# wengroup/matten

Hardware: AMD Instinct MI355X
Metric: edge_tensor_products_per_sec (higher is better)
Workload: dtype f32; 1 GPU; configs[2]: synthetic fcc-64 crystals (64 atoms, cutoff 5 A, 1152 edges each), paper hparams lmax=4, eval forward backbone+out_layer, one batch per step per GPU; last conv layer run for its live outputs only (258/842 radial-weight columns: the irreps its only reader takes) -- `value` counts 4 edge-TP per edge all the same, `value_full_layers` is the rate with the full last layer; nodes_per_gpu=64000, edges_per_gpu=1152000, conv_layers=4

## Files before the change

### include/matten_hip.h

```cpp
#ifndef MATTEN_HIP_H
#define MATTEN_HIP_H

#include <stddef.h>
#include <stdint.h>

#ifdef __cplusplus
extern "C" {
#endif

typedef void* matten_stream_t;

#define MATTEN_OK 0
#define MATTEN_EINVAL (-1)
#define MATTEN_ELAUNCH (-2)
#define MATTEN_ENOMEM (-3)

int matten_abi_version(void);

#define MATTEN_RADIAL_MAX_MID 3

size_t matten_csr_workspace_bytes(int64_t n_edges, int64_t n_nodes);
int matten_csr_counting_max_avg_degree(void);
int matten_csr_build(const int64_t* edge_index, int64_t n_edges, int64_t n_nodes, int32_t* perm,
                     int32_t* rowptr, int32_t* src_sorted, void* workspace, size_t workspace_bytes,
                     int32_t* err_flag, matten_stream_t stream);

int64_t matten_csr_split_bound(int64_t n_nodes, int64_t n_edges, int64_t max_len);
int matten_csr_split(const int32_t* rowptr, int64_t n_nodes, int64_t n_edges, int64_t max_len, int32_t* vrowptr,
                     int64_t* vseg, const float* num_neigh, float* vnn, matten_stream_t stream);

size_t matten_group_workspace_bytes(int64_t n, int64_t n_keys);
int matten_group_by_key(const int64_t* key, int64_t n, int64_t n_keys, int32_t* order, int32_t* seg,
                        void* workspace, size_t workspace_bytes, int32_t* err_flag, matten_stream_t stream);

int matten_species_embed(const int64_t* atomic_numbers, int64_t n_nodes, const int64_t* z_to_index,
                         int64_t min_z, int64_t max_z, int64_t n_species, const float* weight ,
                         const float* bias , int64_t dim, int64_t* species_index, int32_t* species_i32,
                         float* node_feats, float* node_attrs, int32_t* err_flag, matten_stream_t stream);

int matten_edge_geom(const float* pos, const int64_t* edge_index, const float* edge_cell_shift,
                     const float* cell, int64_t n_cells, const int64_t* batch, const int32_t* perm,
                     int64_t n_edges, int64_t n_nodes, int lmax, int n_basis, float r_start, float r_end,
                     float* geom_sorted, float* sh_sorted, int sh_stride, float* edge_vectors, float* edge_lengths,
                     float* edge_attrs, float* edge_embedding, matten_stream_t stream);

int matten_radial_mlp(const float* geom_sorted, int64_t n_edges, int n_basis, float r_start, float r_end,
                      const float* w0p, int nb_pad, const float* w1p, const float* w2p, int hidden, int w_pad,
                      float act_cst, void* w_edge, int out_is_bf16, matten_stream_t stream);
int matten_radial_mlp_deep(const float* geom_sorted, int64_t n_edges, int n_basis, float r_start, float r_end,
                           const float* w0p, int nb_pad, const float* w_mid, int n_mid, const float* w2p, int hidden,
                           int w_pad, float act_cst, void* w_edge, int out_is_bf16, matten_stream_t stream);

int matten_tp_tile_nodes(void);
int matten_tp_paths(const float* x, int64_t d_in, const void* w_edge, int64_t w_pad, const float* sh_sorted,
                    int64_t sh_dim, const int32_t* rowptr, const int32_t* src_sorted, int64_t n_nodes,
                    const int32_t* path_entries, const int32_t* unit_start, int64_t n_entries,
                    int64_t units_per_tile, int64_t d_mid, float avg_num_neighbors, const float* num_neigh,
                    float* agg , int w_is_bf16, matten_stream_t stream);

int matten_agg_linear_max_mt(void);
int matten_agg_linear_block_chunks(void);
size_t matten_agg_linear_lds_bytes(int64_t w_stride, int64_t n_io, int64_t n_blocks);
size_t matten_agg_linear_max_lds_bytes(void);
int matten_agg_linear(const float* agg, int64_t ld, const int32_t* order, const int32_t* seg, int64_t n_species,
                      const float* wtab, int64_t w_stride, const int32_t* io_table, int64_t n_io,
                      const int32_t* blocks, int64_t n_blocks, const float* add, int64_t add_ld, int64_t d_out,
                      int64_t n_rows, float* out, matten_stream_t stream);
int matten_agg_linear_gate(const float* agg, int64_t ld, const int32_t* order, const int32_t* seg, int64_t n_species,
                           const float* wtab, int64_t w_stride, const int32_t* io_table, int64_t n_io,
                           const int32_t* blocks, int64_t n_blocks, const float* add, int64_t add_ld, int64_t d_out,
                           int64_t n_rows, const int32_t* cmeta, const float* act_cst, const float* bn_scale,
                           const float* bn_shift, int64_t d_act, float* out, matten_stream_t stream);
int matten_agg_linear_gate_sets(void);
int matten_radial_hidden(const float* geom_sorted, int64_t n_edges, int n_basis, float r_start, float r_end,
                         const float* w0p, int nb_pad, const float* w1p, int hidden, uint16_t* h2s,
                         const float* h_scale, matten_stream_t stream);
int matten_radial_hidden_multi(const float* geom_sorted, int64_t n_edges, int n_basis, float r_start, float r_end,
                               const float* const* w0p, int nb_pad, const float* const* w1p, int hidden,
                               uint16_t* const* h2s, const float* const* h_scale, int n_layers,
                               matten_stream_t stream);
int matten_radial_hidden_deep(const float* geom_sorted, int64_t n_edges, int n_basis, float r_start, float r_end,
                              const float* w0p, int nb_pad, const float* w_mid, int n_mid, int hidden, uint16_t* h2s,
                              const float* h_scale, matten_stream_t stream);
int matten_radial_hidden_multi_deep(const float* geom_sorted, int64_t n_edges, int n_basis, float r_start, float r_end,
                                    const float* const* w0p, int nb_pad, const float* const* w_mid, int n_mid, int hidden,
                                    uint16_t* const* h2s, const float* const* h_scale, int n_layers,
                                    matten_stream_t stream);
int matten_tp_fused(const float* x, int64_t d_in, const uint16_t* h2s, const float* w2p, int64_t w_pad,
                    const float* sh_sorted, int64_t sh_stride, const int32_t* rowptr, const int32_t* src_sorted,
                    int64_t n_nodes, const int32_t* group_entries, const int32_t* unit_map, int64_t n_entries,
                    int64_t units_per_tile, int64_t lds_floats_per_wave, int64_t d_mid, float avg_num_neighbors,
                    const float* num_neigh, const uint16_t* a_split, const float* a_scale_inv,
                    float* agg , matten_stream_t stream);

int matten_tp_max_cols(void);
int matten_tp_max_cols_l0(void);
int matten_tp_max_cols_l1(void);
int matten_tp_groups_hash(void);

int matten_species_linear(const float* x, int64_t d_in, const int32_t* order, const int32_t* seg, int64_t n_species,
                          const float* wp, int64_t w_stride, const int32_t* segs, int64_t n_segs, int64_t d_out,
                          const float* add, int64_t add_ld, int64_t n_rows, float* out, matten_stream_t stream);

int matten_species_linear_rows(const float* x, int64_t d_in, const int32_t* order, const int32_t* seg, int64_t n_species,
                               const float* wp, int64_t w_stride, const int32_t* segs, int64_t n_segs, int64_t d_out,
                               const float* add, int64_t add_ld, int64_t n_rows, float* out, matten_stream_t stream);

int matten_gate_bn(const float* x, int64_t d_in, const int32_t* meta, int64_t d_out, const float* act_cst,
                   const float* running_mean, const float* running_var, const float* bn_weight,
                   const float* bn_bias, float eps, int64_t n_rows, float* out, matten_stream_t stream);

int matten_segment_reduce(const float* x, int64_t dim, const int64_t* ptr, int64_t n_segments, int mean,
                          float* out, matten_stream_t stream);
int matten_segment_minmax(const float* x, int64_t dim, const int64_t* ptr, int64_t n_segments, int take_max, float* out,
                          int64_t* arg, matten_stream_t stream);
int matten_segment_minmax_bwd(const float* dy, int64_t dim, const int64_t* arg, int64_t n_segments, float* dx,
                              matten_stream_t stream);

int64_t matten_radial_mlp_bwd_small_slices(int64_t n_edges);
int64_t matten_radial_mlp_bwd_w2_ranges(int64_t n_edges, int64_t w_pad);
int matten_radial_mlp_bwd(const float* geom_sorted, int64_t n_edges, int n_basis, float r_start, float r_end,
                          const float* w0p, int nb_pad, const float* w1p, const float* w2p, int hidden, int w_pad,
                          int w_cols, const void* dw, int64_t dw_ld, int dw_is_bf16, float* h2_scratch,
                          float* part_small, float* part_w2, float scale0, float scale1, float scale2,
                          float* grad_small, float* grad_w2, matten_stream_t stream);
int64_t matten_radial_mlp_bwd_w2_ranges_deep(int64_t n_edges, int64_t w_pad, int n_mid);
int matten_radial_mlp_bwd_deep(const float* geom_sorted, int64_t n_edges, int n_basis, float r_start, float r_end,
                               const float* w0p, int nb_pad, const float* w_mid, int n_mid, const float* w2p, int hidden,
                               int w_pad, int w_cols, const void* dw, int64_t dw_ld, int dw_is_bf16, float* h2_scratch,
                               float* part_small, float* part_w2, float scale0, float scale1, float scale2,
                               float* grad_small, float* grad_w2, matten_stream_t stream);
int matten_radial_pack(const float* w0, const float* w1, const float* w2, int n_basis, int nb_pad, int w_cols, int w_pad,
                       float scale0, float scale1, float scale2, float* w0p, float* w1p, float* w2p,
                       matten_stream_t stream);
int matten_radial_pack_deep(const float* w0, const float* w_mid, int n_mid, const float* w2, int n_basis, int nb_pad,
                            int w_cols, int w_pad, float scale0, float scale1, float scale2, float* w0p, float* w_mid_p,
                            float* w2p, matten_stream_t stream);
int matten_radial_pack_cols(const float* w0, const float* w1, const float* w2, int n_basis, int nb_pad, int w_cols,
                            const int64_t* cols, int n_cols, int w_pad, float scale0, float scale1, float scale2, float* w0p,
                            float* w1p, float* w2p, matten_stream_t stream);
int matten_radial_h_scale(const float* w0, const float* w1, int n_basis, float r_start, float r_end, float act_cst,
                          float* out2, matten_stream_t stream);
int matten_radial_pack_cols_deep(const float* w0, const float* w_mid, int n_mid, const float* w2, int n_basis, int nb_pad,
                                 int w_cols, const int64_t* cols, int n_cols, int w_pad, float scale0, float scale1,
                                 float scale2, float* w0p, float* w_mid_p, float* w2p, matten_stream_t stream);
int matten_radial_h_scale_deep(const float* w0, const float* w_mid, int n_mid, int n_basis, float r_start, float r_end,
// ... 34 lines not shown
                                 int64_t dw_ld, int edge_is_bf16, int64_t n_nodes, const int32_t* out_ptr,
                                 const int32_t* out_perm, float* dx_edges, int64_t lds_floats, int max_l, int max_mul,
                                 matten_stream_t stream);

int matten_species_linear_wgrad(const float* x, int64_t d_in, const float* dy, int64_t d_out, const int32_t* order,
                                const int32_t* seg, int64_t n_species, int64_t n_rows, const int32_t* segs,
                                int64_t n_segs, int64_t w_stride, float* dwp, float* scratch, matten_stream_t stream);

int matten_gate_bwd(const float* x, int64_t d_in, const int32_t* meta, int64_t d_out, const float* act_cst,
                    const float* dy, int64_t n_rows, float* dx, matten_stream_t stream);

int64_t matten_bn_scratch_floats(int64_t n_rows, int64_t dim);
int matten_bn_train_fwd(const float* x, int64_t dim, int64_t n_rows, const int32_t* col2chan, const int32_t* chan,
                        int64_t n_chan, const float* weight, const float* bias, float eps, float* mean, float* nu,
                        float* y, float* running_mean, float* running_var, float momentum, float* scratch,
                        matten_stream_t stream);
int matten_bn_train_bwd(const float* x, const float* dy, int64_t dim, int64_t n_rows, const int32_t* col2chan,
                        const int32_t* chan, int64_t n_chan, const float* mean, const float* nu, const float* weight,
                        float eps, float* A, float* B, float* dx, float* dweight, float* dbias, float* scratch,
                        matten_stream_t stream);

int matten_norm_act(const float* x, int64_t dim, int64_t n_rows, const int32_t* chan, int64_t n_chan, int act,
                    float epsilon, const float* running_mean, const float* running_var, const float* bn_weight,
                    const float* bn_bias, float bn_eps, float* y, matten_stream_t stream);
int matten_norm_act_bwd(const float* x, const float* dy, int64_t dim, int64_t n_rows, const int32_t* chan, int64_t n_chan,
                        int act, float epsilon, float* dx, matten_stream_t stream);

int matten_instance_norm_fwd(const float* x, int64_t dim, int64_t n_rows, const int64_t* seg_ptr, const int64_t* seg_of_row,
                             int64_t n_seg, const int32_t* col2chan, const int32_t* chan, int64_t n_chan,
                             const float* weight, const float* bias, float eps, float* mean, float* nu, float* y,
                             matten_stream_t stream);
int matten_instance_norm_bwd(const float* x, const float* dy, int64_t dim, int64_t n_rows, const int64_t* seg_ptr,
                             const int64_t* seg_of_row, int64_t n_seg, const int32_t* col2chan, const int32_t* chan,
                             int64_t n_chan, const float* mean, const float* nu, const float* weight, float eps, float* A,
                             float* B, float* dx, matten_stream_t stream);

int matten_segment_reduce_bwd(const float* dy, int64_t dim, const int64_t* ptr, int64_t n_segments, int mean, float* dx,
                              matten_stream_t stream);


int matten_graph_prep(const double* pos, const double* cell, const int64_t* ptr, int64_t n_crystals, double r_cut,
                      double* frac, double* bound, int64_t* batch, float* pos_f32, float* cell_f32,
                      matten_stream_t stream);
int matten_neighbor_count(const double* pos, const double* cell, const int64_t* ptr, const double* frac,
                          const double* bound, const int64_t* pair_ptr, double r_cut, int64_t n_crystals,
                          int64_t max_atoms, int32_t* counts, int32_t* counts_t, matten_stream_t stream);
int matten_neighbor_summary(const int64_t* offsets, const int64_t* pair_ptr, int64_t n_crystals, int64_t* out2,
                            matten_stream_t stream);
int matten_neighbor_fill(const double* pos, const double* cell, const int64_t* ptr, const double* frac,
                         const double* bound, const int64_t* pair_ptr, double r_cut, int64_t n_crystals,
                         int64_t max_atoms, const int64_t* offsets, int64_t n_edges, int64_t* edge_index,
                         float* edge_cell_shift, float* num_neigh, const int64_t* offsets_t, int64_t n_atoms,
                         int32_t* rowptr, int32_t* src_sorted, int32_t* perm, matten_stream_t stream);

#ifdef __cplusplus
}
#endif
#endif
```

### matten_amd/_lib.py

```python
from __future__ import annotations

import ctypes
import os
from ctypes import c_float, c_int, c_int32, c_int64, c_size_t, c_void_p

_HERE = os.path.dirname(os.path.abspath(__file__))
LIB_PATH = os.path.join(_HERE, "libmatten_hip.so")

ABI_VERSION = 45

P = c_void_p
SIGNATURES = {
    "matten_abi_version": (c_int, []),
    "matten_csr_workspace_bytes": (c_size_t, [c_int64, c_int64]),
    "matten_group_workspace_bytes": (c_size_t, [c_int64, c_int64]),
    "matten_csr_counting_max_avg_degree": (c_int, []),
    "matten_csr_build": (c_int, [P, c_int64, c_int64, P, P, P, P, c_size_t, P, P]),
    "matten_csr_split_bound": (c_int64, [c_int64, c_int64, c_int64]),
    "matten_csr_split": (c_int, [P, c_int64, c_int64, c_int64, P, P, P, P, P]),
    "matten_group_by_key": (c_int, [P, c_int64, c_int64, P, P, P, c_size_t, P, P]),
    "matten_species_embed": (c_int, [P, c_int64, P, c_int64, c_int64, c_int64, P, P, c_int64, P, P, P, P, P, P]),
    "matten_edge_geom": (c_int, [P, P, P, P, c_int64, P, P, c_int64, c_int64, c_int, c_int, c_float, c_float, P, P, c_int, P, P, P, P, P]),
    "matten_radial_mlp": (c_int, [P, c_int64, c_int, c_float, c_float, P, c_int, P, P, c_int, c_int, c_float, P, c_int, P]),
    "matten_radial_mlp_deep": (c_int, [P, c_int64, c_int, c_float, c_float, P, c_int, P, c_int, P, c_int, c_int, c_float, P, c_int,
                                       P]),
    "matten_tp_tile_nodes": (c_int, []),
    "matten_tp_paths": (c_int, [P, c_int64, P, c_int64, P, c_int64, P, P, c_int64, P, P, c_int64, c_int64, c_int64, c_float, P, P, c_int,
                                P]),
    "matten_radial_hidden_multi": (c_int, [P, c_int64, c_int, c_float, c_float, P, c_int, P, c_int, P, P, c_int, P]),
    "matten_radial_hidden_multi_deep": (c_int, [P, c_int64, c_int, c_float, c_float, P, c_int, P, c_int, c_int, P, P, c_int, P]),
    "matten_agg_linear_max_mt": (c_int, []),
    "matten_agg_linear_block_chunks": (c_int, []),
    "matten_agg_linear_lds_bytes": (c_size_t, [c_int64, c_int64, c_int64]),
    "matten_agg_linear_max_lds_bytes": (c_size_t, []),
    "matten_agg_linear": (c_int, [P, c_int64, P, P, c_int64, P, c_int64, P, c_int64, P, c_int64, P, c_int64, c_int64,
                                  c_int64, P, P]),
    "matten_agg_linear_gate": (c_int, [P, c_int64, P, P, c_int64, P, c_int64, P, c_int64, P, c_int64, P, c_int64, c_int64,
                                       c_int64, P, P, P, P, c_int64, P, P]),
    "matten_agg_linear_gate_sets": (c_int, []),
    "matten_radial_hidden": (c_int, [P, c_int64, c_int, c_float, c_float, P, c_int, P, c_int, P, P, P]),
    "matten_radial_hidden_deep": (c_int, [P, c_int64, c_int, c_float, c_float, P, c_int, P, c_int, c_int, P, P, P]),
    "matten_tp_max_cols": (c_int, []),
    "matten_tp_max_cols_l0": (c_int, []),
    "matten_tp_max_cols_l1": (c_int, []),
    "matten_tp_groups_hash": (c_int, []),
    "matten_tp_fused": (c_int, [P, c_int64, P, P, c_int64, P, c_int64, P, P, c_int64, P, P, c_int64, c_int64, c_int64, c_int64, c_float, P, P, P, P, P]),
    "matten_species_linear": (c_int, [P, c_int64, P, P, c_int64, P, c_int64, P, c_int64, c_int64, P, c_int64, c_int64, P, P]),
    "matten_species_linear_rows": (c_int, [P, c_int64, P, P, c_int64, P, c_int64, P, c_int64, c_int64, P, c_int64, c_int64, P, P]),
    "matten_radial_mlp_bwd_small_slices": (c_int64, [c_int64]),
    "matten_radial_mlp_bwd_w2_ranges": (c_int64, [c_int64, c_int64]),
    "matten_radial_mlp_bwd_w2_ranges_deep": (c_int64, [c_int64, c_int64, c_int]),
    "matten_radial_mlp_bwd": (c_int, [P, c_int64, c_int, c_float, c_float, P, c_int, P, P, c_int, c_int, c_int, P, c_int64,
                                      c_int, P, P, P, c_float, c_float, c_float, P, P, P]),
    "matten_radial_mlp_bwd_deep": (c_int, [P, c_int64, c_int, c_float, c_float, P, c_int, P, c_int, P, c_int, c_int, c_int, P,
                                           c_int64, c_int, P, P, P, c_float, c_float, c_float, P, P, P]),
    "matten_radial_pack": (c_int, [P, P, P, c_int, c_int, c_int, c_int, c_float, c_float, c_float, P, P, P, P]),
    "matten_radial_pack_deep": (c_int, [P, P, c_int, P, c_int, c_int, c_int, c_int, c_float, c_float, c_float, P, P, P, P]),
    "matten_radial_pack_cols": (c_int, [P, P, P, c_int, c_int, c_int, P, c_int, c_int, c_float, c_float, c_float, P, P, P, P]),
    "matten_radial_pack_cols_deep": (c_int, [P, P, c_int, P, c_int, c_int, c_int, P, c_int, c_int, c_float, c_float, c_float, P, P,
                                             P, P]),
    "matten_radial_h_scale": (c_int, [P, P, c_int, c_float, c_float, c_float, P, P]),
    "matten_radial_h_scale_deep": (c_int, [P, P, c_int, c_int, c_float, c_float, c_float, P, P]),
    "matten_split_a_tiles": (c_int, [P, c_int64, P, c_int64, P, P, P, P]),
    "matten_gather_scale": (c_int, [P, P, P, c_int64, c_int64, c_int, P, P, P, P]),
    "matten_species_linear_wgrad_scratch_floats": (c_int64, [c_int64, c_int64, c_int64]),
    "matten_tp_backward": (c_int, [P, c_int64, P, c_int64, P, c_int64, P, P, P, c_int64, P, P, P, c_int64, c_float, P, c_int64, P, P, c_int64,
                                   P, P, c_int64, c_int, P]),
    "matten_tp_backward_lit": (c_int, [P, c_int64, P, c_int64, P, c_int64, P, P, P, c_int64, c_int64, P, c_int64, P, c_int64, c_float,
                                       P, c_int64, P, P, c_int64, c_int, c_int64, P, P, P, c_int, P]),
    "matten_tp_backward_lit_wfree": (c_int, [P, c_int64, P, P, P, P, c_int64, P, P, P, c_int64, c_int64, P, c_int64, P, c_int64, c_float,
                                             P, c_int64, P, P, c_int64, c_int, c_int64, P, P, P, c_int64, c_int, c_int, P]),
    "matten_adam_step": (c_int, [P, P, P, P, c_int64, P, c_float, c_float, c_float, c_float, c_float, P]),
    "matten_species_linear_wgrad": (c_int, [P, c_int64, P, c_int64, P, P, c_int64, c_int64, P, c_int64, c_int64, P, P, P]),
    "matten_gate_bwd": (c_int, [P, c_int64, P, c_int64, P, P, c_int64, P, P]),
    "matten_bn_scratch_floats": (c_int64, [c_int64, c_int64]),
    "matten_bn_train_fwd": (c_int, [P, c_int64, c_int64, P, P, c_int64, P, P, c_float, P, P, P, P, P, c_float, P, P]),
    "matten_bn_train_bwd": (c_int, [P, P, c_int64, c_int64, P, P, c_int64, P, P, P, c_float, P, P, P, P, P, P, P]),
    "matten_norm_act": (c_int, [P, c_int64, c_int64, P, c_int64, c_int, c_float, P, P, P, P, c_float, P, P]),
    "matten_norm_act_bwd": (c_int, [P, P, c_int64, c_int64, P, c_int64, c_int, c_float, P, P]),
    "matten_instance_norm_fwd": (c_int, [P, c_int64, c_int64, P, P, c_int64, P, P, c_int64, P, P, c_float, P, P, P, P]),
    "matten_instance_norm_bwd": (c_int, [P, P, c_int64, c_int64, P, P, c_int64, P, P, c_int64, P, P, P, c_float, P, P, P, P]),
    "matten_segment_reduce_bwd": (c_int, [P, c_int64, P, c_int64, c_int, P, P]),
    "matten_graph_prep": (c_int, [P, P, P, c_int64, ctypes.c_double, P, P, P, P, P, P]),
    "matten_neighbor_count": (c_int, [P, P, P, P, P, P, ctypes.c_double, c_int64, c_int64, P, P, P]),
    "matten_neighbor_summary": (c_int, [P, P, c_int64, P, P]),
    "matten_neighbor_fill": (c_int, [P, P, P, P, P, P, ctypes.c_double, c_int64, c_int64, P, c_int64, P, P, P, P, c_int64,
                                     P, P, P, P]),
    "matten_gate_bn": (c_int, [P, c_int64, P, c_int64, P, P, P, P, P, c_float, c_int64, P, P]),
    "matten_segment_reduce": (c_int, [P, c_int64, P, c_int64, c_int, P, P]),
    "matten_segment_minmax": (c_int, [P, c_int64, P, c_int64, c_int, P, P, P]),
    "matten_segment_minmax_bwd": (c_int, [P, c_int64, P, c_int64, P, P]),
    "matten_dense_rows": (c_int, [P, c_int64, P, c_int64, c_int64, P, P]),
}

_lib = None


class MattenHipError(RuntimeError):
    pass


def load() -> ctypes.CDLL:
    global _lib
    if _lib is not None:
        return _lib
    if not os.path.exists(LIB_PATH):
        raise MattenHipError(
            f"{LIB_PATH} not found: the HIP extension is not built. matten_amd has no CPU fallback; "
            "run `make -C matten_amd/csrc` (needs hipcc, --offload-arch=gfx950)."
        )
    lib = ctypes.CDLL(LIB_PATH)
    for name, (res, args) in SIGNATURES.items():
        try:
            fn = getattr(lib, name)
        except AttributeError as e:
            raise MattenHipError(f"symbol {name} missing from {LIB_PATH}") from e
        fn.restype = res
        fn.argtypes = args
    v = lib.matten_abi_version()
    if v != ABI_VERSION:
        raise MattenHipError(f"ABI version mismatch: library {v}, python binding {ABI_VERSION}")
    _lib = lib
    return lib


_ERRORS = {-1: "MATTEN_EINVAL (bad argument)", -2: "MATTEN_ELAUNCH (HIP launch failed)", -3: "MATTEN_ENOMEM (workspace too small)"}


def check(rc: int, what: str) -> None:
    if rc != 0:
        raise MattenHipError(f"{what} failed: {_ERRORS.get(rc, rc)}")
```

### matten_amd/autograd.py

```python
from typing import Optional

import os

import torch

from . import ops


class SpeciesEmbedFn(torch.autograd.Function):

    @staticmethod
    def forward(ctx, weight, bias, feats, species_order, segs):
        ctx.species_order, ctx.segs = species_order, segs
        ctx.n_species = weight.shape[1]
        return feats.view_as(feats)

    @staticmethod
    def backward(ctx, g):
        g = g.contiguous()
        n, dim = g.shape
        ones = torch.ones(n, 1, dtype=torch.float32, device=g.device)
        per_species = ops.species_linear_wgrad(ones, g, ctx.species_order, ctx.n_species, [ctx.segs], dim)
        return per_species.t(), per_species.sum(0), None, None, None

# ... 115 lines not shown
    @staticmethod
    def backward(ctx, g):
        x, w_edge = ctx.saved_tensors
        mod, dev = ctx.mod, g.device
        sh, src, dst = ctx.graph
        impl = os.environ.get("MATTEN_TP_BWD", "lit")
        if impl == "lit":
            out_csr = ctx.out_csr if os.environ.get("MATTEN_TP_BWD_DX", "ordered") != "atomic" else None
            dx, dw = ops.tp_backward_lit(x, w_edge, sh, src, dst, mod._tables.get("bw_blocks", dev),
                                         mod._tables.get("bw_paths", dev), mod.plan.bw_sum_lanes, g.contiguous(), ctx.avg,
                                         ctx.num_neigh, out_csr=out_csr, max_l=mod.plan.bw_max_l,
                                         blocks_cover_input=int(mod.plan.bw_blocks[:, 1].dot(2 * mod.plan.bw_blocks[:, 2] + 1))
                                         == mod.plan.d_in)
            return dx, dw, None, None, None, None
        dx, dw = ops.tp_backward(x, w_edge, sh, src, dst, mod._tables.get("bw_col_meta", dev),
                                 mod._tables.get("bw_nnz_ijk", dev), mod._tables.get("bw_nnz_c", dev), g.contiguous(),
                                 ctx.avg, ctx.num_neigh,
                                 in_groups=None if os.environ.get("MATTEN_TP_BWD_GROUPED", "1") == "0" else
                                 (mod._tables.get("bw_in_ptr", dev), mod._tables.get("bw_in_cols", dev)))
        return dx, dw, None, None, None, None


W_FREE_ADJOINT = os.environ.get("MATTEN_TP_BWD_WFREE", "1") != "0"


class FusedTensorProductFn(torch.autograd.Function):

    @staticmethod
    def forward(ctx, x, mod, data, avg, num_neigh, *ws):
        from .data.irreps import DataKey

        dev = x.device
        p, mlp = mod.plan, mod.weight_nn
        nb, r0, r1 = data[DataKey.AMD_RBF].tolist()
        ctx.mod, ctx.avg, ctx.num_neigh = mod, avg, num_neigh
        ctx.rbf = (int(nb), float(r0), float(r1))
        ctx.graph = (data[DataKey.AMD_GEOM], data[DataKey.AMD_SH], data[DataKey.AMD_SRC], data["_amd_dst_sorted"])
        ctx.out_csr = data.get("_amd_out_csr")
        ctx.save_for_backward(x, *ws)
        gent = mod._tables.get("gentries", dev)
        if mlp.deep:
            w0p, w1p, w2p, hs, frag, inv = ops.fused_operands_deep(ws[0], _stack_mid(ws), ws[-1], mlp.pack_scales(),
                                                                   mod._tables.get("fused_cols", dev), gent, p.fused_a_tiles,
                                                                   r0, r1, mlp.act_cst)
            h2p = ops.radial_hidden_deep(data[DataKey.AMD_GEOM], int(nb), r0, r1, w0p, w1p, hs)
        else:
            w0p, w1p, w2p, hs, frag, inv = ops.fused_operands(*ws, mlp.pack_scales(), mod._tables.get("fused_cols", dev),
                                                              gent, p.fused_a_tiles, r0, r1, mlp.act_cst)
            h2p = ops.radial_hidden(data[DataKey.AMD_GEOM], int(nb), r0, r1, w0p, w1p, hs)
        if W_FREE_ADJOINT and p.bw_max_mul <= ops.WFREE_MAX_MUL:
            ctx.h2p, ctx.hs = h2p, hs
        return ops.tp_fused(x, h2p, w2p, data[DataKey.AMD_SH], data[DataKey.AMD_ROWPTR], data[DataKey.AMD_SRC], gent,
                            mod._tables.get("gumap", dev), len(p.fused_unit_map), p.fused_lds_floats_per_wave, p.d_mid, avg,
                            num_neigh, a_split=(frag, inv))

    @staticmethod
    def backward(ctx, g):
        x, *ws = ctx.saved_tensors
        mod, dev = ctx.mod, g.device
        mlp = mod.weight_nn
        geom, sh, src, dst = ctx.graph
        scales = mlp.pack_scales()
        w0p, w1p, w2p = _radial_pack(mlp, ws)
        out_csr = ctx.out_csr if os.environ.get("MATTEN_TP_BWD_DX", "ordered") != "atomic" else None
        covered = int(mod.plan.bw_blocks[:, 1].dot(2 * mod.plan.bw_blocks[:, 2] + 1)) == mod.plan.d_in
        h2p = getattr(ctx, "h2p", None)
        if h2p is not None:
            frag, inv = ops.split_a_tiles_dev(w2p, mod._tables.get("bw_w_entries", dev), mod.plan.bw_a_tiles, ctx.hs)
            dx, dw = ops.tp_backward_lit(x, None, sh, src, dst, mod._tables.get("bw_blocks", dev),
                                         mod._tables.get("bw_paths", dev), mod.plan.bw_sum_lanes, g.contiguous(), ctx.avg,
                                         ctx.num_neigh, out_csr=out_csr, blocks_cover_input=covered, wfree=(h2p, frag, inv),
                                         dw_shape=((geom.shape[0], w2p.shape[1]), EDGE_STORAGE_DTYPE),
                                         lds_floats=mod.plan.bw_wfree_lds_floats, max_l=mod.plan.bw_max_l,
                                         max_mul=mod.plan.bw_max_mul)
        else:
            w_edge = _radial_mlp(mlp, geom, ctx.rbf, w0p, w1p, w2p)
            dx, dw = ops.tp_backward_lit(x, w_edge, sh, src, dst, mod._tables.get("bw_blocks", dev),
                                         mod._tables.get("bw_paths", dev), mod.plan.bw_sum_lanes, g.contiguous(), ctx.avg,
                                         ctx.num_neigh, out_csr=out_csr, blocks_cover_input=covered, max_l=mod.plan.bw_max_l)
            del w_edge
        return (dx, None, None, None, None) + _radial_mlp_bwd(mlp, geom, ctx.rbf, w0p, w1p, w2p, dw, scales)


class GateFn(torch.autograd.Function):
    @staticmethod
    def forward(ctx, x, mod):
        dev = x.device
        ctx.mod = mod
        ctx.save_for_backward(x)
        return ops.gate_bn(x, mod._tables.get("meta", dev), mod._tables.get("act_cst", dev))

    @staticmethod
    def backward(ctx, g):
        (x,) = ctx.saved_tensors
        mod, dev = ctx.mod, g.device
        return ops.gate_bwd(x, mod._tables.get("meta", dev), mod._tables.get("act_cst", dev), g.contiguous()), None


class NormActFn(torch.autograd.Function):
    @staticmethod
    def forward(ctx, x, mod):
        ctx.mod = mod
        ctx.save_for_backward(x)
        return ops.norm_act(x, mod._tables.get("chan", x.device), mod.plan.act_code, mod.plan.epsilon)

    @staticmethod
    def backward(ctx, g):
# ... 88 lines not shown
```

### matten_amd/csrc/csr.hip

```cpp
#include <cstring>

#include <rocprim/device/device_radix_sort.hpp>
#include <rocprim/device/device_scan.hpp>

#include "common.h"

namespace {

__global__ void csr_keys_kernel(const int64_t* __restrict__ edge_index, int64_t E, int64_t N,
                                int32_t* __restrict__ keys, int32_t* __restrict__ vals, int32_t* err_flag) {
    int64_t e = (int64_t)blockIdx.x * blockDim.x + threadIdx.x;
    if (e >= E) return;
    int64_t s = edge_index[e];
    int64_t d = edge_index[E + e];
    if (s < 0 || s >= N || d < 0 || d >= N) {
        atomicOr(err_flag, 1);
        d = d < 0 ? 0 : (d >= N ? N - 1 : d);
    }
    keys[e] = (int32_t)d;
    vals[e] = (int32_t)e;
}

__global__ void csr_rowptr_kernel(const int32_t* __restrict__ keys_sorted, int64_t E, int64_t N,
                                  int32_t* __restrict__ rowptr) {
    int64_t n = (int64_t)blockIdx.x * blockDim.x + threadIdx.x;
    if (n > N) return;
    int64_t lo = 0, hi = E;
    while (lo < hi) {
        int64_t mid = (lo + hi) >> 1;
        if (keys_sorted[mid] < (int32_t)n) lo = mid + 1; else hi = mid;
    }
    rowptr[n] = (int32_t)lo;
}

__global__ void csr_src_kernel(const int64_t* __restrict__ edge_index, const int32_t* __restrict__ perm, int64_t E,
                               int64_t N, int32_t* __restrict__ src_sorted) {
    int64_t e = (int64_t)blockIdx.x * blockDim.x + threadIdx.x;
    if (e >= E) return;
    int64_t s = edge_index[perm[e]];
    s = s < 0 ? 0 : (s >= N ? N - 1 : s);
    src_sorted[e] = (int32_t)s;
}

__global__ void zero_i32_kernel(int32_t* __restrict__ p, int64_t n) {
    int64_t i = (int64_t)blockIdx.x * blockDim.x + threadIdx.x;
    if (i < n) p[i] = 0;
}

__global__ void csr_count_kernel(const int64_t* __restrict__ edge_index, int64_t E, int64_t N,
                                 int32_t* __restrict__ deg, int32_t* __restrict__ slot, int32_t* err_flag) {
    int64_t e = (int64_t)blockIdx.x * blockDim.x + threadIdx.x;
    if (e >= E) return;
    int64_t s = edge_index[e];
    int64_t d = edge_index[E + e];
    if (s < 0 || s >= N || d < 0 || d >= N) {
        atomicOr(err_flag, 1);
        d = d < 0 ? 0 : (d >= N ? N - 1 : d);
    }
    slot[e] = atomicAdd(&deg[d], 1);
}

__global__ void csr_place_kernel(const int64_t* __restrict__ edge_index, int64_t E, int64_t N,
                                 const int32_t* __restrict__ rowptr, const int32_t* __restrict__ slot,
                                 int32_t* __restrict__ ids) {
    int64_t e = (int64_t)blockIdx.x * blockDim.x + threadIdx.x;
    if (e >= E) return;
    int64_t d = edge_index[E + e];
    d = d < 0 ? 0 : (d >= N ? N - 1 : d);
    ids[rowptr[d] + slot[e]] = (int32_t)e;
}

constexpr int CSR_HUB_DEGREE = 2048;
constexpr int CSR_HUB_THREADS = 1024;
constexpr int CSR_HUB_BLOCKS = 64;

__global__ void csr_rank_kernel(const int64_t* __restrict__ edge_index, const int32_t* __restrict__ rowptr,
                                const int32_t* __restrict__ ids, int64_t E, int64_t N, int32_t* __restrict__ perm,
                                int32_t* __restrict__ src_sorted, int32_t* __restrict__ hubs) {
    const int64_t node = ((int64_t)blockIdx.x * blockDim.x + threadIdx.x) >> 4;
    if (node >= N) return;
    const int sub = threadIdx.x & 15;
    const int beg = rowptr[node], d = rowptr[node + 1] - beg;
    if (d > CSR_HUB_DEGREE) {
        if (sub == 0) hubs[atomicAdd(&hubs[N], 1)] = (int32_t)node;
        return;
    }
    for (int i = sub; i < d; i += 16) {
        const int id = ids[beg + i];
        int rank = 0;
        int j = 0;
        for (; j + 8 <= d; j += 8) {
            int v[8];
#pragma unroll
            for (int q = 0; q < 8; ++q) v[q] = ids[beg + j + q];
#pragma unroll
            for (int q = 0; q < 8; ++q) rank += v[q] < id;
        }
        for (; j < d; ++j) rank += ids[beg + j] < id;
        perm[beg + rank] = id;
        int64_t s = edge_index[id];
        s = s < 0 ? 0 : (s >= N ? N - 1 : s);
        src_sorted[beg + rank] = (int32_t)s;
    }
}

__global__ __launch_bounds__(CSR_HUB_THREADS) void csr_hub_kernel(const int64_t* __restrict__ edge_index,
                                                                  const int32_t* __restrict__ rowptr, int32_t* ids,
                                                                  int64_t N, int32_t* __restrict__ perm,
                                                                  int32_t* __restrict__ src_sorted,
                                                                  const int32_t* __restrict__ hubs) {
    const int n_hubs = hubs[N];
    for (int h = blockIdx.x; h < n_hubs; h += gridDim.x) {
        const int node = hubs[h];
        const int beg = rowptr[node], d = rowptr[node + 1] - beg;
        int32_t* a = ids + beg;
        for (int64_t k = 2; (k >> 1) < d; k <<= 1) {
            for (int64_t j = k >> 1; j > 0; j >>= 1) {
                const int64_t m = (j == (k >> 1)) ? k - 1 : j;
                for (int64_t i = threadIdx.x; i < d; i += CSR_HUB_THREADS) {
                    const int64_t l = i ^ m;
                    if (l > i && l < d) {
                        const int32_t x = a[i], y = a[l];
                        if (y < x) a[i] = y, a[l] = x;
                    }
                }
                __syncthreads();
            }
        }
        for (int64_t i = threadIdx.x; i < d; i += CSR_HUB_THREADS) {
            const int32_t id = a[i];
            perm[beg + i] = id;
            int64_t s = edge_index[id];
            s = s < 0 ? 0 : (s >= N ? N - 1 : s);
            src_sorted[beg + i] = (int32_t)s;
        }
        __syncthreads();
    }
}

__global__ void group_keys_kernel(const int64_t* __restrict__ key, int64_t n, int64_t n_keys,
                                  int32_t* __restrict__ keys, int32_t* __restrict__ vals, int32_t* err_flag) {
    int64_t i = (int64_t)blockIdx.x * blockDim.x + threadIdx.x;
    if (i >= n) return;
    int64_t k = key[i];
    if (k < 0 || k >= n_keys) {
        atomicOr(err_flag, 1);
        k = k < 0 ? 0 : n_keys - 1;
    }
    keys[i] = (int32_t)k;
    vals[i] = (int32_t)i;
}

constexpr int GROUP_COUNTING_MAX_KEYS = 256;
constexpr int GROUP_WAVES = 4;

__device__ __forceinline__ int group_key_of(const int64_t* __restrict__ key, int64_t i, int64_t n, int64_t n_keys,
                                            int32_t* err_flag) {
    if (i >= n) return -1;
    int64_t k = key[i];
    if (k < 0 || k >= n_keys) {
        atomicOr(err_flag, 1);
        k = k < 0 ? 0 : n_keys - 1;
    }
    return (int)k;
}

__global__ __launch_bounds__(GROUP_WAVES * 64) void group_hist_kernel(const int64_t* __restrict__ key, int64_t n,
                                                                      int64_t n_keys, int64_t n_runs,
                                                                      int32_t* __restrict__ cnt, int32_t* err_flag) {
    __shared__ int h[GROUP_WAVES][GROUP_COUNTING_MAX_KEYS];
    const int wv = threadIdx.x >> 6, lane = threadIdx.x & 63;
    const int64_t run = (int64_t)blockIdx.x * GROUP_WAVES + wv;
    for (int kk = lane; kk < n_keys; kk += 64) h[wv][kk] = 0;
    __builtin_amdgcn_wave_barrier();
    const int k = group_key_of(key, run * 64 + lane, n, n_keys, err_flag);
    if (k >= 0) atomicAdd(&h[wv][k], 1);
    __builtin_amdgcn_s_waitcnt(0xc07f);
    __builtin_amdgcn_wave_barrier();
    if (run < n_runs)
        for (int kk = lane; kk < n_keys; kk += 64) cnt[(int64_t)kk * n_runs + run] = h[wv][kk];
}

__global__ __launch_bounds__(GROUP_WAVES * 64) void group_place_kernel(const int64_t* __restrict__ key, int64_t n,
                                                                       int64_t n_keys, int64_t n_runs,
                                                                       const int32_t* __restrict__ offs,
                                                                       int32_t* __restrict__ order,
                                                                       int32_t* __restrict__ seg, int32_t* err_flag) {
    const int lane = threadIdx.x & 63;
    const int64_t i = (int64_t)blockIdx.x * blockDim.x + threadIdx.x;
    const int64_t run = i >> 6;
    if (i <= n_keys) seg[i] = i < n_keys ? offs[i * n_runs] : (int32_t)n;
    const int k = group_key_of(key, i, n, n_keys, err_flag);
    unsigned long long todo = __ballot(k >= 0);
    int rank = 0;
    while (todo) {
        const int kf = __shfl(k, __ffsll((long long)todo) - 1);
        const unsigned long long m = __ballot(k == kf);
        if (k == kf) rank = __popcll(m & ((1ull << lane) - 1ull));
        todo &= ~m;
    }
    if (k >= 0) order[offs[(int64_t)k * n_runs + run] + rank] = (int32_t)i;
}

inline size_t align256(size_t x) { return (x + 255) & ~(size_t)255; }

inline int key_bits(int64_t N) {
    int b = 1;
    while (((int64_t)1 << b) < N && b < 31) ++b;
    return b;
}

}

__global__ __launch_bounds__(1024) void csr_split_kernel(const int* __restrict__ rowptr, int N, int max_len, int nv_bound,
                                                         int* __restrict__ vrowptr, int64_t* __restrict__ vseg,
                                                         const float* __restrict__ num_neigh, float* __restrict__ vnn) {
    __shared__ int sh[1024];
    __shared__ int carry_s;
    const int t = threadIdx.x;
    if (t == 0) carry_s = 0;
    __syncthreads();
    const int E = rowptr[N];
    for (int base = 0; base < N; base += 1024) {
        const int n = base + t;
        int beg = 0, k = 0, d = 0;
        if (n < N) {
            beg = rowptr[n];
            d = rowptr[n + 1] - beg;
            k = max(1, (d + max_len - 1) / max_len);
        }
        sh[t] = k;
        __syncthreads();
        for (int off = 1; off < 1024; off <<= 1) {
            const int v = t >= off ? sh[t - off] : 0;
            __syncthreads();
            sh[t] += v;
            __syncthreads();
        }
        const int carry = carry_s;
        const int first = carry + sh[t] - k;
        if (n < N) {
            vseg[n] = first;
            for (int i = 0; i < k; ++i) {
                const int v = first + i;
                if (v < nv_bound) {
                    vrowptr[v] = beg + (int)((int64_t)i * d / k);
                    if (vnn) vnn[v] = num_neigh[n];
                }
            }
        }
        __syncthreads();
        if (t == 1023) carry_s = carry + sh[1023];
        __syncthreads();
    }
    const int nv = min(carry_s, nv_bound);
    if (t == 0) vseg[N] = nv;
    for (int v = nv + t; v <= nv_bound; v += 1024) {
        vrowptr[v] = E;
        if (vnn && v < nv_bound) vnn[v] = 1.0f;
    }
}

extern "C" size_t matten_csr_workspace_bytes(int64_t E, int64_t N) {
    if (E < 0 || N < 0) return 0;
    size_t tmp = 0;
    int32_t* p = nullptr;
    (void)rocprim::radix_sort_pairs(nullptr, tmp, p, p, p, p, (size_t)(E > 0 ? E : 1), 0, key_bits(N), 0, false);
    size_t scan_tmp = 0;
    (void)rocprim::exclusive_scan(nullptr, scan_tmp, p, p, 0, (size_t)(N + 1), rocprim::plus<int32_t>());
    return 3 * align256((size_t)(E > 0 ? E : 1) * sizeof(int32_t)) + align256(tmp) + align256((size_t)(N + 1) * sizeof(int32_t)) +
           align256(scan_tmp) + 256;
}

extern "C" size_t matten_group_workspace_bytes(int64_t n, int64_t n_keys) {
    if (n < 0 || n_keys <= 0) return 0;
    size_t need = matten_csr_workspace_bytes(n, n_keys);
    if (n_keys <= GROUP_COUNTING_MAX_KEYS) {
        const size_t table = (size_t)n_keys * (size_t)((n + 63) / 64 + 1);
        size_t scan_tmp = 0;
        int32_t* p = nullptr;
        (void)rocprim::exclusive_scan(nullptr, scan_tmp, p, p, 0, table, rocprim::plus<int32_t>());
        const size_t counting = 2 * align256(table * sizeof(int32_t)) + align256(scan_tmp) + 256;
        if (counting > need) need = counting;
    }
    return need;
}

constexpr int64_t CSR_COUNTING_MAX_AVG_DEGREE = 64;

extern "C" int matten_csr_counting_max_avg_degree(void) { return (int)CSR_COUNTING_MAX_AVG_DEGREE; }

extern "C" int matten_csr_build(const int64_t* edge_index, int64_t E, int64_t N, int32_t* perm, int32_t* rowptr,
                                int32_t* src_sorted, void* workspace, size_t workspace_bytes, int32_t* err_flag,
                                matten_stream_t stream_) {
    hipStream_t stream = (hipStream_t)stream_;
    if (E < 0 || N < 0 || N >= ((int64_t)1 << 31) || E >= ((int64_t)1 << 31)) return MATTEN_EINVAL;
    if (!rowptr || !err_flag) return MATTEN_EINVAL;
    if (E == 0) {
        zero_i32_kernel<<<(unsigned)matten_cdiv(N + 1, 256), 256, 0, stream>>>(rowptr, N + 1);
        MATTEN_LAUNCH_CHECK();
        return MATTEN_OK;
    }
    if (!edge_index || !perm || !src_sorted || !workspace) return MATTEN_EINVAL;
    size_t need = matten_csr_workspace_bytes(E, N);
    if (workspace_bytes < need) return MATTEN_ENOMEM;

    char* ws = (char*)workspace;
    size_t seg = align256((size_t)E * sizeof(int32_t));
    int32_t* keys_in = (int32_t*)ws;
    int32_t* keys_out = (int32_t*)(ws + seg);
    int32_t* vals_in = (int32_t*)(ws + 2 * seg);
    void* tmp = ws + 3 * seg;
    size_t tmp_bytes = workspace_bytes - 3 * seg;

    const int T = 256;
    if (N > 0 && E <= CSR_COUNTING_MAX_AVG_DEGREE * N) {
        int32_t* ids = (int32_t*)ws;
        int32_t* slot = (int32_t*)(ws + seg);
        int32_t* deg = (int32_t*)(ws + 2 * seg);
        const size_t deg_bytes = align256((size_t)(N + 1) * sizeof(int32_t));
        void* scan_tmp = ws + 2 * seg + deg_bytes;
        size_t scan_bytes = workspace_bytes - 2 * seg - deg_bytes;
        zero_i32_kernel<<<(unsigned)matten_cdiv(N + 1, T), T, 0, stream>>>(deg, N + 1);
        MATTEN_LAUNCH_CHECK();
        csr_count_kernel<<<(unsigned)matten_cdiv(E, T), T, 0, stream>>>(edge_index, E, N, deg, slot, err_flag);
        MATTEN_LAUNCH_CHECK();
        if (rocprim::exclusive_scan(scan_tmp, scan_bytes, deg, rowptr, 0, (size_t)(N + 1), rocprim::plus<int32_t>(),
                                    stream) != hipSuccess)
            return MATTEN_ELAUNCH;
        csr_place_kernel<<<(unsigned)matten_cdiv(E, T), T, 0, stream>>>(edge_index, E, N, rowptr, slot, ids);
        MATTEN_LAUNCH_CHECK();
        csr_rank_kernel<<<(unsigned)matten_cdiv(N * 16, T), T, 0, stream>>>(edge_index, rowptr, ids, E, N, perm,
                                                                           src_sorted, deg);
        MATTEN_LAUNCH_CHECK();
        if (E > CSR_HUB_DEGREE) {
            const int64_t max_hubs = E / CSR_HUB_DEGREE;
            csr_hub_kernel<<<(unsigned)(max_hubs < CSR_HUB_BLOCKS ? max_hubs : CSR_HUB_BLOCKS), CSR_HUB_THREADS, 0,
                             stream>>>(edge_index, rowptr, ids, N, perm, src_sorted, deg);
            MATTEN_LAUNCH_CHECK();
        }
        return MATTEN_OK;
    }
    csr_keys_kernel<<<(unsigned)matten_cdiv(E, T), T, 0, stream>>>(edge_index, E, N, keys_in, vals_in, err_flag);
    MATTEN_LAUNCH_CHECK();
    if (rocprim::radix_sort_pairs(tmp, tmp_bytes, keys_in, keys_out, vals_in, perm, (size_t)E, 0, key_bits(N), stream,
                                  false) != hipSuccess)
        return MATTEN_ELAUNCH;
    csr_rowptr_kernel<<<(unsigned)matten_cdiv(N + 1, T), T, 0, stream>>>(keys_out, E, N, rowptr);
    MATTEN_LAUNCH_CHECK();
    csr_src_kernel<<<(unsigned)matten_cdiv(E, T), T, 0, stream>>>(edge_index, perm, E, N, src_sorted);
    MATTEN_LAUNCH_CHECK();
    return MATTEN_OK;
}

extern "C" int matten_group_by_key(const int64_t* key, int64_t n, int64_t n_keys, int32_t* order, int32_t* seg,
                                   void* workspace, size_t workspace_bytes, int32_t* err_flag, matten_stream_t stream_) {
    hipStream_t stream = (hipStream_t)stream_;
    if (n < 0 || n_keys <= 0 || n_keys >= ((int64_t)1 << 31) || n >= ((int64_t)1 << 31)) return MATTEN_EINVAL;
    if (!seg || !err_flag) return MATTEN_EINVAL;
    if (n == 0) {
        zero_i32_kernel<<<(unsigned)matten_cdiv(n_keys + 1, 256), 256, 0, stream>>>(seg, n_keys + 1);
        MATTEN_LAUNCH_CHECK();
        return MATTEN_OK;
    }
    if (!key || !order || !workspace) return MATTEN_EINVAL;
    if (workspace_bytes < matten_group_workspace_bytes(n, n_keys)) return MATTEN_ENOMEM;
    char* ws = (char*)workspace;
    if (n_keys <= GROUP_COUNTING_MAX_KEYS) {
        const int64_t n_runs = (n + 63) / 64;
        const size_t table = (size_t)n_keys * (size_t)n_runs;
        const size_t tb = align256((size_t)n_keys * (size_t)(n_runs + 1) * sizeof(int32_t));
        int32_t* cnt = (int32_t*)ws;
        int32_t* offs = (int32_t*)(ws + tb);
        void* scan_tmp = ws + 2 * tb;
        size_t scan_bytes = workspace_bytes - 2 * tb;
        const int TB = GROUP_WAVES * 64;
        group_hist_kernel<<<(unsigned)matten_cdiv(n_runs, GROUP_WAVES), TB, 0, stream>>>(key, n, n_keys, n_runs, cnt,
                                                                                        err_flag);
        MATTEN_LAUNCH_CHECK();
        if (rocprim::exclusive_scan(scan_tmp, scan_bytes, cnt, offs, 0, table, rocprim::plus<int32_t>(), stream) !=
            hipSuccess)
            return MATTEN_ELAUNCH;
        const int64_t threads = n > n_keys + 1 ? n : n_keys + 1;
        group_place_kernel<<<(unsigned)matten_cdiv(threads, TB), TB, 0, stream>>>(key, n, n_keys, n_runs, offs, order,
                                                                                 seg, err_flag);
        MATTEN_LAUNCH_CHECK();
        return MATTEN_OK;
    }
    size_t sg = align256((size_t)n * sizeof(int32_t));
    int32_t* keys_in = (int32_t*)ws;
    int32_t* keys_out = (int32_t*)(ws + sg);
    int32_t* vals_in = (int32_t*)(ws + 2 * sg);
    void* tmp = ws + 3 * sg;
    size_t tmp_bytes = workspace_bytes - 3 * sg;
    const int T = 256;
    group_keys_kernel<<<(unsigned)matten_cdiv(n, T), T, 0, stream>>>(key, n, n_keys, keys_in, vals_in, err_flag);
    MATTEN_LAUNCH_CHECK();
    if (rocprim::radix_sort_pairs(tmp, tmp_bytes, keys_in, keys_out, vals_in, order, (size_t)n, 0, key_bits(n_keys),
                                  stream, false) != hipSuccess)
        return MATTEN_ELAUNCH;
    csr_rowptr_kernel<<<(unsigned)matten_cdiv(n_keys + 1, T), T, 0, stream>>>(keys_out, n, n_keys, seg);
    MATTEN_LAUNCH_CHECK();
    return MATTEN_OK;
}

extern "C" int64_t matten_csr_split_bound(int64_t n_nodes, int64_t n_edges, int64_t max_len) {
    return max_len > 0 ? n_nodes + n_edges / max_len : n_nodes;
}

extern "C" int matten_csr_split(const int32_t* rowptr, int64_t n_nodes, int64_t n_edges, int64_t max_len, int32_t* vrowptr,
                                int64_t* vseg, const float* num_neigh, float* vnn, matten_stream_t stream_) {
    if (n_nodes < 0 || n_edges < 0 || max_len <= 0 || n_nodes >= ((int64_t)1 << 30) || n_edges >= ((int64_t)1 << 31))
        return MATTEN_EINVAL;
    if (!rowptr || !vrowptr || !vseg || ((num_neigh == nullptr) != (vnn == nullptr))) return MATTEN_EINVAL;
    const int64_t bound = matten_csr_split_bound(n_nodes, n_edges, max_len);
    if (bound >= ((int64_t)1 << 31)) return MATTEN_EINVAL;
    csr_split_kernel<<<1, 1024, 0, (hipStream_t)stream_>>>(rowptr, (int)n_nodes, (int)max_len, (int)bound, vrowptr, vseg,
                                                          num_neigh, vnn);
    MATTEN_LAUNCH_CHECK();
    return MATTEN_OK;
}
```

### matten_amd/csrc/neighbor.hip

```cpp
#include "common.h"

#pragma clang fp contract(off)

namespace {

struct Cry {
    const double* pos;
    const double* cell;
    const int64_t* ptr;
    const double* frac;
    const double* bound;
    const int64_t* pair_ptr;
};

__global__ __launch_bounds__(64) void graph_prep_kernel(const double* __restrict__ pos, const double* __restrict__ cell,
                                                        const int64_t* __restrict__ ptr, double r_cut,
                                                        double* __restrict__ frac, double* __restrict__ bound,
                                                        int64_t* __restrict__ batch, float* __restrict__ pos_f32,
                                                        float* __restrict__ cell_f32) {
    const int64_t b = blockIdx.x;
    const double* cl = cell + 9 * b;
    const double ax = cl[0], ay = cl[1], az = cl[2], bx = cl[3], by = cl[4], bz = cl[5], cx = cl[6], cy = cl[7], cz = cl[8];
    const double c0x = by * cz - bz * cy, c0y = bz * cx - bx * cz, c0z = bx * cy - by * cx;
    const double c1x = cy * az - cz * ay, c1y = cz * ax - cx * az, c1z = cx * ay - cy * ax;
    const double c2x = ay * bz - az * by, c2y = az * bx - ax * bz, c2z = ax * by - ay * bx;
    const double det = (ax * c0x + ay * c0y) + az * c0z;
    const double i00 = c0x / det, i10 = c0y / det, i20 = c0z / det;
    const double i01 = c1x / det, i11 = c1y / det, i21 = c1z / det;
    const double i02 = c2x / det, i12 = c2y / det, i22 = c2z / det;
    if (threadIdx.x < 9) cell_f32[9 * b + threadIdx.x] = (float)cl[threadIdx.x];
    if (threadIdx.x == 0) {
        bound[3 * b] = r_cut * sqrt((i00 * i00 + i10 * i10) + i20 * i20);
        bound[3 * b + 1] = r_cut * sqrt((i01 * i01 + i11 * i11) + i21 * i21);
        bound[3 * b + 2] = r_cut * sqrt((i02 * i02 + i12 * i12) + i22 * i22);
    }
    const int64_t lo = ptr[b], hi = ptr[b + 1];
    for (int64_t n = lo + threadIdx.x; n < hi; n += blockDim.x) {
        const double x = pos[3 * n], y = pos[3 * n + 1], z = pos[3 * n + 2];
        frac[3 * n] = (x * i00 + y * i10) + z * i20;
        frac[3 * n + 1] = (x * i01 + y * i11) + z * i21;
        frac[3 * n + 2] = (x * i02 + y * i12) + z * i22;
        pos_f32[3 * n] = (float)x, pos_f32[3 * n + 1] = (float)y, pos_f32[3 * n + 2] = (float)z;
        batch[n] = b;
    }
}

__device__ __forceinline__ void shift_range(double bound, double df, int& lo, int& hi) {
    const double slack = 1e-6 * (1.0 + fabs(df) + bound);
    lo = (int)ceil(-bound - df - slack);
    hi = (int)floor(bound - df + slack);
}

struct CsrOut {
    const int64_t* offsets_t;
    int32_t* rowptr;
    int32_t* src_sorted;
    int32_t* perm;
    int64_t n_atoms;
};

template <bool FILL>
__global__ __launch_bounds__(256) void neighbor_kernel(Cry c, double r_cut, int32_t* __restrict__ counts,
                                                       int32_t* __restrict__ counts_t,
                                                       const int64_t* __restrict__ offsets,
                                                       int64_t* __restrict__ edge_index, int64_t n_edges,
                                                       float* __restrict__ shifts, float* __restrict__ num_neigh,
                                                       CsrOut csr) {
    const int64_t b = blockIdx.y;
    const int64_t lo = c.ptr[b];
    const int64_t n = c.ptr[b + 1] - lo;
    const int64_t t = (int64_t)blockIdx.x * blockDim.x + threadIdx.x;
    if (t >= n * n) return;
    const int64_t i = lo + t / n, j = lo + t % n;
    const int64_t pair = c.pair_ptr[b] + t;
    const double* cl = c.cell + 9 * b;
    int x0, x1, y0, y1, z0, z1;
    shift_range(c.bound[3 * b], c.frac[3 * j] - c.frac[3 * i], x0, x1);
    shift_range(c.bound[3 * b + 1], c.frac[3 * j + 1] - c.frac[3 * i + 1], y0, y1);
    shift_range(c.bound[3 * b + 2], c.frac[3 * j + 2] - c.frac[3 * i + 2], z0, z1);
    const double pix = c.pos[3 * i], piy = c.pos[3 * i + 1], piz = c.pos[3 * i + 2];
    const double pjx = c.pos[3 * j], pjy = c.pos[3 * j + 1], pjz = c.pos[3 * j + 2];
    const double r2 = r_cut * r_cut;
    const double r2_in = r2 * (1.0 - 1e-15), r2_out = r2 * (1.0 + 1e-15);
    int64_t out = FILL ? offsets[pair] : 0;
    if (FILL && num_neigh && j == lo) num_neigh[i] = (float)(offsets[pair + n] - offsets[pair]);
    const int64_t pair_t = c.pair_ptr[b] + (j - lo) * n + (i - lo);
    int64_t out_t = 0;
    if (FILL && csr.rowptr) {
        out_t = csr.offsets_t[pair_t] - csr.offsets_t[0];
        if (i == lo) csr.rowptr[j] = (int32_t)out_t;
        if (pair == 0) csr.rowptr[csr.n_atoms] = (int32_t)n_edges;
    }
    int cnt = 0;
    for (int sx = x0; sx <= x1; ++sx)
        for (int sy = y0; sy <= y1; ++sy) {
            const double ax = (double)sx * cl[0] + (double)sy * cl[3];
            const double ay = (double)sx * cl[1] + (double)sy * cl[4];
            const double az = (double)sx * cl[2] + (double)sy * cl[5];
            for (int sz = z0; sz <= z1; ++sz) {
                const double tx = ax + (double)sz * cl[6];
                const double ty = ay + (double)sz * cl[7];
                const double tz = az + (double)sz * cl[8];
                const double dx = (pjx + tx) - pix, dy = (pjy + ty) - piy, dz = (pjz + tz) - piz;
                const double d2 = (dx * dx + dy * dy) + dz * dz;
                bool hit = d2 < r2_in;
                if (!hit && d2 <= r2_out) hit = sqrt(d2) < r_cut;
                if (hit && !(i == j && sx == 0 && sy == 0 && sz == 0)) {
                    if (FILL) {
                        edge_index[out] = i;
                        edge_index[n_edges + out] = j;
                        shifts[3 * out] = (float)sx;
                        shifts[3 * out + 1] = (float)sy;
                        shifts[3 * out + 2] = (float)sz;
                        if (csr.rowptr) {
                            csr.perm[out_t] = (int32_t)out;
                            csr.src_sorted[out_t] = (int32_t)i;
                            ++out_t;
                        }
                        ++out;
                    }
                    ++cnt;
                }
            }
        }
    if (!FILL) {
        counts[pair] = cnt;
        if (counts_t) counts_t[pair_t] = cnt;
    }
}

__global__ __launch_bounds__(256) void neighbor_summary_kernel(const int64_t* __restrict__ offsets,
                                                               const int64_t* __restrict__ pair_ptr, int64_t n_crystals,
                                                               int64_t* __restrict__ out) {
    __shared__ long long red[256];
    long long m = LLONG_MAX;
    for (int64_t b = threadIdx.x; b < n_crystals; b += blockDim.x)
        m = min(m, (long long)(offsets[pair_ptr[b + 1]] - offsets[pair_ptr[b]]));
    red[threadIdx.x] = m;
    __syncthreads();
    for (int o = 128; o > 0; o >>= 1) {
        if (threadIdx.x < o) red[threadIdx.x] = min(red[threadIdx.x], red[threadIdx.x + o]);
        __syncthreads();
    }
    if (threadIdx.x == 0) {
        out[0] = offsets[pair_ptr[n_crystals]];
        out[1] = n_crystals > 0 ? (int64_t)red[0] : 0;
    }
}

}

extern "C" int matten_graph_prep(const double* pos, const double* cell, const int64_t* ptr, int64_t n_crystals,
                                 double r_cut, double* frac, double* bound, int64_t* batch, float* pos_f32,
                                 float* cell_f32, matten_stream_t stream_) {
    hipStream_t stream = (hipStream_t)stream_;
    if (n_crystals < 0 || !(r_cut > 0.0) || n_crystals >= ((int64_t)1 << 31)) return MATTEN_EINVAL;
    if (n_crystals == 0) return MATTEN_OK;
    if (!pos || !cell || !ptr || !frac || !bound || !batch || !pos_f32 || !cell_f32) return MATTEN_EINVAL;
    graph_prep_kernel<<<(unsigned)n_crystals, 64, 0, stream>>>(pos, cell, ptr, r_cut, frac, bound, batch, pos_f32, cell_f32);
    MATTEN_LAUNCH_CHECK();
    return MATTEN_OK;
}

extern "C" int matten_neighbor_count(const double* pos, const double* cell, const int64_t* ptr, const double* frac,
                                     const double* bound, const int64_t* pair_ptr, double r_cut, int64_t n_crystals,
                                     int64_t max_atoms, int32_t* counts, int32_t* counts_t, matten_stream_t stream_) {
    hipStream_t stream = (hipStream_t)stream_;
    if (n_crystals < 0 || max_atoms < 0 || !(r_cut > 0.0) || n_crystals > 65535) return MATTEN_EINVAL;
    if (n_crystals == 0 || max_atoms == 0) return MATTEN_OK;
    if (!pos || !cell || !ptr || !frac || !bound || !pair_ptr || !counts) return MATTEN_EINVAL;
    Cry c{pos, cell, ptr, frac, bound, pair_ptr};
    dim3 grid((unsigned)matten_cdiv(max_atoms * max_atoms, 256), (unsigned)n_crystals);
    neighbor_kernel<false><<<grid, 256, 0, stream>>>(c, r_cut, counts, counts_t, nullptr, nullptr, 0, nullptr, nullptr, CsrOut{});
    MATTEN_LAUNCH_CHECK();
    return MATTEN_OK;
}

extern "C" int matten_neighbor_summary(const int64_t* offsets, const int64_t* pair_ptr, int64_t n_crystals,
                                       int64_t* out2, matten_stream_t stream_) {
    hipStream_t stream = (hipStream_t)stream_;
    if (n_crystals < 0 || !offsets || !pair_ptr || !out2) return MATTEN_EINVAL;
    neighbor_summary_kernel<<<1, 256, 0, stream>>>(offsets, pair_ptr, n_crystals, out2);
    MATTEN_LAUNCH_CHECK();
    return MATTEN_OK;
}

extern "C" int matten_neighbor_fill(const double* pos, const double* cell, const int64_t* ptr, const double* frac,
                                    const double* bound, const int64_t* pair_ptr, double r_cut, int64_t n_crystals,
                                    int64_t max_atoms, const int64_t* offsets, int64_t n_edges, int64_t* edge_index,
                                    float* edge_cell_shift, float* num_neigh, const int64_t* offsets_t, int64_t n_atoms,
                                    int32_t* rowptr, int32_t* src_sorted, int32_t* perm, matten_stream_t stream_) {
    hipStream_t stream = (hipStream_t)stream_;
    if (n_crystals < 0 || max_atoms < 0 || n_edges < 0 || !(r_cut > 0.0) || n_crystals > 65535) return MATTEN_EINVAL;
    if (n_crystals == 0 || max_atoms == 0) return MATTEN_OK;
    if (!pos || !cell || !ptr || !frac || !bound || !pair_ptr || !offsets) return MATTEN_EINVAL;
    if (n_edges > 0 && (!edge_index || !edge_cell_shift)) return MATTEN_EINVAL;
    const bool want_csr = offsets_t || rowptr || src_sorted || perm;
    if (want_csr && (!offsets_t || !rowptr || n_atoms < 0 || n_edges >= ((int64_t)1 << 31) ||
                     (n_edges > 0 && (!src_sorted || !perm))))
        return MATTEN_EINVAL;
    Cry c{pos, cell, ptr, frac, bound, pair_ptr};
    CsrOut csr{offsets_t, want_csr ? rowptr : nullptr, src_sorted, perm, n_atoms};
    dim3 grid((unsigned)matten_cdiv(max_atoms * max_atoms, 256), (unsigned)n_crystals);
    neighbor_kernel<true><<<grid, 256, 0, stream>>>(c, r_cut, nullptr, nullptr, offsets, edge_index, n_edges, edge_cell_shift,
                                                    num_neigh, csr);
    MATTEN_LAUNCH_CHECK();
    return MATTEN_OK;
}
```

### matten_amd/csrc/node.hip

```cpp
#include "common.h"

namespace {

__device__ __forceinline__ float apply_act(int code, float v) {
    switch (code) {
        case 1: return v / (1.0f + expf(-v));
        case 2: return tanhf(v);
        case 3: return 1.0f / (1.0f + expf(-v));
        case 4: return (v > 20.0f ? v : log1pf(expf(v))) - 0.6931471805599453f;
        case 5: return fabsf(v);
        default: return v;
    }
}

#ifndef GB_R
#define GB_R 16
#endif
#ifndef GB_U
#define GB_U 8
#endif
constexpr int GB_ROWS = GB_R, GB_UNROLL = GB_U;
__global__ __launch_bounds__(256) void gate_bn_kernel(const float* __restrict__ x, int d_in,
                                                           const int4* __restrict__ meta, int d_out,
                                                           const float* __restrict__ act_cst,
// ... 121 lines not shown
}

extern "C" int matten_segment_reduce(const float* x, int64_t dim, const int64_t* ptr, int64_t n_segments, int mean,
                                     float* out, matten_stream_t stream_) {
    hipStream_t stream = (hipStream_t)stream_;
    if (n_segments < 0 || dim <= 0) return MATTEN_EINVAL;
    if (n_segments == 0) return MATTEN_OK;
    if (!x || !ptr || !out) return MATTEN_EINVAL;
    const int T = 256;
    segment_reduce_kernel<<<(unsigned)matten_cdiv(n_segments * dim, T), T, 0, stream>>>(x, (int)dim, ptr, n_segments,
                                                                                        mean, out);
    MATTEN_LAUNCH_CHECK();
    return MATTEN_OK;
}

extern "C" int matten_segment_minmax(const float* x, int64_t dim, const int64_t* ptr, int64_t n_segments, int take_max,
                                     float* out, int64_t* arg, matten_stream_t stream_) {
    hipStream_t stream = (hipStream_t)stream_;
    if (n_segments < 0 || dim <= 0) return MATTEN_EINVAL;
    if (n_segments == 0) return MATTEN_OK;
    if (!x || !ptr || !out) return MATTEN_EINVAL;
    const int T = 256;
    segment_minmax_kernel<<<(unsigned)matten_cdiv(n_segments * dim, T), T, 0, stream>>>(x, (int)dim, ptr, n_segments,
                                                                                        take_max, out, arg);
    MATTEN_LAUNCH_CHECK();
    return MATTEN_OK;
}

extern "C" int matten_segment_minmax_bwd(const float* dy, int64_t dim, const int64_t* arg, int64_t n_segments, float* dx,
                                         matten_stream_t stream_) {
    hipStream_t stream = (hipStream_t)stream_;
    if (n_segments < 0 || dim <= 0) return MATTEN_EINVAL;
    if (n_segments == 0) return MATTEN_OK;
    if (!dy || !arg || !dx) return MATTEN_EINVAL;
    const int T = 256;
    segment_minmax_bwd_kernel<<<(unsigned)matten_cdiv(n_segments * dim, T), T, 0, stream>>>(dy, (int)dim, arg, n_segments, dx);
    MATTEN_LAUNCH_CHECK();
    return MATTEN_OK;
}

extern "C" int matten_dense_rows(const float* x, int64_t n_in, const float* q, int64_t n_out, int64_t n_rows,
                                 float* out, matten_stream_t stream_) {
    hipStream_t stream = (hipStream_t)stream_;
    if (n_rows < 0 || n_in <= 0 || n_out <= 0) return MATTEN_EINVAL;
    if (n_rows == 0) return MATTEN_OK;
    if (!x || !q || !out) return MATTEN_EINVAL;
    const int T = 256;
    dense_rows_kernel<<<(unsigned)matten_cdiv(n_rows * n_out, T), T, 0, stream>>>(x, (int)n_in, q, (int)n_out, n_rows,
                                                                                  out);
    MATTEN_LAUNCH_CHECK();
    return MATTEN_OK;
}

extern "C" int matten_abi_version(void) { return 45; }
```

### matten_amd/csrc/tp_fused.hip

```cpp
#include "tp_walk.h"

namespace {

using namespace matten_walk;

constexpr int KIND_MERGED = 256;
struct StoreAgg {
    template <class G>
    __device__ __forceinline__ void store(const Args& a, const GroupEntry& ge, const float* __restrict__ acc,
                                          float a_scale_inv, int node, int j, int u, bool valid) const {
        if (TPF_LAB_NO_STORE ? (valid && acc[0] == 12345.678f) : valid) {
            const float nn = a.avg_nn > 0.0f ? a.avg_nn : a.num_neigh[node];
            const float norm = a_scale_inv / sqrtf(nn);
            float* orow = a.agg + (int64_t)node * a.d_mid;
            const bool merged = (ge.kind & KIND_MERGED) != 0;
            const GroupEntry& g2 = (&ge)[merged ? 1 : 0];
            const bool second = merged && u >= 2;
            const unsigned mask = merged ? (second ? g2.mask : (unsigned)g2.w_base) : ge.mask;
            const int uc = second ? u - 2 : u;
#pragma unroll
            for (int cc = 0; cc < G::NC; ++cc) {
                if ((mask >> cc) & 1u) {
                    const int d3 = 2 * G::L3[cc] + 1;
                    const int ks = second ? g2.t_off[cc] : ge.t_off[cc];
                    float* op = orow + (second ? g2.out_off[cc] : ge.out_off[cc]) + (ks ? uc : uc * d3);
                    const int kstep = ks ? ks : 1;
#pragma unroll
                    for (int k = 0; k < 2 * matten::CG_LMAX + 1; ++k)
                        if (k < d3) op[k * kstep] = acc[G::OFF[cc] + k] * norm;
                }
            }
        }
    }
};

template <int L1, int GI>
__device__ __forceinline__ void run_group(const Args& a, const GroupEntry& ge, float* __restrict__ tile, int node,
                                          int lane, bool valid, int beg, int deg_node, int maxdeg) {
    const int deg = valid ? deg_node : 0;
    using G = matten::Group<L1, GI>;
    constexpr int NC = G::NC;
    float acc[G::NACC];
#pragma unroll
    for (int k = 0; k < G::NACC; ++k) acc[k] = 0.0f;

    const unsigned mask = ge.mask;
    const int cu_log2 = ge.cu_log2;
    const int cu = 1 << cu_log2;
    const int npw = 64 >> cu_log2;
    const int ch_log2 = npw >= 16 ? 0 : (4 - (6 - cu_log2));
    const int CH = 1 << ch_log2;
    const int T = npw >= 16 ? (npw >> 4) : 1;
    const int ncols = ge.mul * NC;
    const int MT = (ncols + 15) >> 4;
    const int ycol = MT * 16;
    const int stride = MT * 16 + 32 + 4;

    const int j = lane >> cu_log2;
    const int u = lane & (cu - 1);
    const int g = lane >> 4, c = lane & 15;
    const int xcol = ge.x_off + u * G::D1;
    constexpr int CAPC = cap_channels(L1, NC);
    constexpr int MTMAX = (CAPC * NC + 15) / 16;
    f16x8 ah[MTMAX], al[MTMAX];
    float a_scale_inv;
    {
        float av[MTMAX][8];
        float amax = 0.0f;
#pragma unroll
        for (int mt = 0; mt < MTMAX; ++mt) {
#pragma unroll
            for (int kk = 0; kk < 8; ++kk) {
                const int k = 16 * (kk >> 2) + 4 * g + (kk & 3);
                av[mt][kk] = (mt < MT) ? a.w2p[(int64_t)k * a.w_pad + ge.w_base + mt * 16 + c] : 0.0f;
                amax = fmaxf(amax, fabsf(av[mt][kk]));
            }
        }
#pragma unroll
        for (int off = 32; off > 0; off >>= 1) amax = fmaxf(amax, __shfl_xor(amax, off));
        int e = (int)((__float_as_uint(amax) >> 23) & 0xffu) - 127;
        e = amax > 0.0f ? max(-100, min(100, e)) : 13;
        const float a_scale = __uint_as_float((unsigned)(127 + 13 - e) << 23);
        a_scale_inv = __uint_as_float((unsigned)(127 - 13 + e) << 23);
#pragma unroll
        for (int mt = 0; mt < MTMAX; ++mt) {
#pragma unroll
            for (int kk = 0; kk < 8; ++kk) {
                _Float16 hi, lo;
                split_f16(av[mt][kk] * a_scale, hi, lo);
                ah[mt][kk] = hi;
                al[mt][kk] = lo;
            }
        }
    }

    const int e_last = deg > 0 ? beg + deg - 1 : 0;
    float xn[G::D1];
    int src_nn;
    {
        const int src0 = a.src_sorted[min(beg, e_last)];
        src_nn = a.src_sorted[min(beg + 1, e_last)];
        const float* xp0 = a.x + (int64_t)src0 * a.d_in + xcol;
#pragma unroll
        for (int i = 0; i < G::D1; ++i) xn[i] = xp0[i];
    }
    for (int s0 = 0; s0 < maxdeg; s0 += CH) {
#pragma unroll
        for (int t = 0; t < 4; ++t) {
            if (t < T) {
                const int n = 16 * t + c;
                const int jn = n >> ch_log2, so = n & (CH - 1);
                const int begn = __shfl(beg, jn << cu_log2);
                const int degn = __shfl(deg_node, jn << cu_log2);
                f16x8 bh = {0, 0, 0, 0, 0, 0, 0, 0}, bl = {0, 0, 0, 0, 0, 0, 0, 0};
                if (s0 + so < degn) {
                    const int64_t en = begn + s0 + so;
                    const f16x8* hp = reinterpret_cast<const f16x8*>(a.h2s + en * (2 * HID) + g * 8);
                    bh = hp[0];
                    bl = hp[HID / 8];
                    const f32x4* yp4 = reinterpret_cast<const f32x4*>(a.sh + en * a.sh_stride + g * 8);
                    f32x4* yd = reinterpret_cast<f32x4*>(tile + (16 * t + c) * stride + ycol + g * 8);
                    yd[0] = yp4[0];
                    yd[1] = yp4[1];
                }
#pragma unroll
                for (int mt = 0; mt < MTMAX; ++mt) {
                    if (mt < MT) {
                        const f32x4 zero = {0.f, 0.f, 0.f, 0.f};
                        f32x4 dx = __builtin_amdgcn_mfma_f32_16x16x32_f16(al[mt], bh, zero, 0, 0, 0);
                        f32x4 dh = __builtin_amdgcn_mfma_f32_16x16x32_f16(ah[mt], bh, zero, 0, 0, 0);
                        dx = __builtin_amdgcn_mfma_f32_16x16x32_f16(ah[mt], bl, dx, 0, 0, 0);
                        *reinterpret_cast<f32x4*>(tile + (16 * t + c) * stride + mt * 16 + 4 * g) =
                            dh + SPLIT_LO_INV * dx;
                    }
                }
            }
        }
        __builtin_amdgcn_s_waitcnt(0xc07f);
        __builtin_amdgcn_wave_barrier();
        for (int so = 0; so < CH; ++so) {
            const int s = s0 + so;
            if (s >= maxdeg) break;
            float x[G::D1];
#pragma unroll
            for (int i = 0; i < G::D1; ++i) x[i] = xn[i];
            {
                const float* xp = a.x + (int64_t)src_nn * a.d_in + xcol;
#pragma unroll
                for (int i = 0; i < G::D1; ++i) xn[i] = xp[i];
                src_nn = a.src_sorted[min(beg + s + 2, e_last)];
            }
            if (s < deg) {
                const float* wp = tile + ((j << ch_log2) + so) * stride + u * NC;
                const float* yp = tile + ((j << ch_log2) + so) * stride + ycol + G::Y0;
                float y[G::NY], w[NC];
#pragma unroll
                for (int jj = 0; jj < G::NY; ++jj) y[jj] = yp[jj];
#pragma unroll
                for (int cc = 0; cc < NC; ++cc) w[cc] = wp[cc];
                G::apply(mask, x, y, w, acc);
            }
        }
        __builtin_amdgcn_wave_barrier();
    }
    StoreAgg{}.store<G>(a, ge, acc, a_scale_inv, node, j, u, valid);
}

#define MATTEN_RGS_ARGS a, ge, tile, stage, (um >> 8) & 0xffff, tile_id, r, reps, lane, StoreAgg{}
#define MATTEN_RGS(L1, GI, TT, TD, P) \
    do { \
        using HM = HotMask<L1, GI>; \
        if (HM::M0 && ge.mask == HM::M0) run_group_shared<L1, GI, TT, TD, P, HM::M0>(MATTEN_RGS_ARGS); \
        else if (HM::M1 && ge.mask == HM::M1) run_group_shared<L1, GI, TT, TD, P, HM::M1>(MATTEN_RGS_ARGS); \
        else run_group_shared<L1, GI, TT, TD, P, 0u>(MATTEN_RGS_ARGS); \
    } while (0)
#if defined(MATTEN_LAB) && defined(TPF_ONLY_VARIANT)
#ifndef TPF_ONLY_MASK
#define TPF_ONLY_MASK 0
#endif
#define MATTEN_RGS_ONLY(L1, GI, TT, TD, P) run_group_shared<L1, GI, TT, TD, P, (unsigned)(TPF_ONLY_MASK)>(MATTEN_RGS_ARGS)
#define MATTEN_GROUP_CASE_SHARED(L1, GI) \
    case (L1 * matten::GROUP_KIND_STRIDE + GI): \
        if (TPF_ONLY_VARIANT == 0) MATTEN_RGS_ONLY(L1, GI, 1, (TPF_CHUNK_DEEP && L1 == 0 ? 2 : 0), true); \
        else if (TPF_ONLY_VARIANT == 1) MATTEN_RGS_ONLY(L1, GI, 2, 0, false); \
        else if (TPF_ONLY_VARIANT == 2) MATTEN_RGS_ONLY(L1, GI, 1, (TPF_CHUNK_DEEP && L1 == 0 ? 2 : TwoDeepOk<L1, GI>::value ? 1 : 0), false); \
        else MATTEN_RGS_ONLY(L1, GI, 1, 0, false); \
        break;
#else
#define MATTEN_GROUP_CASE_SHARED(L1, GI) \
    case (L1 * matten::GROUP_KIND_STRIDE + GI): \
        if (paired && TPF_CHUNK_DEEP && L1 == 0 && nodes_per_wave <= 8 && nodes_per_wave >= 4) MATTEN_RGS(L1, GI, 1, (L1 == 0 ? 2 : 0), true); \
        else if (paired) MATTEN_RGS(L1, GI, 1, 0, true); \
        else if (nodes_per_wave > 16) MATTEN_RGS(L1, GI, 2, 0, false); \
        else if (TPF_CHUNK_DEEP && L1 == 0 && nodes_per_wave <= 8 && nodes_per_wave >= 4) MATTEN_RGS(L1, GI, 1, (L1 == 0 ? 2 : 0), false); \
        else if (TwoDeepOk<L1, GI>::value && nodes_per_wave <= 8 && nodes_per_wave >= TPF_TWO_DEEP_MIN_NPW) MATTEN_RGS(L1, GI, 1, (TwoDeepOk<L1, GI>::value ? 1 : 0), false); \
        else MATTEN_RGS(L1, GI, 1, 0, false); \
        break;
#endif

#define MATTEN_GROUP_CASE(L1, GI) \
    case (L1 * matten::GROUP_KIND_STRIDE + GI): run_group<L1, GI>(a, ge, tile, un.node, lane, un.valid, un.beg, un.deg, un.maxdeg); break;

#ifndef TPF_MIN_BLOCKS
#define TPF_MIN_BLOCKS 3
#endif
#ifndef TPF_CHUNK_DEEP
#define TPF_CHUNK_DEEP 1
#endif
#ifndef TPF_TWO_DEEP_MIN_NPW
#define TPF_TWO_DEEP_MIN_NPW 2
#endif
#if defined(MATTEN_LAB) && defined(TPF_ONLY_L1) && defined(TPF_ONLY_GI)
#define TPF_FOR_EACH_GROUP(X) X(TPF_ONLY_L1, TPF_ONLY_GI)
#elif defined(MATTEN_LAB) && defined(TPF_ONLY_LIGHT)
#define TPF_FOR_EACH_GROUP(X) X(0, 0) X(1, 0) X(1, 1)
#elif defined(MATTEN_LAB) && defined(TPF_ONLY_HEAVY)
#define TPF_FOR_EACH_GROUP(X) X(2, 0) X(2, 1) X(3, 0) X(3, 1) X(4, 0) X(4, 1)
#else
#define TPF_FOR_EACH_GROUP(X) MATTEN_FOR_EACH_GROUP(X)
#endif
__global__ __launch_bounds__(WAVES_PER_BLOCK * 64, TPF_MIN_BLOCKS) void tp_fused_kernel(Args a, const GroupEntry* __restrict__ entries,
                                                                        const int* __restrict__ umap,
                                                                        int n_entries, int units_per_tile,
                                                                        int blocks_per_tile, int n_tiles) {
    extern __shared__ __attribute__((aligned(16))) float lds[];
    const int xcd = blockIdx.x % N_XCD;
    const int q = blockIdx.x / N_XCD;
    const int tile_id = (q / blocks_per_tile) * N_XCD + xcd;
    if (tile_id >= n_tiles) return;
    const int wave = __builtin_amdgcn_readfirstlane(threadIdx.x >> 6);
    const int unit = (q % blocks_per_tile) * WAVES_PER_BLOCK + wave;
    if (unit >= units_per_tile) return;
    const int lane = threadIdx.x & 63;
    float* tile = lds + wave * a.lds_per_wave;

    const int um = __builtin_amdgcn_readfirstlane(umap[unit]);
    if (((um >> 8) & 0xffff) >= n_entries) return;
    const GroupEntry& ge = entries[(um >> 8) & 0xffff];
    const int r = um & 255;
    const bool shared_stage = (um >> 24) & 1;
    const int reps = 1 << ((um >> 27) & 3);

    const int cu_log2 = ge.cu_log2;
    const int nodes_per_wave = 64 >> cu_log2;
    if (shared_stage) {
        float* stage = lds + WAVES_PER_BLOCK * a.lds_per_wave;
        const bool paired = (um >> 26) & 1;
        if ((um >> 25) & 1) {
            if (paired) run_loader_only_paired(a, ge, stage, tile_id, r, reps, lane);
            else run_loader_only(a, ge, stage, tile_id, r, reps, lane);
            return;
        }
        switch (ge.kind & (KIND_MERGED - 1)) {
            TPF_FOR_EACH_GROUP(MATTEN_GROUP_CASE_SHARED)
            default: break;
        }
        return;
    }
#if !(defined(MATTEN_LAB) && defined(TPF_ONLY_VARIANT))
    const UnitNodes un = unit_nodes(a, ge, tile_id, r, lane);
    switch (ge.kind & (KIND_MERGED - 1)) {
        TPF_FOR_EACH_GROUP(MATTEN_GROUP_CASE)
        default: break;
    }
#endif
}

constexpr int NT = 4;
__device__ __forceinline__ float silu(float z) {
#if defined(MATTEN_LAB) && defined(RH_ABLATE_NO_SILU)
    return z * 0.5f;
#endif
    return z * __builtin_amdgcn_rcpf(1.0f + __builtin_amdgcn_exp2f(-1.4426950408889634f * z));
}

template <int KS0, int N_MID>
__global__ __launch_bounds__(256) void radial_hidden_kernel(const float4* __restrict__ geom, int64_t E, int n_basis,
                                                            float r_start, float r_end,
                                                            const float* __restrict__ w0p,
                                                            const float* __restrict__ w_mid, _Float16* __restrict__ h2s,
                                                            const float* __restrict__ h_scale) {
    const int lane = threadIdx.x & 63;
    const int wave = threadIdx.x >> 6;
    const int g = lane >> 4, c = lane & 15;
    const int64_t e0 = ((int64_t)blockIdx.x * 4 + wave) * (NT * 16);
    if (e0 >= E) return;
    const float hs = h_scale ? *h_scale : 1.0f;
    const float inv_c = 1.0f / (r_end - r_start);
    const float bes_pref = sqrtf(2.0f * inv_c) * sqrtf((float)n_basis);
    float a1[N_MID > 0 ? N_MID : 1][2][8];
#pragma unroll
    for (int m = 0; m < N_MID; ++m)
#pragma unroll
        for (int kk = 0; kk < 8; ++kk) {
            int k = 16 * (kk >> 2) + 4 * g + (kk & 3);
            a1[m][0][kk] = w_mid[m * HID * HID + k * HID + c];
            a1[m][1][kk] = w_mid[m * HID * HID + k * HID + 16 + c];
        }
    float lens[NT];
#pragma unroll
    for (int nt = 0; nt < NT; ++nt) {
        const int64_t e = e0 + nt * 16 + c;
        lens[nt] = geom[e < E ? e : E - 1].w;
    }
#pragma unroll
    for (int nt = 0; nt < NT; ++nt) {
        const int64_t e = e0 + nt * 16 + c;
        const float len = lens[nt];
        const float xr = len - r_start;
        const float t01 = xr * inv_c, inv_xr = __builtin_amdgcn_rcpf(xr);
        f32x4 h0 = {0.f, 0.f, 0.f, 0.f}, h1 = {0.f, 0.f, 0.f, 0.f};
#pragma unroll
        for (int kk = 0; kk < KS0; ++kk) {
// ... 207 lines not shown
                                const float* h_scale, matten_stream_t stream_) {
    hipStream_t stream = (hipStream_t)stream_;
    if (n_edges < 0 || hidden != HID || (nb_pad & 3) || nb_pad < n_basis || nb_pad > 16 || n_mid < 0 ||
        n_mid > MATTEN_RADIAL_MAX_MID)
        return MATTEN_EINVAL;
    if (n_edges == 0) return MATTEN_OK;
    if (!geom_sorted || !w0p || (n_mid > 0 && !w_mid) || !h2s) return MATTEN_EINVAL;
    unsigned grid = (unsigned)matten_cdiv(n_edges, 4 * NT * 16);
#define LAUNCH(K, M) \
    radial_hidden_kernel<K, M><<<grid, 256, 0, stream>>>((const float4*)geom_sorted, n_edges, n_basis, r_start, r_end, w0p, w_mid, (_Float16*)h2s, h_scale)
#define LAUNCH_M(K)                  \
    switch (n_mid) {                 \
        case 0: LAUNCH(K, 0); break; \
        case 1: LAUNCH(K, 1); break; \
        case 2: LAUNCH(K, 2); break; \
        default: LAUNCH(K, 3); break; \
    }
    switch (nb_pad >> 2) {
        case 1: LAUNCH_M(1); break;
        case 2: LAUNCH_M(2); break;
        case 3: LAUNCH_M(3); break;
        default: LAUNCH_M(4); break;
    }
#undef LAUNCH_M
#undef LAUNCH
    MATTEN_LAUNCH_CHECK();
    return MATTEN_OK;
}

extern "C" int matten_radial_hidden(const float* geom_sorted, int64_t n_edges, int n_basis, float r_start, float r_end,
                                    const float* w0p, int nb_pad, const float* w1p, int hidden, uint16_t* h2s,
                                    const float* h_scale, matten_stream_t stream_) {
    if (!w1p && n_edges > 0) return MATTEN_EINVAL;
    return radial_hidden_launch(geom_sorted, n_edges, n_basis, r_start, r_end, w0p, nb_pad, w1p, 1, hidden, h2s, h_scale,
                                stream_);
}

extern "C" int matten_radial_hidden_deep(const float* geom_sorted, int64_t n_edges, int n_basis, float r_start, float r_end,
                                         const float* w0p, int nb_pad, const float* w_mid, int n_mid, int hidden,
                                         uint16_t* h2s, const float* h_scale, matten_stream_t stream_) {
    return radial_hidden_launch(geom_sorted, n_edges, n_basis, r_start, r_end, w0p, nb_pad, w_mid, n_mid, hidden, h2s,
                                h_scale, stream_);
}

#if TPF_TRACING
static unsigned* g_tp_trace = nullptr;
static int64_t g_tp_trace_waves = 0, g_tp_trace_skip = 0;
extern "C" int matten_lab_tp_trace(unsigned* buf, int64_t n_waves, int64_t skip) {
    g_tp_trace = buf, g_tp_trace_waves = n_waves, g_tp_trace_skip = skip;
    return 0;
}
#endif

extern "C" int matten_tp_fused(const float* x, int64_t d_in, const uint16_t* h2s, const float* w2p, int64_t w_pad,
                               const float* sh_sorted, int64_t sh_stride, const int32_t* rowptr,
                               const int32_t* src_sorted, int64_t n_nodes, const int32_t* group_entries,
                               const int32_t* unit_map, int64_t n_entries, int64_t units_per_tile,
                               int64_t lds_floats_per_wave, int64_t d_mid, float avg_num_neighbors,
                               const float* num_neigh, const uint16_t* a_split, const float* a_scale_inv, float* agg,
                               matten_stream_t stream_) {
    hipStream_t stream = (hipStream_t)stream_;
    if (n_nodes < 0 || d_in <= 0 || w_pad <= 0 || sh_stride < 32 || (sh_stride & 3) || n_entries <= 0 ||
        units_per_tile <= 0 || d_mid <= 0 || lds_floats_per_wave <= 0 || (lds_floats_per_wave & 3))
        return MATTEN_EINVAL;
    if (n_nodes == 0) return MATTEN_OK;
    if (!x || !h2s || !w2p || !sh_sorted || !rowptr || !src_sorted || !group_entries || !unit_map || !agg)
        return MATTEN_EINVAL;
    if (!(avg_num_neighbors > 0.0f) && !num_neigh) return MATTEN_EINVAL;
    const size_t lds = sizeof(float) * ((size_t)lds_floats_per_wave * WAVES_PER_BLOCK + STAGE_TOTAL_FLOATS + PAIR_INFO_INTS);
    if (lds > 64 * 1024) return MATTEN_EINVAL;
    if ((a_split == nullptr) != (a_scale_inv == nullptr)) return MATTEN_EINVAL;
    Args a{x, (const _Float16*)h2s, w2p, (const _Float16*)a_split, a_scale_inv, sh_sorted, rowptr, src_sorted, num_neigh, agg, (int)d_in, (int)w_pad, (int)sh_stride,
           (int)d_mid, (int)n_nodes, (int)lds_floats_per_wave, avg_num_neighbors};
    const int n_tiles = (int)matten_cdiv(n_nodes, TILE_NODES);
    const int blocks_per_tile = (int)matten_cdiv(units_per_tile, WAVES_PER_BLOCK);
    const int64_t grid = matten_cdiv(n_tiles, N_XCD) * N_XCD * (int64_t)blocks_per_tile;
    if (grid >= ((int64_t)1 << 31)) return MATTEN_EINVAL;
#if TPF_TRACING
    a.trace = nullptr;
    if (g_tp_trace && grid * WAVES_PER_BLOCK <= g_tp_trace_waves) {
        if (g_tp_trace_skip <= 0) a.trace = g_tp_trace;
        if (g_tp_trace_skip == 0) g_tp_trace = nullptr;
        if (g_tp_trace_skip > 0) --g_tp_trace_skip;
    }
#endif
    tp_fused_kernel<<<(unsigned)grid, WAVES_PER_BLOCK * 64, lds, stream>>>(
        a, (const GroupEntry*)group_entries, unit_map, (int)n_entries, (int)units_per_tile, blocks_per_tile, n_tiles);
    MATTEN_LAUNCH_CHECK();
    return MATTEN_OK;
}

extern "C" int matten_tp_max_cols(void) { return TPF_MAX_COLS; }
extern "C" int matten_tp_max_cols_l0(void) { return TPF_MAX_COLS_L0; }
extern "C" int matten_tp_max_cols_l1(void) { return TPF_MAX_COLS_L1; }
extern "C" int matten_tp_groups_hash(void) { return matten::GROUPS_HASH; }
```

### matten_amd/csrc/tp_walk.h

```cpp
#pragma once
#include <type_traits>

#include "cg_gen.h"
#include "common.h"
#include "sh.h"

#ifndef MATTEN_LAB
#if defined(MATTEN_ABLATE_NO_GATHER) || defined(MATTEN_ABLATE_NO_XLOAD) || defined(MATTEN_ABLATE_NO_H2LOAD) || \
    defined(MATTEN_ABLATE_NO_MFMA) || defined(MATTEN_ABLATE_NO_VALU) || defined(MATTEN_ABLATE_NO_STORE) ||      \
    defined(MATTEN_ABLATE_NO_BARRIER) || defined(MATTEN_ABLATE_NO_LOOP) || defined(MATTEN_ABLATE_NO_EPI) || defined(MATTEN_ABLATE_ONE_YQUAD)
#error "MATTEN_ABLATE_* switches are honoured by -DMATTEN_LAB builds only (tools/*.sh)"
#endif
#endif
#if defined(MATTEN_LAB) && defined(MATTEN_ABLATE_NO_GATHER)
#define TPF_SRC(v) ((v) >= 0 ? (node < a.n_nodes ? node : 0) : 0)
#else
#define TPF_SRC(v) (v)
#endif
#if defined(MATTEN_LAB) && defined(MATTEN_ABLATE_NO_XLOAD)
#define TPF_XLD(xp, i, v) (1e-9f * (float)((v) + (i)))
#else
#define TPF_XLD(xp, i, v) ((xp)[i])
#endif
#if defined(MATTEN_LAB) && defined(MATTEN_ABLATE_NO_H2LOAD)
// ... 72 lines not shown
#ifndef TPF_SETPRIO
#define TPF_SETPRIO 3
#endif
#ifndef TPF_W_FIRST
#define TPF_W_FIRST 1
#endif
#ifndef TPF_W_FIRST2
#define TPF_W_FIRST2 1
#endif
#ifndef TPF_PAIR_SUM
#define TPF_PAIR_SUM 1
#endif
#ifndef TPF_EXACT_Y0
#define TPF_EXACT_Y0 0
#endif

#ifndef TPF_REP_PREFETCH
#define TPF_REP_PREFETCH 1
#endif
#ifndef TPF_MAX_COLS
#define TPF_MAX_COLS 64
#endif
#ifndef TPF_MAX_COLS_L0
#define TPF_MAX_COLS_L0 96
#endif
#ifndef TPF_MAX_COLS_L1
#define TPF_MAX_COLS_L1 TPF_MAX_COLS
#endif
__host__ __device__ constexpr int cap_channels(int l1, int nc) {
    int cap = 64;
    while (cap > 1 && cap * nc > (l1 == 0 ? TPF_MAX_COLS_L0 : l1 == 1 ? TPF_MAX_COLS_L1 : TPF_MAX_COLS)) cap /= 2;
    return cap;
}
constexpr int TILE_NODES = 64;
constexpr int WAVES_PER_BLOCK = 4;
constexpr int N_XCD = 8;
constexpr int MAXC = matten::GROUP_MAX_COMBOS;
constexpr int HID = 32;

struct GroupEntry {
    int kind;
    int x_off;
    int mul;
    int cu_log2;
    unsigned mask;
    int w_base;
    int a_tile;
    int n_mt;
    int t_off[MAXC];
    int out_off[MAXC];
};
static_assert(sizeof(GroupEntry) == 32 * 4, "GroupEntry layout");

struct Args {
    const float* x;
    const _Float16* h2s;
    const float* w2p;
    const _Float16* a_split;
    const float* a_scale_inv;
    const float* sh;
    const int* rowptr;
    const int* src_sorted;
    const float* num_neigh;
    float* agg;
    int d_in, w_pad, sh_stride, d_mid, n_nodes, lds_per_wave;
    float avg_nn;
#if TPF_TRACING
    unsigned* trace;
#endif
};


struct UnitNodes {
    int node, beg, deg, maxdeg;
    bool valid;
};
struct RawNodes {
    int node, b0, b1;
    bool valid;
};
__device__ __forceinline__ RawNodes unit_nodes_issue(const Args& a, const GroupEntry& ge, int tile_id, int r, int lane) {
    const int cu_log2 = ge.cu_log2;
    const int nodes_per_wave = 64 >> cu_log2;
    const int g_in_tile = r * nodes_per_wave + (lane >> cu_log2);
    const int u = lane & ((1 << cu_log2) - 1);
    RawNodes n;
    n.node = tile_id * TILE_NODES + g_in_tile;
    const bool in_range = (g_in_tile < TILE_NODES) && (n.node < a.n_nodes);
    n.valid = in_range && (u < ge.mul);
    n.b0 = 0, n.b1 = 0;
    if (in_range) {
        n.b0 = a.rowptr[n.node];
        n.b1 = a.rowptr[n.node + 1];
    }
    return n;
}
__device__ __forceinline__ UnitNodes unit_nodes_finish(const RawNodes& raw) {
    UnitNodes n;
    n.node = raw.node, n.valid = raw.valid, n.beg = raw.b0, n.deg = raw.b1 - raw.b0;
    int maxdeg = n.deg;
#pragma unroll
    for (int off = 32; off > 0; off >>= 1) maxdeg = max(maxdeg, __shfl_xor(maxdeg, off));
    if constexpr (TPF_LAB_NO_LOOP) maxdeg = 0;
    n.maxdeg = maxdeg;
    return n;
}
__device__ __forceinline__ UnitNodes unit_nodes(const Args& a, const GroupEntry& ge, int tile_id, int r, int lane) {
    return unit_nodes_finish(unit_nodes_issue(a, ge, tile_id, r, lane));
}

constexpr int STAGE_ROW = 68;
constexpr int STAGE_TMAX = 2;
constexpr int STAGE_FLOATS = 16 * STAGE_TMAX * STAGE_ROW;
constexpr int STAGE_TOTAL_FLOATS = 2 * STAGE_FLOATS;

template <int MTC>
__device__ __forceinline__ void mfma_tiles(const f16x8* __restrict__ ah, const f16x8* __restrict__ al, f16x8 bh, f16x8 bl,
                                           float* __restrict__ trow) {
    const f32x4 zero = {0.f, 0.f, 0.f, 0.f};
    f32x4 dx[MTC], dh[MTC];
#pragma unroll
    for (int mt = 0; mt < MTC; ++mt) {
        dx[mt] = __builtin_amdgcn_mfma_f32_16x16x32_f16(al[mt], bh, zero, 0, 0, 0);
        dh[mt] = __builtin_amdgcn_mfma_f32_16x16x32_f16(ah[mt], bh, zero, 0, 0, 0);
    }
#pragma unroll
    for (int mt = 0; mt < MTC; ++mt) dx[mt] = __builtin_amdgcn_mfma_f32_16x16x32_f16(ah[mt], bl, dx[mt], 0, 0, 0);
#pragma unroll
    for (int mt = 0; mt < MTC; ++mt) *reinterpret_cast<f32x4*>(trow + mt * 16) = dh[mt] + SPLIT_LO_INV * dx[mt];
}



template <int TT>
struct StageLoader {
    const char* base;
    const char* safe;
    int64_t row_bytes;
    float* st_w;
    int beg_ld[TT], deg_ld[TT], so_ld[TT];
    int CH;
    f32x4 pf[TT];

    __device__ __forceinline__ void init(const Args& a, float* stage, int cu_log2, int beg, int deg_node) {
        const int npw = 64 >> cu_log2;
        const int ch_log2 = npw >= 16 ? 0 : 4 - (6 - cu_log2);
        CH = 1 << ch_log2;
        const int piece = threadIdx.x & 15;
        base = piece < 8 ? reinterpret_cast<const char*>(a.h2s) + piece * 16
                         : reinterpret_cast<const char*>(a.sh) + (piece - 8) * 16;
        row_bytes = piece < 8 ? (int64_t)(2 * HID * sizeof(_Float16)) : (int64_t)a.sh_stride * 4;
        safe = reinterpret_cast<const char*>(a.w2p);
        st_w = stage + (threadIdx.x >> 4) * STAGE_ROW + piece * 4;
#pragma unroll
        for (int t = 0; t < TT; ++t) {
            const int n = (int)(threadIdx.x >> 4) + 16 * t;
            const int jn = (n >> ch_log2) & (npw - 1);
            so_ld[t] = n & (CH - 1);
            beg_ld[t] = __shfl(beg, jn << cu_log2);
            deg_ld[t] = __shfl(deg_node, jn << cu_log2);
            pf[t] = f32x4{0.f, 0.f, 0.f, 0.f};
// ... 16 lines not shown
constexpr int PAIR_INFO_INTS = 2 * 16 * 2 + 2;
struct PairLoader {
    const char* base;
    const char* safe;
    int64_t row_bytes;
    float* st_w;
    int beg_ld[2], deg_ld[2], so_ld;
    int CH, maxdeg;
    f32x4 pf[2];

    __device__ __forceinline__ void init(const Args& a, float* stage, int* info, int cu_log2, int beg, int deg_node,
                                         int my_maxdeg) {
        const int npw = 64 >> cu_log2;
        const int ch_log2 = 4 - (6 - cu_log2);
        CH = 1 << ch_log2;
        const int wave = threadIdx.x >> 6, lane = threadIdx.x & 63;
        if ((wave & 1) == 0 && (lane & ((1 << cu_log2) - 1)) == 0) {
            info[((wave >> 1) * 16 + (lane >> cu_log2)) * 2] = beg;
            info[((wave >> 1) * 16 + (lane >> cu_log2)) * 2 + 1] = deg_node;
            if (lane == 0) info[2 * 16 * 2 + (wave >> 1)] = my_maxdeg;
        }
        __syncthreads();
        maxdeg = max(info[2 * 16 * 2], info[2 * 16 * 2 + 1]);
        const int piece = threadIdx.x & 15;
        base = piece < 8 ? reinterpret_cast<const char*>(a.h2s) + piece * 16
                         : reinterpret_cast<const char*>(a.sh) + (piece - 8) * 16;
        row_bytes = piece < 8 ? (int64_t)(2 * HID * sizeof(_Float16)) : (int64_t)a.sh_stride * 4;
        safe = reinterpret_cast<const char*>(a.w2p);
        const int n = (int)(threadIdx.x >> 4);
        st_w = stage + n * STAGE_ROW + piece * 4;
        const int jn = (n >> ch_log2) & (npw - 1);
        so_ld = n & (CH - 1);
#pragma unroll
        for (int t = 0; t < 2; ++t) {
            beg_ld[t] = info[(t * 16 + jn) * 2];
            deg_ld[t] = info[(t * 16 + jn) * 2 + 1];
            pf[t] = f32x4{0.f, 0.f, 0.f, 0.f};
        }
    }
    __device__ __forceinline__ void issue(int s0) {
#pragma unroll
        for (int t = 0; t < 2; ++t)
            pf[t] = *reinterpret_cast<const f32x4*>(
                deg_ld[t] > 0 ? base + (int64_t)(beg_ld[t] + min(s0 + so_ld, deg_ld[t] - 1)) * row_bytes : safe);
    }
    __device__ __forceinline__ void publish(int buf) {
#pragma unroll
        for (int t = 0; t < 2; ++t)
            *reinterpret_cast<f32x4*>(st_w + buf * (32 * STAGE_ROW) + 16 * t * STAGE_ROW) = pf[t];
    }
};

__device__ __forceinline__ void run_loader_only_paired(const Args& a, const GroupEntry& ge, float* __restrict__ stage,
                                                       int tile_id, int r0, int reps, int lane) {
    for (int rep = 0; rep < reps; ++rep) {
        const UnitNodes un = unit_nodes(a, ge, tile_id, r0 + 2 * rep, lane);
        PairLoader ld;
        ld.init(a, stage, reinterpret_cast<int*>(stage + STAGE_TOTAL_FLOATS), ge.cu_log2, un.beg, un.deg, un.maxdeg);
        ld.issue(0);
        ld.publish(0);
        __syncthreads();
        int buf = 0;
        for (int s0 = 0; s0 < ld.maxdeg; s0 += ld.CH, buf ^= 1) {
            ld.issue(s0 + ld.CH);
            ld.publish(buf ^ 1);
            __syncthreads();
        }
    }
}

template <int TT>
__device__ __forceinline__ void run_loader_only_t(const Args& a, const GroupEntry& ge, float* __restrict__ stage, int tile_id,
                                                  int r0, int reps, int lane) {
    for (int rep = 0; rep < reps; ++rep) {
        const UnitNodes un = unit_nodes(a, ge, tile_id, r0 + rep, lane);
        StageLoader<TT> ld;
        ld.init(a, stage, ge.cu_log2, un.beg, un.deg);
        ld.issue(0);
        ld.publish(0);
        __syncthreads();
        int buf = 0;
        for (int s0 = 0; s0 < un.maxdeg; s0 += ld.CH, buf ^= 1) {
            ld.issue(s0 + ld.CH);
            ld.publish(buf ^ 1);
            __syncthreads();
        }
    }
}
__device__ __forceinline__ void run_loader_only(const Args& a, const GroupEntry& ge, float* __restrict__ stage, int tile_id,
                                                int r0, int reps, int lane) {
    if ((64 >> ge.cu_log2) > 16) run_loader_only_t<2>(a, ge, stage, tile_id, r0, reps, lane);
    else run_loader_only_t<1>(a, ge, stage, tile_id, r0, reps, lane);
}

template <int L1, int GI>
struct TwoDeepOk { static constexpr bool value = L1 == 0 || (L1 == 1 && (GI == 0 || TPF_PAIR_SUM)); };

template <int L1, int GI, int TT, int TWO_DEEP, bool PAIRED, unsigned CMASK, class Epilogue>
__device__ __forceinline__ void run_group_shared(const Args& a, const GroupEntry& ge, float* __restrict__ tile,
                                                 float* __restrict__ stage, int entry, int tile_id, int r0, int reps, int lane,
                                                 const Epilogue& epi) {
    static_assert(!PAIRED || TT == 1, "paired workgroups stage 2 x 16 rows");
#if TPF_TRACING
    const unsigned tr_in_hi = tpf_stamp_hi();
    const unsigned tr_in = tpf_stamp();
    unsigned tr_mfma = 0, tr_con = 0, tr_pub = 0, tr_bar = 0, tr_chunks = 0, tr_pro = 0, tr_epi = 0;
    unsigned tr_pro_pre = 0, tr_epi_sg = 0;
#endif
    const int row0 = PAIRED ? 16 * (int)(threadIdx.x >> 7) : 0;
    constexpr int STAGE_BUF = (PAIRED ? 32 : 16 * TT) * STAGE_ROW;
    using G = matten::Group<L1, GI>;
    constexpr int NC = G::NC;

    const unsigned mask = ge.mask;
    const int cu_log2 = ge.cu_log2;
    const int cu = 1 << cu_log2;
    const int npw = 64 >> cu_log2;
    const int ch_log2 = npw >= 16 ? 0 : 4 - (6 - cu_log2);
    const int CH = 1 << ch_log2;
    const int ncols = ge.mul * NC;
#if defined(MATTEN_LAB) && defined(TPF_ONLY_MT)
    const int MT = TPF_ONLY_MT;
#else
    const int MT = (ncols + 15) >> 4;
#endif

    const int j = lane >> cu_log2;
    const int u = lane & (cu - 1);
    const int g = lane >> 4, c = lane & 15;
    const int xcol = ge.x_off + u * G::D1;
    constexpr int CAPC = cap_channels(L1, NC);
    constexpr int MTMAX = (CAPC * NC + 15) / 16;
    const int stride = MT * 16 + 4;
    f16x8 ah[MTMAX], al[MTMAX];
    float a_scale_inv;
    if (a.a_split) {
        const f16x8* ap = reinterpret_cast<const f16x8*>(a.a_split) + ((int64_t)ge.a_tile * 64 + lane) * 2;
#pragma unroll
        for (int mt = 0; mt < MTMAX; ++mt) {
            const f16x8 z = {0, 0, 0, 0, 0, 0, 0, 0};
            ah[mt] = mt < MT ? ap[mt * 128] : z;
            al[mt] = mt < MT ? ap[mt * 128 + 1] : z;
        }
        a_scale_inv = a.a_scale_inv[entry];
    } else
    {
        float av[MTMAX][8];
        float amax = 0.0f;
#pragma unroll
        for (int mt = 0; mt < MTMAX; ++mt) {
#pragma unroll
            for (int kk = 0; kk < 8; ++kk) {
                const int k = 16 * (kk >> 2) + 4 * g + (kk & 3);
                av[mt][kk] = (mt < MT) ? a.w2p[(int64_t)k * a.w_pad + ge.w_base + mt * 16 + c] : 0.0f;
                amax = fmaxf(amax, fabsf(av[mt][kk]));
            }
        }
#pragma unroll
        for (int off = 32; off > 0; off >>= 1) amax = fmaxf(amax, __shfl_xor(amax, off));
        int e = (int)((__float_as_uint(amax) >> 23) & 0xffu) - 127;
        e = amax > 0.0f ? max(-100, min(100, e)) : 13;
        const float a_scale = __uint_as_float((unsigned)(127 + 13 - e) << 23);
        a_scale_inv = __uint_as_float((unsigned)(127 - 13 + e) << 23);
#pragma unroll
        for (int mt = 0; mt < MTMAX; ++mt) {
#pragma unroll
            for (int kk = 0; kk < 8; ++kk) {
                _Float16 hi, lo;
                split_f16(av[mt][kk] * a_scale, hi, lo);
                ah[mt][kk] = hi;
                al[mt][kk] = lo;
            }
        }
    }

    typename std::conditional<PAIRED, PairLoader, StageLoader<TT>>::type ld;
    static_assert(!TWO_DEEP || TwoDeepOk<L1, GI>::value, "two rows in flight only for the light kinds");
    static_assert(TWO_DEEP != 2 || G::D1 == 1, "a chunk of rows in flight: scalar input blocks");
    constexpr bool two_deep = TWO_DEEP == 1;
    constexpr bool chunk_deep = TWO_DEEP == 2;
    constexpr int XQ = 4;
    float xqa[XQ], xqb[XQ];
    int sq[XQ];
    int node, beg, deg, maxdeg, e_last;
    bool valid;
    float xn[G::D1], xb[G::D1];
    int src_nn, src_b = 0;
    auto start_group = [&](const UnitNodes& un) {
        node = un.node, beg = un.beg, valid = un.valid, maxdeg = un.maxdeg;
        deg = valid ? un.deg : 0;
        if constexpr (PAIRED) {
            ld.init(a, stage, reinterpret_cast<int*>(stage + STAGE_TOTAL_FLOATS), cu_log2, un.beg, un.deg, un.maxdeg);
            maxdeg = ld.maxdeg;
        } else {
            ld.init(a, stage, cu_log2, un.beg, un.deg);
        }
        ld.issue(0);
        e_last = deg > 0 ? beg + deg - 1 : 0;
        if constexpr (chunk_deep) {
            int s0q[XQ];
#pragma unroll
            for (int i = 0; i < XQ; ++i) s0q[i] = a.src_sorted[min(beg + i, e_last)];
#pragma unroll
            for (int i = 0; i < XQ; ++i) sq[i] = a.src_sorted[min(beg + CH + i, e_last)];
#pragma unroll
            for (int i = 0; i < XQ; ++i) {
                const float* xp = a.x + (int64_t)TPF_SRC(s0q[i]) * a.d_in + xcol;
                xqa[i] = TPF_XLD(xp, 0, s0q[i]);
            }
            return;
        }
        const int src0 = a.src_sorted[min(beg, e_last)];
        const int src1 = a.src_sorted[min(beg + 1, e_last)];
        const float* xp0 = a.x + (int64_t)src0 * a.d_in + xcol;
#pragma unroll
        for (int i = 0; i < G::D1; ++i) xn[i] = xp0[i];
        src_nn = src1;
        if (two_deep) {
            const float* xp1 = a.x + (int64_t)src1 * a.d_in + xcol;
#pragma unroll
            for (int i = 0; i < G::D1; ++i) xb[i] = xp1[i];
            src_nn = a.src_sorted[min(beg + 2, e_last)];
            src_b = a.src_sorted[min(beg + 3, e_last)];
        }
    };
    constexpr int RSTEP = PAIRED ? 2 : 1;
    start_group(unit_nodes(a, ge, tile_id, r0, lane));
    for (int rep = 0; rep < reps; ++rep) {
#if TPF_TRACING
    const unsigned tr_rep = rep == 0 ? tr_in : tpf_stamp();
#endif
    const bool more = rep + 1 < reps;
    const RawNodes raw_next = unit_nodes_issue(a, ge, tile_id, r0 + RSTEP * (rep + (more ? 1 : 0)), lane);
    float acc[G::NACC];
#pragma unroll
    for (int k = 0; k < G::NACC; ++k) acc[k] = 0.0f;
    ld.publish(0);
#if TPF_TRACING
    tr_pro_pre += (unsigned)(tpf_stamp() - tr_rep);
#endif
    __syncthreads();
#if TPF_TRACING
    const unsigned tr_loop = tpf_stamp();
    unsigned tr_a = tr_loop;
    tr_pro += (unsigned)(tr_loop - tr_rep);
#endif
    auto chunk_body = [&](const int s0, const int buf, float (&xcur)[XQ], float (&xnext)[XQ]) {
        __builtin_amdgcn_s_setprio(TPF_SETPRIO);
        ld.issue(s0 + CH);
        const float* sb = stage + buf * STAGE_BUF + row0 * STAGE_ROW;
#pragma unroll
        for (int t = 0; t < TT; ++t) {
            {
                const f16x8 bh = *reinterpret_cast<const f16x8*>(sb + (16 * t + c) * STAGE_ROW + g * 4);
                const f16x8 bl = *reinterpret_cast<const f16x8*>(sb + (16 * t + c) * STAGE_ROW + 16 + g * 4);
                if constexpr (TPF_LAB_NO_MFMA) {
                    if ((float)bh[0] == 12345.f) tile[c] = (float)bl[0];
                    continue;
                }
                float* trow = tile + (16 * t + c) * stride + 4 * g;
                if (MTMAX == 1 || MT == 1) mfma_tiles<1>(ah, al, bh, bl, trow);
                else if (MTMAX == 2 || MT == 2) mfma_tiles<(MTMAX < 2 ? MTMAX : 2)>(ah, al, bh, bl, trow);
                else if (MTMAX == 3 || MT == 3) mfma_tiles<(MTMAX < 3 ? MTMAX : 3)>(ah, al, bh, bl, trow);
                else if (MTMAX == 4 || MT == 4) mfma_tiles<(MTMAX < 4 ? MTMAX : 4)>(ah, al, bh, bl, trow);
                else if (MTMAX == 5 || MT == 5) mfma_tiles<(MTMAX < 5 ? MTMAX : 5)>(ah, al, bh, bl, trow);
                else if (MTMAX == 6 || MT == 6) mfma_tiles<(MTMAX < 6 ? MTMAX : 6)>(ah, al, bh, bl, trow);
                else mfma_tiles<MTMAX>(ah, al, bh, bl, trow);
            }
        }
        __builtin_amdgcn_s_waitcnt(0xc07f);
        __builtin_amdgcn_wave_barrier();
        __builtin_amdgcn_s_setprio(0);
#if TPF_TRACING
        const unsigned tr_b = tpf_stamp();
#endif
        auto contract = [&](int so, const float* __restrict__ x) {
            const float* wp = tile + ((j << ch_log2) + so) * stride + u * NC;
            const float* yp = sb + ((j << ch_log2) + so) * STAGE_ROW + 32 + G::Y0;
            float y[G::NY], w[NC];
            if constexpr (TPF_W_FIRST) {
#pragma unroll
                for (int cc = 0; cc < NC; ++cc) w[cc] = wp[cc];
                asm volatile("" ::: "memory");
            }
            if constexpr (TPF_EXACT_Y0 && L1 == 0 && G::Y0 == 0 && G::NY % 4 == 1) {
                y[G::NY - 1] = yp[G::NY - 1];
// ... 102 lines not shown
                    src_b = a.src_sorted[min(beg + s + 5, e_last)];
                }
            }
        } else {
            for (int so = 0; so < CH; ++so) {
                const int s = s0 + so;
                if (s >= maxdeg) break;
                float x[G::D1];
#pragma unroll
                for (int i = 0; i < G::D1; ++i) x[i] = xn[i];
                {
                    const float* xp = a.x + (int64_t)TPF_SRC(src_nn) * a.d_in + xcol;
#pragma unroll
                    for (int i = 0; i < G::D1; ++i) xn[i] = TPF_XLD(xp, i, src_nn);
                    src_nn = a.src_sorted[min(beg + s + 2, e_last)];
                }
                if (s < deg) contract(so, x);
            }
        }
#if TPF_TRACING
        const unsigned tr_c = tpf_stamp_after(acc);
#endif
        ld.publish(buf ^ 1);
#if TPF_TRACING
        const unsigned tr_d = tpf_stamp();
#endif
        if constexpr (TPF_LAB_NO_BARRIER) {
            __builtin_amdgcn_s_waitcnt(0xc07f);
            __builtin_amdgcn_wave_barrier();
        } else {
            __syncthreads();
        }
#if TPF_TRACING
        const unsigned tr_e = tpf_stamp();
        tr_mfma += (unsigned)(tr_b - tr_a), tr_con += (unsigned)(tr_c - tr_b), tr_pub += (unsigned)(tr_d - tr_c);
        tr_bar += (unsigned)(tr_e - tr_d), tr_chunks += 1;
        tr_a = tr_e;
#endif
    };
    if constexpr (chunk_deep) {
        for (int s0 = 0; s0 < maxdeg; s0 += 2 * CH) {
            chunk_body(s0, 0, xqa, xqb);
            if (s0 + CH < maxdeg) chunk_body(s0 + CH, 1, xqb, xqa);
        }
    } else {
        int buf = 0;
        for (int s0 = 0; s0 < maxdeg; s0 += CH, buf ^= 1) chunk_body(s0, buf, xqa, xqb);
    }
#if TPF_TRACING
    const unsigned tr_end = tpf_stamp();
#endif
    const int node_done = node;
    const bool valid_done = valid;
    if (TPF_REP_PREFETCH && more) start_group(unit_nodes_finish(raw_next));
#if TPF_TRACING
    tr_epi_sg += (unsigned)(tpf_stamp() - tr_end);
#endif
    epi.template store<G>(a, ge, acc, a_scale_inv, node_done, j, u, valid_done);
    if (!TPF_REP_PREFETCH && more) start_group(unit_nodes_finish(raw_next));
#if TPF_TRACING
    if (a.trace && lane == 0) {
        if (rep + 1 == reps) asm volatile("s_waitcnt vmcnt(0)" ::: "memory");
        const unsigned tr_out = tpf_stamp();
        tr_epi += (unsigned)(tr_out - tr_end);
        if (rep + 1 == reps) {
            unsigned* tr = a.trace + ((size_t)blockIdx.x * WAVES_PER_BLOCK + (threadIdx.x >> 6)) * 16;
            tr[0] = 1u, tr[1] = (unsigned)ge.kind, tr[2] = (unsigned)cu_log2 | (PAIRED ? 256u : 0u) | ((unsigned)reps << 9) | ((unsigned)TT << 12) | ((unsigned)MT << 16);
            tr[3] = tr_chunks, tr[4] = tr_pro, tr[5] = tr_mfma, tr[6] = tr_con, tr[7] = tr_pub, tr[8] = tr_bar;
            tr[9] = tr_epi, tr[10] = (unsigned)(tr_out - tr_in), tr[11] = (unsigned)ge.mask;
            tr[12] = tr_in, tr[13] = tr_in_hi, tr[14] = tr_pro_pre, tr[15] = tr_epi_sg;
        }
    }
#endif
    }
}

template <int L1, int GI> struct HotMask { static constexpr unsigned M0 = 0, M1 = 0; };
#ifndef TPF_NO_HOT_MASKS
template <> struct HotMask<0, 0> { static constexpr unsigned M0 = 0x1f, M1 = 0xf; };
#endif
#ifndef TPF_HOT_ALL
#define TPF_HOT_ALL 1
#endif
#if TPF_HOT_ALL
template <> struct HotMask<1, 0> { static constexpr unsigned M0 = 0x7f, M1 = 0; };
template <> struct HotMask<1, 1> { static constexpr unsigned M0 = 0x1b, M1 = 0xf; };
template <> struct HotMask<2, 0> { static constexpr unsigned M0 = 0x7ff, M1 = 0x6ff; };
template <> struct HotMask<2, 1> { static constexpr unsigned M0 = 0x1d, M1 = 0xf; };
template <> struct HotMask<3, 0> { static constexpr unsigned M0 = 0x3ff, M1 = 0x37f; };
template <> struct HotMask<3, 1> { static constexpr unsigned M0 = 0x7f, M1 = 0x3f; };
template <> struct HotMask<4, 0> { static constexpr unsigned M0 = 0xfb, M1 = 0; };
template <> struct HotMask<4, 1> { static constexpr unsigned M0 = 0x7d, M1 = 0; };
#endif
#ifndef TPF_HOT_ALT
#define TPF_HOT_ALT 1
#endif
#if TPF_HOT_ALT
template <> struct HotMask<0, 1> { static constexpr unsigned M0 = 0x7, M1 = 0; };
template <> struct HotMask<1, 4> { static constexpr unsigned M0 = 0x3f, M1 = 0; };
template <> struct HotMask<2, 4> { static constexpr unsigned M0 = 0x3f, M1 = 0; };
template <> struct HotMask<1, 2> { static constexpr unsigned M0 = 0xf, M1 = 0; };
template <> struct HotMask<1, 3> { static constexpr unsigned M0 = 0x3, M1 = 0; };
template <> struct HotMask<2, 2> { static constexpr unsigned M0 = 0x7, M1 = 0; };
template <> struct HotMask<2, 3> { static constexpr unsigned M0 = 0x3f, M1 = 0; };
template <> struct HotMask<3, 2> { static constexpr unsigned M0 = 0x1f, M1 = 0; };
template <> struct HotMask<3, 3> { static constexpr unsigned M0 = 0xf, M1 = 0; };
template <> struct HotMask<4, 2> { static constexpr unsigned M0 = 0x7, M1 = 0; };
template <> struct HotMask<4, 3> { static constexpr unsigned M0 = 0x3f, M1 = 0; };
#endif

}
```

### matten_amd/nn/_nequip.py

```python
from typing import Union

import torch

from .. import ops
from ..data.irreps import DataKey, ModuleIrreps
from ..o3 import Irreps


def with_batch(data: DataKey.Type) -> DataKey.Type:
    if DataKey.BATCH not in data:
        pos = data[DataKey.POSITIONS]
        data[DataKey.BATCH] = torch.zeros(len(pos), dtype=torch.long, device=pos.device)
    return data


def ensure_graph(data: DataKey.Type, err=None) -> DataKey.Type:
    if DataKey.AMD_ROWPTR not in data:
        n_nodes = data[DataKey.POSITIONS].shape[0]
        perm, rowptr, src, err = ops.csr_build(data[DataKey.EDGE_INDEX], n_nodes, err=err)
        data[DataKey.AMD_PERM], data[DataKey.AMD_ROWPTR], data[DataKey.AMD_SRC] = perm, rowptr, src
        data["_amd_csr_err"] = err
    return data


def ensure_edge_geometry(data: DataKey.Type, lmax: int = None, want_vectors=False, want_lengths=False,
                         want_attrs=False, want_embedding=False) -> DataKey.Type:
    have = DataKey.AMD_GEOM in data
    missing = (
        (want_vectors and DataKey.EDGE_VECTORS not in data)
        or (want_lengths and DataKey.EDGE_LENGTH not in data)
        or (want_attrs and DataKey.EDGE_ATTRS not in data)
        or (want_embedding and DataKey.EDGE_EMBEDDING not in data)
    )
    if have and not missing:
        return data
    ensure_graph(data)
    if lmax is None:
        lmax = int(data["_amd_lmax"]) if "_amd_lmax" in data else 0
    data["_amd_lmax"] = lmax
    nb, r0, r1 = 0, 0.0, 1.0
    if DataKey.AMD_RBF in data:
        nb, r0, r1 = data[DataKey.AMD_RBF].tolist()
        nb = int(nb)
    out = ops.edge_geom(
        data[DataKey.POSITIONS], data[DataKey.EDGE_INDEX], data.get(DataKey.EDGE_CELL_SHIFT),
        data.get(DataKey.CELL), data.get(DataKey.BATCH), data[DataKey.AMD_PERM], lmax, nb, r0, r1,
        want_vectors=want_vectors, want_lengths=want_lengths, want_attrs=want_attrs,
        want_embedding=want_embedding and nb > 0,
    )
    data[DataKey.AMD_GEOM], data[DataKey.AMD_SH] = out["geom_sorted"], out["sh_sorted"]
    for key, name in ((DataKey.EDGE_VECTORS, "edge_vectors"), (DataKey.EDGE_LENGTH, "edge_lengths"),
                      (DataKey.EDGE_ATTRS, "edge_attrs"), (DataKey.EDGE_EMBEDDING, "edge_embedding")):
        if out[name] is not None:
            data[key] = out[name]
    return data


def ensure_training_edge_tensors(data: DataKey.Type) -> DataKey.Type:
    if "_amd_dst_sorted" not in data:
        ensure_edge_geometry(data)
        perm = data[DataKey.AMD_PERM].long()
        data["_amd_dst_sorted"] = data[DataKey.EDGE_INDEX][1][perm].to(torch.int32).contiguous()
        src = data[DataKey.AMD_SRC].long()
        pairs = torch.stack([src, src])
        out_perm, out_ptr, _, _ = ops.csr_build(pairs, int(data[DataKey.POSITIONS].shape[0]))
        data["_amd_out_csr"] = (out_ptr, out_perm)
    return data


def with_edge_vectors(data: DataKey.Type, with_lengths: bool = True) -> DataKey.Type:
    return ensure_edge_geometry(data, want_vectors=True, want_lengths=with_lengths)

# ... 34 lines not shown
```

### matten_amd/nn/utils.py

```python
import os
from typing import Callable, Dict, List, Optional

import numpy as np
import torch
from torch import Tensor

from .. import autograd as _ag
from .. import ops, plan as _plan
from ..data.irreps import DataKey, ModuleIrreps
from ..o3 import Irrep, Irreps
from ._activation import act_const_table, normalize2mom_const
from ._tables import DerivedWeight, DeviceTables

ACTIVATION = {"e": {"ssp": "ssp", "silu": "silu", "sigmoid": "sigmoid"}, "o": {"abs": "abs", "tanh": "tanh"}}

tp_path_exists = _plan.tp_path_exists


def _inverse_permutation(gather):
    import numpy as np

    g = np.asarray(gather).reshape(-1)
    assert g.size == 0 or (np.sort(g) == np.arange(g.size)).all(), "packed weight table is not a permutation"
    inv = np.empty_like(g)
# ... 241 lines not shown
            bw_blocks=self.plan.bw_blocks, bw_paths=self.plan.bw_paths, bw_w_entries=self.plan.bw_w_entries,
            fused_cols=self.plan.fused_cols,
        )

        self._a_split = DerivedWeight(self._split_last_layer)
        self._a_split_c = None

    def _split_last_layer(self, *ws: Tensor):
        w2p = self.weight_nn._packed.get(*ws)[2]
        frag, scale_inv = ops.split_a_tiles(w2p, self.plan.group_entries)
        return frag, (scale_inv * self.weight_nn._h_scale.get(*ws[:-1])[1]).contiguous()

    def a_split(self, r_start: float, r_end: float):
        mlp = self.weight_nn
        mlp.h_scale(r_start, r_end)
        c = float(r_end - r_start)
        if c != self._a_split_c:
            self._a_split_c = c
            self._a_split._key = None
        return self._a_split.get(*mlp.weights())

    @property
    def irreps_out(self) -> Irreps:
        return self.irreps_mid.simplify()

    def forward(self, node_feats: Tensor, data: DataKey.Type, avg_num_neighbors=None, out_layout=None) -> Tensor:
        nb, r0, r1 = data[DataKey.AMD_RBF].tolist()
        dev = node_feats.device
        avg = avg_num_neighbors if avg_num_neighbors is not None else 0.0
        num_neigh = None if avg_num_neighbors is not None else data[DataKey.NUM_NEIGH]
        if _ag.needs_grad_lazy(lambda: (node_feats, *_ag.params_of(self.weight_nn))):
            from ._nequip import ensure_training_edge_tensors

            ensure_training_edge_tensors(data)
            mode = os.environ.get("MATTEN_TRAIN_TP", "auto")
            n_edges = data[DataKey.AMD_SRC].shape[0]
            if mode == "auto":
                if self._train_tp_auto is None:
                    self._train_tp_auto = "fused" if n_edges >= TRAIN_FUSED_MIN_EDGES else "paths"
                mode = self._train_tp_auto
            if self.impl == "fused" and mode == "fused":
                return _ag.FusedTensorProductFn.apply(node_feats, self, data, avg, num_neigh, *self.weight_nn.weights())
            w_edge = self.weight_nn.forward_train(data[DataKey.AMD_GEOM], int(nb), r0, r1)
            return _ag.TensorProductScatterFn.apply(node_feats, w_edge, self, data, avg, num_neigh)
        if self.impl == "fused":
            h2p, w2p = self.weight_nn.hidden(data[DataKey.AMD_GEOM], int(nb), r0, r1, data)
            rowptr = data[DataKey.AMD_ROWPTR]
            split = None
            piece = hub_split_len(node_feats.shape[0])
            if out_layout is None and piece > 0 and node_feats.shape[0] < HUB_SPLIT_MAX_ROWS:
                key = ("_amd_csr_split", piece, num_neigh is None)
                split = data.get(key)
                if split is None or split[3] is not rowptr:
                    split = ops.csr_split(rowptr, data[DataKey.AMD_SRC].shape[0], piece, num_neigh) + (rowptr,)
                    data[key] = split
            agg = ops.tp_fused(
                node_feats, h2p, w2p, data[DataKey.AMD_SH], rowptr if split is None else split[0], data[DataKey.AMD_SRC],
                out_layout[0] if out_layout is not None else self._tables.get("gentries", dev),
                self._tables.get("gumap", dev), len(self.plan.fused_unit_map),
                self.plan.fused_lds_floats_per_wave, out_layout[1] if out_layout is not None else self.plan.d_mid, avg,
                num_neigh if split is None else split[2], a_split=self.a_split(r0, r1),
            )
            return agg if split is None else ops.segment_reduce(agg, split[1], mean=False)
        w_edge = self.weight_nn(data[DataKey.AMD_GEOM], int(nb), r0, r1)
        return ops.tp_paths(
            node_feats, w_edge, data[DataKey.AMD_SH], data[DataKey.AMD_ROWPTR], data[DataKey.AMD_SRC],
            self._tables.get("entries", dev), self._tables.get("unit_start", dev), self.plan.units_per_tile,
            self.plan.d_mid, avg, num_neigh,
        )


class ActivationLayer(torch.nn.Module):
    def __init__(
        self,
        tp_irreps_in1: Irreps,
        tp_irreps_in2: Irreps,
        tp_irreps_out: Irreps,
        *,
        activation_type: str = "gate",
        activation_scalars: Dict[str, str] = None,
        activation_gates: Dict[str, str] = None,
    ):
        super().__init__()
        key = {"e": 1, "o": -1}
        scal = {1: "ssp", -1: "tanh"} if activation_scalars is None else {
            key[k]: ACTIVATION[k][v] for k, v in activation_scalars.items()
        }
        gat = {1: "ssp", -1: "abs"} if activation_gates is None else {
            key[k]: ACTIVATION[k][v] for k, v in activation_gates.items()
        }
        self.activation_type = activation_type
        if activation_type == "norm":
            self.plan = _plan.plan_norm_act(tp_irreps_in1, tp_irreps_in2, tp_irreps_out, scal)
            self._tables = DeviceTables(chan=self.plan.chan)
            return
        if activation_type != "gate":
            supported = ("gate", "norm")
            raise ValueError(f"Support `activation_type` includes {supported}, got {activation_type}")
        self.plan = _plan.plan_gate(tp_irreps_in1, tp_irreps_in2, tp_irreps_out, scal, gat)
        self._tables = DeviceTables(meta=self.plan.meta, act_cst=act_const_table().numpy())

    @property
    def irreps_in(self) -> Irreps:
        return self.plan.irreps_in

    @property
    def irreps_out(self) -> Irreps:
        return self.plan.irreps_out

    def _forward_norm_act(self, x: Tensor, norm, data) -> Tensor:
        dev = x.device
        bn = norm.n if (norm is not None and norm.method == "batch") else None
        if _ag.needs_grad(x) or (bn is not None and bn.training) or (norm is not None and norm.method == "instance"):
            y = _ag.NormActFn.apply(x, self) if _ag.needs_grad(x) else ops.norm_act(
# ... 112 lines not shown
```

### matten_amd/ops.py

```python
from __future__ import annotations

from typing import Optional, Tuple

import os

import numpy as np

import torch

from . import _lib
from .nn._tables import bump_weights_epoch


_EVENTS = None
_EVENTS_ONLY = None


def enable_event_timing(flag: bool = True, only=None) -> None:
    global _EVENTS, _EVENTS_ONLY
    _EVENTS = {} if flag else None
    _EVENTS_ONLY = tuple(only) if (flag and only) else None


def event_timings_ms():
# ... 14 lines not shown
        return self

    def __exit__(self, *exc):
        if self.on and _EVENTS is not None:
            b = torch.cuda.Event(enable_timing=True)
            b.record(torch.cuda.current_stream())
            _EVENTS.setdefault(self.name, []).append((self.a, b))
        return False


SH_STRIDE = 32


def _ptr(t: Optional[torch.Tensor]):
    return None if t is None else t.data_ptr()


_raw_stream = getattr(torch._C, "_cuda_getCurrentRawStream", None)


def _stream() -> int:
    if _raw_stream is not None:
        return _raw_stream(torch.cuda.current_device())
    return torch.cuda.current_stream().cuda_stream


def _need(t: torch.Tensor, dtype, name: str) -> torch.Tensor:
    if not isinstance(t, torch.Tensor):
        raise TypeError(f"{name}: expected a tensor, got {type(t)}")
    if not t.is_cuda:
        raise _lib.MattenHipError(
            f"{name} is on {t.device}: matten_amd runs on MI355X only (no CPU fallback). Move the batch to cuda."
        )
    if t.dtype != dtype:
        raise TypeError(f"{name}: expected dtype {dtype}, got {t.dtype}")
    return t if t.is_contiguous() else t.contiguous()


def _need_rows(t: torch.Tensor, dtype, name: str) -> torch.Tensor:
    if isinstance(t, torch.Tensor) and t.dim() == 2 and t.stride(1) == 1 and t.stride(0) >= t.shape[1] and t.is_cuda \
            and t.dtype == dtype:
        return t
    return _need(t, dtype, name)


def _err_flag(err, dev) -> torch.Tensor:
    if err is None:
        return torch.zeros(1, dtype=torch.int32, device=dev)
    if err.dtype != torch.int32 or err.numel() != 1 or err.device != dev:
        raise ValueError("err must be an int32 tensor of one element on the inputs' device")
    return err


def csr_build(edge_index: torch.Tensor, n_nodes: int, err: torch.Tensor = None) -> Tuple[torch.Tensor, torch.Tensor, torch.Tensor, torch.Tensor]:
    lib = _lib.load()
    edge_index = _need(edge_index, torch.int64, "edge_index")
    E = edge_index.shape[1]
    dev = edge_index.device
    perm = torch.empty(E, dtype=torch.int32, device=dev)
    rowptr = torch.empty(n_nodes + 1, dtype=torch.int32, device=dev)
    src = torch.empty(E, dtype=torch.int32, device=dev)
    err = _err_flag(err, dev)
    nbytes = lib.matten_csr_workspace_bytes(E, n_nodes)
    ws = torch.empty(max(nbytes, 1), dtype=torch.uint8, device=dev)
    _lib.check(
        lib.matten_csr_build(_ptr(edge_index), E, n_nodes, _ptr(perm), _ptr(rowptr), _ptr(src), _ptr(ws), nbytes,
                             _ptr(err), _stream()),
        "matten_csr_build",
    )
    return perm, rowptr, src, err


def csr_split(rowptr: torch.Tensor, n_edges: int, max_len: int, num_neigh: torch.Tensor = None):
    lib = _lib.load()
    rowptr = _need(rowptr, torch.int32, "rowptr")
    N = rowptr.shape[0] - 1
    bound = int(lib.matten_csr_split_bound(N, n_edges, max_len))
    dev = rowptr.device
    vrowptr = torch.empty(bound + 1, dtype=torch.int32, device=dev)
    vseg = torch.empty(N + 1, dtype=torch.int64, device=dev)
    vnn = None
    if num_neigh is not None:
        num_neigh = _need(num_neigh, torch.float32, "num_neigh")
        vnn = torch.empty(bound, dtype=torch.float32, device=dev)
    _lib.check(lib.matten_csr_split(_ptr(rowptr), N, n_edges, max_len, _ptr(vrowptr), _ptr(vseg), _ptr(num_neigh), _ptr(vnn),
                                    _stream()), "matten_csr_split")
    return vrowptr, vseg, vnn


def group_by_key(key: torch.Tensor, n_keys: int, err: torch.Tensor = None) -> Tuple[torch.Tensor, torch.Tensor, torch.Tensor]:
    lib = _lib.load()
    key = _need(key, torch.int64, "key")
    n = key.shape[0]
    dev = key.device
    order = torch.empty(n, dtype=torch.int32, device=dev)
    seg = torch.empty(n_keys + 1, dtype=torch.int32, device=dev)
    err = _err_flag(err, dev)
    nbytes = lib.matten_group_workspace_bytes(n, n_keys)
    ws = torch.empty(max(nbytes, 1), dtype=torch.uint8, device=dev)
    _lib.check(lib.matten_group_by_key(_ptr(key), n, n_keys, _ptr(order), _ptr(seg), _ptr(ws), nbytes, _ptr(err),
                                       _stream()), "matten_group_by_key")
    return order, seg, err


def species_embed(atomic_numbers, z_to_index, min_z: int, max_z: int, n_species: int, weight, bias,
                  want_attrs: bool = False, err: torch.Tensor = None):
    lib = _lib.load()
    Z = _need(atomic_numbers, torch.int64, "atomic_numbers")
    lut = _need(z_to_index, torch.int64, "_Z_to_index")
    W = _need(weight, torch.float32, "linear.weight")
    b = _need(bias, torch.float32, "linear.bias")
    N, dim = Z.shape[0], W.shape[0]
    dev = Z.device
    sidx = torch.empty(N, dtype=torch.int64, device=dev)
    s32 = torch.empty(N, dtype=torch.int32, device=dev)
    feats = torch.empty(N, dim, dtype=torch.float32, device=dev)
    attrs = torch.empty(N, n_species, dtype=torch.float32, device=dev) if want_attrs else None
    err = _err_flag(err, dev)
    _lib.check(
        lib.matten_species_embed(_ptr(Z), N, _ptr(lut), min_z, max_z, n_species, _ptr(W), _ptr(b), dim, _ptr(sidx),
                                 _ptr(s32), _ptr(feats), _ptr(attrs), _ptr(err), _stream()),
        "matten_species_embed",
    )
    return sidx, s32, feats, attrs, err


def edge_geom(pos, edge_index, edge_cell_shift, cell, batch, perm, lmax: int, n_basis: int = 0, r_start: float = 0.0,
              r_end: float = 1.0, want_vectors=False, want_lengths=False, want_attrs=False, want_embedding=False):
    lib = _lib.load()
    pos = _need(pos, torch.float32, "pos")
    edge_index = _need(edge_index, torch.int64, "edge_index")
    E = edge_index.shape[1]
    dev = pos.device
    n_cells = 0
    if cell is not None:
        cell = _need(cell, torch.float32, "cell").reshape(-1, 3, 3)
        n_cells = cell.shape[0]
        edge_cell_shift = _need(edge_cell_shift, torch.float32, "edge_cell_shift")
        if n_cells > 1:
# ... 339 lines not shown
    geom_sorted = _need(geom_sorted, torch.float32, "geom_sorted")
    w0ps = [_need(w, torch.float32, "w0p") for w in w0ps]
    mids = [_mid(w, "w_mid") for w in w_mids]
    L, E = len(w0ps), geom_sorted.shape[0]
    if not 1 <= L <= 8 or len(mids) != L or any(w.shape != w0ps[0].shape for w in w0ps) or \
            any(m[1] != mids[0][1] for m in mids):
        raise ValueError("radial_hidden_multi_deep: 1..8 layers with equal basis / hidden sizes and depth")
    n_mid = mids[0][1]
    out = [torch.empty(E, 2, 32, dtype=torch.float16, device=geom_sorted.device) for _ in range(L)]
    arr = lambda ts: (ctypes.c_void_p * L)(*[t.data_ptr() for t in ts])
    if h_scales is not None:
        h_scales = [_need(h, torch.float32, "h_scale") for h in h_scales]
        if len(h_scales) != L:
            raise ValueError("one h_scale per layer")
    with _timed("radial_hidden_multi"):
        rc = lib.matten_radial_hidden_multi_deep(_ptr(geom_sorted), E, n_basis, r_start, r_end, arr(w0ps), w0ps[0].shape[0],
                                                 arr([m[0] for m in mids]) if n_mid else None, n_mid, w0ps[0].shape[1],
                                                 arr(out), arr(h_scales) if h_scales is not None else None, L, _stream())
    _lib.check(rc, "matten_radial_hidden_multi_deep")
    return out


def split_a_tiles(w2p: torch.Tensor, group_entries) -> Tuple[torch.Tensor, torch.Tensor]:
    dev = w2p.device
    g = torch.arange(4, device=dev)[:, None]
    kk = torch.arange(8, device=dev)[None, :]
    k_idx = 16 * (kk >> 2) + 4 * g + (kk & 3)
    tiny = 2.0 ** -14
    tiles, inv = [], []
    for row in np.asarray(group_entries).reshape(-1, 32):
        w_base, n_mt = int(row[5]), int(row[7])
        if int(row[0]) < 0 or n_mt == 0:
            inv.append(torch.ones((), device=dev))
            continue
        A = w2p[k_idx][:, :, w_base:w_base + 16 * n_mt]
        A = A.reshape(4, 8, n_mt, 16).permute(2, 0, 3, 1)
        amax = A.abs().max()
        e = torch.where(amax > 0, (torch.frexp(amax)[1] - 1).clamp(-100, 100), torch.full_like(amax, 13, dtype=torch.int32))
        scale = torch.ldexp(torch.ones_like(amax), 13 - e)
        inv.append(torch.ldexp(torch.ones_like(amax), e - 13))
        v = A * scale
        hi = torch.where(v.abs() < tiny, torch.zeros_like(v), v.half().float())
        lo = (v - hi) * 2048.0
        lo = torch.where(lo.abs() < tiny, torch.zeros_like(lo), lo)
        tiles.append(torch.cat([hi.half(), lo.half()], dim=-1).reshape(n_mt, 64, 16))
    return torch.cat(tiles).contiguous(), torch.stack(inv).float().contiguous()


_GROUPS_CHECKED = False


def tp_fused(x, h2p, w2p, sh_sorted, rowptr, src_sorted, entries, unit_map, units_per_tile: int,
             lds_floats_per_wave: int, d_mid: int, avg_num_neighbors: float, num_neigh=None,
             a_split=None) -> torch.Tensor:
    lib = _lib.load()
    from .plan import TP_TILE_NODES

    if lib.matten_tp_tile_nodes() != TP_TILE_NODES:
        raise _lib.MattenHipError("plan.TP_TILE_NODES does not match the library's node tile")
    from .plan import TP_MAX_COLS, TP_MAX_COLS_L0, TP_MAX_COLS_L1
    if (lib.matten_tp_max_cols() != TP_MAX_COLS or lib.matten_tp_max_cols_l0() != TP_MAX_COLS_L0
            or lib.matten_tp_max_cols_l1() != TP_MAX_COLS_L1):
        raise _lib.MattenHipError("plan.TP_MAX_COLS does not match the library's entry width (-DTPF_MAX_COLS)")
    global _GROUPS_CHECKED
    from .plan import tp_groups_hash
    if not _GROUPS_CHECKED and lib.matten_tp_groups_hash() != tp_groups_hash():
        raise _lib.MattenHipError("the library's coupling code (cg_gen.h) was generated for other coupling groups than plan.TP_GROUPS "
                                  "(MATTEN_TP_GROUPS / an interrupted tools/*.sh A/B build?): make -C matten_amd/csrc clean all")
    _GROUPS_CHECKED = True
    x = _need_rows(x, torch.float32, "node_features")
    h2p = _need(h2p, torch.float16, "h2s")
    if h2p.dim() != 3 or h2p.shape[1:] != (2, 32):
        raise ValueError(f"h2s must be [E,2,32] fp16 (ops.split_hidden / ops.radial_hidden), got {tuple(h2p.shape)}")
    w2p = _need(w2p, torch.float32, "w2p")
    sh_sorted = _need(sh_sorted, torch.float32, "sh_sorted")
    N, d_in = rowptr.shape[0] - 1, x.stride(0)
    if num_neigh is not None:
        num_neigh = _need(num_neigh, torch.float32, "num_neigh")
    if a_split is not None:
        a_split = (_need(a_split[0], torch.float16, "a_split"), _need(a_split[1], torch.float32, "a_scale_inv"))
        if a_split[1].numel() != entries.shape[0]:
            raise ValueError("a_scale_inv needs one value per group entry")
    if unit_map.numel() != units_per_tile:
        raise ValueError(f"unit_map has {unit_map.numel()} units, expected {units_per_tile} (plan.fused_unit_map)")
    agg = torch.empty(N, d_mid, dtype=torch.float32, device=x.device)
    with _timed(f"tp_scatter/d_mid={d_mid}/d_in={x.shape[1]}"):
        rc = lib.matten_tp_fused(_ptr(x), d_in, _ptr(h2p), _ptr(w2p), w2p.shape[1], _ptr(sh_sorted),
                                 sh_sorted.shape[1], _ptr(rowptr), _ptr(src_sorted), N, _ptr(entries),
                                 _ptr(unit_map), entries.shape[0], units_per_tile, lds_floats_per_wave, d_mid,
                                 float(avg_num_neighbors or 0.0), _ptr(num_neigh),
                                 _ptr(a_split[0]) if a_split is not None else None,
                                 _ptr(a_split[1]) if a_split is not None else None, _ptr(agg), _stream())
    _lib.check(rc, "matten_tp_fused")
    return agg


def agg_linear(agg, species_order, wtab, io_table, blocks, d_out: int, add=None) -> torch.Tensor:
    lib = _lib.load()
    from .plan import AGG_BLOCK, AGG_MAX_MT
    if lib.matten_agg_linear_block_chunks() != AGG_BLOCK or lib.matten_agg_linear_max_mt() != AGG_MAX_MT:
        raise _lib.MattenHipError("plan.AGG_BLOCK / AGG_MAX_MT do not match the library (-DAL_BLK_CHUNKS)")
    agg = _need(agg, torch.float32, "agg")
    wtab = _need(wtab, torch.float32, "A fragments")
    n_rows, ld = agg.shape
    order, seg = species_order if species_order is not None else (None, None)
    n_species = wtab.shape[0] if wtab.dim() == 2 else 1
    if add is not None:
        add = _need_rows(add, torch.float32, "add")
    out = torch.empty(n_rows, d_out, dtype=torch.float32, device=agg.device)
    with _timed(f"agg_linear/ld={ld}"):
        rc = lib.matten_agg_linear(_ptr(agg), ld, _ptr(order), _ptr(seg), n_species, _ptr(wtab), wtab.shape[-1],
                                   _ptr(io_table), io_table.shape[0], _ptr(blocks), blocks.shape[0], _ptr(add),
                                   add.stride(0) if add is not None else d_out, d_out, n_rows, _ptr(out), _stream())
    _lib.check(rc, "matten_agg_linear")
    return out


def agg_linear_gate(agg, species_order, wtab, io_table, blocks, d_out: int, cmeta, act_cst, d_act: int, add=None,
                    bn_scale=None, bn_shift=None) -> torch.Tensor:
    lib = _lib.load()
    from .plan import AGG_BLOCK, AGG_GATE_SETS, AGG_MAX_MT
    if (lib.matten_agg_linear_block_chunks() != AGG_BLOCK or lib.matten_agg_linear_max_mt() != AGG_MAX_MT
            or lib.matten_agg_linear_gate_sets() != AGG_GATE_SETS):
        raise _lib.MattenHipError("plan.AGG_BLOCK / AGG_MAX_MT / AGG_GATE_SETS do not match the library")
    agg = _need(agg, torch.float32, "agg")
    wtab = _need(wtab, torch.float32, "A fragments")
    n_rows, ld = agg.shape
    order, seg = species_order if species_order is not None else (None, None)
    n_species = wtab.shape[0] if wtab.dim() == 2 else 1
    if add is not None:
        add = _need_rows(add, torch.float32, "add")
    if cmeta.shape != (d_out, 4):
        raise ValueError("cmeta must be [d_out, 4]")
    if bn_scale is not None:
        bn_scale, bn_shift = _need(bn_scale, torch.float32, "bn_scale"), _need(bn_shift, torch.float32, "bn_shift")
        if bn_scale.numel() != d_act or bn_shift.numel() != d_act:
            raise ValueError("bn_scale / bn_shift must have one value per activated column")
    out = torch.empty(n_rows, d_act, dtype=torch.float32, device=agg.device)
    with _timed(f"agg_linear/ld={ld}"):
        rc = lib.matten_agg_linear_gate(_ptr(agg), ld, _ptr(order), _ptr(seg), n_species, _ptr(wtab), wtab.shape[-1],
                                        _ptr(io_table), io_table.shape[0], _ptr(blocks), blocks.shape[0], _ptr(add),
                                        add.stride(0) if add is not None else d_out, d_out, n_rows, _ptr(cmeta),
                                        _ptr(act_cst), _ptr(bn_scale), _ptr(bn_shift), d_act, _ptr(out), _stream())
    _lib.check(rc, "matten_agg_linear_gate")
    return out
# ... 306 lines not shown
    _lib.check(lib.matten_segment_reduce_bwd(_ptr(dy), dy.shape[1], _ptr(ptr), dy.shape[0], int(mean), _ptr(dx),
                                             _stream()), "matten_segment_reduce_bwd")
    return dx


def graph_prep(pos64, cell64, ptr, r_cut: float):
    lib = _lib.load()
    pos64 = _need(pos64, torch.float64, "pos")
    cell64 = _need(cell64, torch.float64, "cell")
    ptr = _need(ptr, torch.int64, "ptr")
    N, B, dev = pos64.shape[0], ptr.shape[0] - 1, pos64.device
    frac = torch.empty(N, 3, dtype=torch.float64, device=dev)
    bound = torch.empty(B, 3, dtype=torch.float64, device=dev)
    batch = torch.empty(N, dtype=torch.int64, device=dev)
    pos32 = torch.empty(N, 3, dtype=torch.float32, device=dev)
    cell32 = torch.empty(3 * B, 3, dtype=torch.float32, device=dev)
    _lib.check(lib.matten_graph_prep(_ptr(pos64), _ptr(cell64), _ptr(ptr), B, float(r_cut), _ptr(frac), _ptr(bound),
                                     _ptr(batch), _ptr(pos32), _ptr(cell32), _stream()), "matten_graph_prep")
    return frac, bound, batch, pos32, cell32


def neighbor_list(pos64, cell64, ptr, frac, bound, pair_ptr, r_cut: float, max_atoms: int, n_pairs: int, want_csr: bool = True):
    lib = _lib.load()
    pos64 = _need(pos64, torch.float64, "pos")
    cell64 = _need(cell64, torch.float64, "cell")
    ptr = _need(ptr, torch.int64, "ptr")
    frac = _need(frac, torch.float64, "frac")
    bound = _need(bound, torch.float64, "bound")
    pair_ptr = _need(pair_ptr, torch.int64, "pair_ptr")
    B = ptr.shape[0] - 1
    N = pos64.shape[0]
    dev = pos64.device
    counts = torch.empty((2 if want_csr else 1) * n_pairs, dtype=torch.int32, device=dev)
    with _timed("neighbor_count"):
        _lib.check(
            lib.matten_neighbor_count(_ptr(pos64), _ptr(cell64), _ptr(ptr), _ptr(frac), _ptr(bound), _ptr(pair_ptr),
                                      float(r_cut), B, int(max_atoms), _ptr(counts),
                                      counts.data_ptr() + 4 * n_pairs if (want_csr and n_pairs) else None, _stream()),
            "matten_neighbor_count",
        )
    scan = torch.zeros(counts.numel() + 1, dtype=torch.int64, device=dev)
    torch.cumsum(counts, 0, dtype=torch.int64, out=scan[1:])
    offsets = scan[: n_pairs + 1]
    if n_pairs:
        summary = torch.empty(2, dtype=torch.int64, device=dev)
        _lib.check(lib.matten_neighbor_summary(_ptr(offsets), _ptr(pair_ptr), B, _ptr(summary), _stream()),
                   "matten_neighbor_summary")
        E, min_edges = summary.tolist()
    else:
        E, min_edges = 0, 0
    edge_index = torch.empty(2, E, dtype=torch.int64, device=dev)
    shifts = torch.empty(E, 3, dtype=torch.float32, device=dev)
    num_neigh = torch.empty(N, dtype=torch.float32, device=dev)
    csr = offsets_t = None
    if want_csr and n_pairs and E < 2 ** 31:
        offsets_t = scan[n_pairs:]
        csr = (torch.empty(E, dtype=torch.int32, device=dev), torch.empty(N + 1, dtype=torch.int32, device=dev),
               torch.empty(E, dtype=torch.int32, device=dev))
    with _timed("neighbor_fill"):
        _lib.check(
            lib.matten_neighbor_fill(_ptr(pos64), _ptr(cell64), _ptr(ptr), _ptr(frac), _ptr(bound), _ptr(pair_ptr),
                                     float(r_cut), B, int(max_atoms), _ptr(offsets), E, _ptr(edge_index), _ptr(shifts),
                                     _ptr(num_neigh), _ptr(offsets_t), N, _ptr(csr[1]) if csr else None,
                                     _ptr(csr[2]) if csr else None, _ptr(csr[0]) if csr else None, _stream()),
            "matten_neighbor_fill",
        )
    return edge_index, shifts, num_neigh, offsets, int(min_edges), csr
```

### matten_amd/plan.py

```python
from __future__ import annotations

import math
import os
from dataclasses import dataclass, field
from typing import Dict, List, Optional, Sequence, Tuple

import numpy as np

from .o3 import Irrep, Irreps, wigner_3j

TP_TILE_NODES = 64

def _range_groups(ranges, l1, lmax=4):
    return [[(l2, l3) for l2 in range(lo, hi + 1) for l3 in range(abs(l1 - l2), min(lmax, l1 + l2) + 1)] for lo, hi in ranges]


def _moved(l1, to_first, lmax=4):
    g0, g1 = _range_groups([(0, 2), (3, 4)], l1, lmax)
    assert all(c in g1 for c in to_first)
    return [g0 + list(to_first), [c for c in g1 if c not in to_first]]


_GROUP_SCHEMES = {
    "A": {l1: _range_groups([(0, 4)] if l1 == 0 else [(0, 2), (3, 4)], l1) for l1 in range(5)},
# ... 8 lines not shown
    0: [[(0, 0), (1, 1), (2, 2)]],
    1: [[(1, 0), (1, 2), (3, 2), (3, 4)], [(2, 2), (4, 4)], [(0, 1), (1, 0), (1, 1), (1, 2), (2, 1), (2, 2)]],
    2: [[(1, 2), (3, 2), (3, 4)], [(0, 2), (2, 0), (2, 2), (2, 4), (4, 2), (4, 4)],
        [(0, 2), (1, 1), (1, 2), (2, 0), (2, 1), (2, 2)]],
    3: [[(1, 2), (1, 4), (3, 0), (3, 2), (3, 4)], [(2, 2), (2, 4), (4, 2), (4, 4)]],
    4: [[(1, 4), (3, 2), (3, 4)], [(0, 4), (2, 2), (2, 4), (4, 0), (4, 2), (4, 4)]],
}
TP_ALT_GROUPS = os.environ.get("MATTEN_TP_ALT_GROUPS", "1") != "0"
TP_GROUPS_REGULAR = {l1: len(g) for l1, g in _GROUP_SCHEMES[TP_GROUPS_SCHEME].items()}
TP_GROUPS = {l1: list(g) + (_ALT_GROUPS.get(l1, []) if TP_GROUPS_SCHEME == "D" else [])
             for l1, g in _GROUP_SCHEMES[TP_GROUPS_SCHEME].items()}


def tp_groups_hash() -> int:
    global _TP_GROUPS_HASH
    if _TP_GROUPS_HASH is None:
        h = 0x811C9DC5
        for b in repr(sorted((l1, [list(map(tuple, g)) for g in gs]) for l1, gs in TP_GROUPS.items())).encode():
            h = ((h ^ b) * 0x01000193) & 0xFFFFFFFF
        _TP_GROUPS_HASH = h & 0x7FFFFFFF
    return _TP_GROUPS_HASH


_TP_GROUPS_HASH = None


def groups_for_block(l1: int, couplings) -> list:
    n_reg = TP_GROUPS_REGULAR[l1]
    couplings = set(couplings)
    if TP_ALT_GROUPS and couplings:
        cover = [gi for gi in range(n_reg, len(TP_GROUPS[l1])) if couplings <= set(TP_GROUPS[l1][gi])]
        if cover:
            gi = min(cover, key=lambda g: (len(TP_GROUPS[l1][g]), g))
            return [(gi, TP_GROUPS[l1][gi])]
    return list(enumerate(TP_GROUPS[l1][:n_reg]))
TP_MAX_COMBOS = 12
TP_MAX_COLS = int(os.environ.get("MATTEN_TP_MAX_COLS", "64"))
TP_MAX_COLS_L0 = int(os.environ.get("MATTEN_TP_MAX_COLS_L0", "96"))
TP_MAX_COLS_L1 = int(os.environ.get("MATTEN_TP_MAX_COLS_L1", str(TP_MAX_COLS)))
TP_KIND_STRIDE = 8

ACT_CODE = {None: 0, "silu": 1, "tanh": 2, "sigmoid": 3, "ssp": 4, "abs": 5}


LIGHT_LMAX = 1

TP_KIND_MERGED = 256
TP_MERGE = os.environ.get("MATTEN_TP_MERGE", "1") != "0"

FUSED_UNIT_SHARED = 1 << 24
FUSED_UNIT_LOADER_ONLY = 1 << 25
FUSED_UNIT_PAIRED = 1 << 26
FUSED_UNIT_REPS_SHIFT = 27


def fused_persist(cu_log2: int, groups: int, mode: str) -> int:
    spec = os.environ.get("MATTEN_TP_PERSIST", TP_PERSIST_DEFAULT)
    want = 1
    for item in filter(None, spec.split(",")):
        lanes, reps = item.split(":")
        if int(lanes) == (1 << cu_log2):
            want = int(reps)
    avail = groups // 2 if mode == "paired" else groups
    reps = 1
    while reps * 2 <= min(want, 8) and avail % (reps * 2) == 0:
        reps *= 2
    return reps


TP_PERSIST_DEFAULT = "16:4,8:2"


def fused_workgroups(group_entries, order: Optional[str] = None):
    order = order or os.environ.get("MATTEN_FUSED_UNIT_ORDER", "node")
    ent = np.asarray(group_entries).reshape(-1, 32)
    out = []
    classes: Dict[int, List[int]] = {}
    for e in range(len(ent)):
        if int(ent[e][0]) < 0:
            continue
        classes.setdefault(int(ent[e][3]), []).append(e)
    for cu_log2, members in classes.items():
        npw = max(1, 64 >> cu_log2)
        run = sorted(members, key=lambda e: int(ent[e][0]) & (TP_KIND_MERGED - 1))
        if order != "node" or cu_log2 < 1:
            out.append((cu_log2, run, "plain"))
        elif npw <= 16 and os.environ.get("MATTEN_FUSED_PAIRED", "1") != "0":
            n4 = len(run) // 4 * 4
            for k in range(0, n4, 4):
                out.append((cu_log2, run[k:k + 4], "shared"))
            rest = run[n4:]
            if len(rest) == 3:
                out.append((cu_log2, rest, "shared"))
            elif rest:
                out.append((cu_log2, rest, "paired"))
        else:
            nblk = -(-len(run) // 4)
            cuts = [round(k * len(run) / nblk) for k in range(nblk + 1)]
            for k in range(nblk):
                out.append((cu_log2, run[cuts[k]:cuts[k + 1]], "shared"))
    return out


def fused_unit_map(group_entries, order: Optional[str] = None) -> np.ndarray:
    ent = np.asarray(group_entries).reshape(-1, 32)
    assert len(ent) < 65536
    shared_units: List[int] = []
    plain_units: List[int] = []
    for cu_log2, blk, mode in fused_workgroups(ent, order):
        groups = -(-TP_TILE_NODES // max(1, 64 >> cu_log2))
        assert groups < 256
        reps = fused_persist(cu_log2, groups, mode) if mode in ("shared", "paired") else 1
        rbits = (reps.bit_length() - 1) << FUSED_UNIT_REPS_SHIFT
        if mode == "shared":
            for r in range(0, groups, reps):
                shared_units += [FUSED_UNIT_SHARED | rbits | (e << 8) | r for e in blk]
                shared_units += [FUSED_UNIT_SHARED | FUSED_UNIT_LOADER_ONLY | rbits | (blk[-1] << 8) | r] * (4 - len(blk))
        elif mode == "paired":
            assert groups % 2 == 0 and 1 <= len(blk) <= 2
            flags = FUSED_UNIT_SHARED | FUSED_UNIT_PAIRED | rbits
            for r in range(0, groups, 2 * reps):
                for rr in (r, r + 1):
                    shared_units += [flags | (e << 8) | rr for e in blk]
                    shared_units += [flags | FUSED_UNIT_LOADER_ONLY | (blk[-1] << 8) | rr] * (2 - len(blk))
        else:
            plain_units += [(e << 8) | r for e in blk for r in range(groups)]
    return np.array(shared_units + plain_units, dtype=np.int64).astype(np.int32)


def tp_path_exists(irreps_in1, irreps_in2, ir_out) -> bool:
    ir_out = Irrep(ir_out)
    for _, ir1 in Irreps(irreps_in1).simplify():
        for _, ir2 in Irreps(irreps_in2).simplify():
            if ir_out in ir1 * ir2:
                return True
    return False


@dataclass
class UVUPath:
    i_in1: int
    i_sh: int
    l1: int
    l2: int
    l3: int
    p3: int
    mul: int
    x_off: int
    w_off: int
    slot: int
    out_off: int
    m_off: int


@dataclass
class UVUPlan:
    irreps_in1: Irreps
    irreps_sh: Irreps
    irreps_mid: Irreps
    irreps_out: Irreps
    paths: List[UVUPath]
    weight_numel: int
    d_in: int
    d_mid: int
    sh_dim: int
    m_total: int
    m_nterms: int
    m_terms_idx: np.ndarray
    m_terms_coef: np.ndarray
    out_meta: np.ndarray
    cg_nnz: int = 0
    path_entries: np.ndarray = None
    unit_start: np.ndarray = None
    units_per_tile: int = 0
    group_entries: np.ndarray = None
    group_unit_start: np.ndarray = None
    group_units_per_tile: int = 0
    fused_cols: np.ndarray = None
    fused_lds_floats_per_wave: int = 0
# ... 727 lines not shown
```

Before: 1.266 billion edge-TP/s.

## Precompute per-node walk records to feed fused tensor-product kernel

Adds a packed int4 per-node record (row start, degree, first two source indices), built during CSR construction, neighbor fill, or split, and passes it to a new fused TP kernel entry point. The aim is to replace several dependent loads of rowptr and src_sorted at the start of each node's edge walk with one 16-byte load, shortening the latency chain. Unit words also gain a lanes-per-node field so the kernel can decode the lane layout from the unit itself. The cost is extra memory, extra writes during graph construction, and a new kernel path that must stay consistent with the CSR.

```diff
diff --git a/include/matten_hip.h b/include/matten_hip.h
--- a/include/matten_hip.h
+++ b/include/matten_hip.h
@@ -25,9 +25,18 @@
                      int32_t* rowptr, int32_t* src_sorted, void* workspace, size_t workspace_bytes,
                      int32_t* err_flag, matten_stream_t stream);
 
+int matten_walk_records(const int32_t* rowptr, const int32_t* src_sorted, int64_t n_nodes, int32_t* walk,
+                        matten_stream_t stream);
+int matten_csr_build_walk(const int64_t* edge_index, int64_t n_edges, int64_t n_nodes, int32_t* perm,
+                          int32_t* rowptr, int32_t* src_sorted, int32_t* walk, void* workspace,
+                          size_t workspace_bytes, int32_t* err_flag, matten_stream_t stream);
+
 int64_t matten_csr_split_bound(int64_t n_nodes, int64_t n_edges, int64_t max_len);
 int matten_csr_split(const int32_t* rowptr, int64_t n_nodes, int64_t n_edges, int64_t max_len, int32_t* vrowptr,
                      int64_t* vseg, const float* num_neigh, float* vnn, matten_stream_t stream);
+int matten_csr_split_walk(const int32_t* rowptr, int64_t n_nodes, int64_t n_edges, int64_t max_len, int32_t* vrowptr,
+                          int64_t* vseg, const float* num_neigh, float* vnn, const int32_t* src_sorted,
+                          int32_t* vwalk, matten_stream_t stream);
 
 size_t matten_group_workspace_bytes(int64_t n, int64_t n_keys);
 int matten_group_by_key(const int64_t* key, int64_t n, int64_t n_keys, int32_t* order, int32_t* seg,
@@ -92,6 +101,12 @@
                     int64_t units_per_tile, int64_t lds_floats_per_wave, int64_t d_mid, float avg_num_neighbors,
                     const float* num_neigh, const uint16_t* a_split, const float* a_scale_inv,
                     float* agg , matten_stream_t stream);
+int matten_tp_fused_walk(const float* x, int64_t d_in, const uint16_t* h2s, const float* w2p, int64_t w_pad,
+                         const float* sh_sorted, int64_t sh_stride, const int32_t* rowptr, const int32_t* src_sorted,
+                         const int32_t* walk, int64_t n_nodes, const int32_t* group_entries, const int32_t* unit_map,
+                         int64_t n_entries, int64_t units_per_tile, int64_t lds_floats_per_wave, int64_t d_mid,
+                         float avg_num_neighbors, const float* num_neigh, const uint16_t* a_split,
+                         const float* a_scale_inv, float* agg , matten_stream_t stream);
 
 int matten_tp_max_cols(void);
 int matten_tp_max_cols_l0(void);
@@ -232,6 +247,12 @@
                          int64_t max_atoms, const int64_t* offsets, int64_t n_edges, int64_t* edge_index,
                          float* edge_cell_shift, float* num_neigh, const int64_t* offsets_t, int64_t n_atoms,
                          int32_t* rowptr, int32_t* src_sorted, int32_t* perm, matten_stream_t stream);
+int matten_neighbor_fill_walk(const double* pos, const double* cell, const int64_t* ptr, const double* frac,
+                              const double* bound, const int64_t* pair_ptr, double r_cut, int64_t n_crystals,
+                              int64_t max_atoms, const int64_t* offsets, int64_t n_edges, int64_t* edge_index,
+                              float* edge_cell_shift, float* num_neigh, const int64_t* offsets_t, int64_t n_atoms,
+                              int32_t* rowptr, int32_t* src_sorted, int32_t* perm, int32_t* walk,
+                              matten_stream_t stream);
 
 #ifdef __cplusplus
 }
diff --git a/matten_amd/_lib.py b/matten_amd/_lib.py
--- a/matten_amd/_lib.py
+++ b/matten_amd/_lib.py
@@ -7,7 +7,7 @@
 _HERE = os.path.dirname(os.path.abspath(__file__))
 LIB_PATH = os.path.join(_HERE, "libmatten_hip.so")
 
-ABI_VERSION = 45
+ABI_VERSION = 46
 
 P = c_void_p
 SIGNATURES = {
@@ -16,6 +16,9 @@
     "matten_group_workspace_bytes": (c_size_t, [c_int64, c_int64]),
     "matten_csr_counting_max_avg_degree": (c_int, []),
     "matten_csr_build": (c_int, [P, c_int64, c_int64, P, P, P, P, c_size_t, P, P]),
+    "matten_walk_records": (c_int, [P, P, c_int64, P, P]),
+    "matten_csr_build_walk": (c_int, [P, c_int64, c_int64, P, P, P, P, P, c_size_t, P, P]),
+    "matten_csr_split_walk": (c_int, [P, c_int64, c_int64, c_int64, P, P, P, P, P, P, P]),
     "matten_csr_split_bound": (c_int64, [c_int64, c_int64, c_int64]),
     "matten_csr_split": (c_int, [P, c_int64, c_int64, c_int64, P, P, P, P, P]),
     "matten_group_by_key": (c_int, [P, c_int64, c_int64, P, P, P, c_size_t, P, P]),
@@ -45,6 +48,8 @@
     "matten_tp_max_cols_l1": (c_int, []),
     "matten_tp_groups_hash": (c_int, []),
     "matten_tp_fused": (c_int, [P, c_int64, P, P, c_int64, P, c_int64, P, P, c_int64, P, P, c_int64, c_int64, c_int64, c_int64, c_float, P, P, P, P, P]),
+    "matten_tp_fused_walk": (c_int, [P, c_int64, P, P, c_int64, P, c_int64, P, P, P, c_int64, P, P, c_int64, c_int64, c_int64, c_int64, c_float, P, P, P, P,
+                                     P]),
     "matten_species_linear": (c_int, [P, c_int64, P, P, c_int64, P, c_int64, P, c_int64, c_int64, P, c_int64, c_int64, P, P]),
     "matten_species_linear_rows": (c_int, [P, c_int64, P, P, c_int64, P, c_int64, P, c_int64, c_int64, P, c_int64, c_int64, P, P]),
     "matten_radial_mlp_bwd_small_slices": (c_int64, [c_int64]),
@@ -86,6 +91,8 @@
     "matten_neighbor_summary": (c_int, [P, P, c_int64, P, P]),
     "matten_neighbor_fill": (c_int, [P, P, P, P, P, P, ctypes.c_double, c_int64, c_int64, P, c_int64, P, P, P, P, c_int64,
                                      P, P, P, P]),
+    "matten_neighbor_fill_walk": (c_int, [P, P, P, P, P, P, ctypes.c_double, c_int64, c_int64, P, c_int64, P, P, P, P, c_int64,
+                                          P, P, P, P, P]),
     "matten_gate_bn": (c_int, [P, c_int64, P, c_int64, P, P, P, P, P, c_float, c_int64, P, P]),
     "matten_segment_reduce": (c_int, [P, c_int64, P, c_int64, c_int, P, P]),
     "matten_segment_minmax": (c_int, [P, c_int64, P, c_int64, c_int, P, P, P]),
diff --git a/matten_amd/autograd.py b/matten_amd/autograd.py
--- a/matten_amd/autograd.py
+++ b/matten_amd/autograd.py
@@ -191,7 +191,7 @@
             ctx.h2p, ctx.hs = h2p, hs
         return ops.tp_fused(x, h2p, w2p, data[DataKey.AMD_SH], data[DataKey.AMD_ROWPTR], data[DataKey.AMD_SRC], gent,
                             mod._tables.get("gumap", dev), len(p.fused_unit_map), p.fused_lds_floats_per_wave, p.d_mid, avg,
-                            num_neigh, a_split=(frag, inv))
+                            num_neigh, a_split=(frag, inv), walk=ops.walk_of(data[DataKey.AMD_ROWPTR]))
 
     @staticmethod
     def backward(ctx, g):
diff --git a/matten_amd/csrc/csr.hip b/matten_amd/csrc/csr.hip
--- a/matten_amd/csrc/csr.hip
+++ b/matten_amd/csrc/csr.hip
@@ -74,13 +74,39 @@
 constexpr int CSR_HUB_THREADS = 1024;
 constexpr int CSR_HUB_BLOCKS = 64;
 
+__global__ void walk_records_kernel(const int32_t* __restrict__ rowptr, const int32_t* __restrict__ src_sorted, int64_t N,
+                                    int32_t* __restrict__ walk) {
+    const int64_t n = (int64_t)blockIdx.x * blockDim.x + threadIdx.x;
+    if (n >= N) return;
+    const int beg = rowptr[n], d = rowptr[n + 1] - beg;
+    int4 rec = {beg, d, 0, 0};
+    if (d > 0) {
+        rec.z = src_sorted[beg];
+        rec.w = src_sorted[beg + (d > 1 ? 1 : 0)];
+    }
+    reinterpret_cast<int4*>(walk)[n] = rec;
+}
+
+__device__ __forceinline__ void walk_put_src(int32_t* __restrict__ walk, int64_t node, int rank, int d, int32_t s) {
+    if (rank == 0) {
+        walk[4 * node + 2] = s;
+        if (d == 1) walk[4 * node + 3] = s;
+    } else if (rank == 1) {
+        walk[4 * node + 3] = s;
+    }
+}
+
 __global__ void csr_rank_kernel(const int64_t* __restrict__ edge_index, const int32_t* __restrict__ rowptr,
                                 const int32_t* __restrict__ ids, int64_t E, int64_t N, int32_t* __restrict__ perm,
-                                int32_t* __restrict__ src_sorted, int32_t* __restrict__ hubs) {
+                                int32_t* __restrict__ src_sorted, int32_t* __restrict__ hubs, int32_t* __restrict__ walk) {
     const int64_t node = ((int64_t)blockIdx.x * blockDim.x + threadIdx.x) >> 4;
     if (node >= N) return;
     const int sub = threadIdx.x & 15;
     const int beg = rowptr[node], d = rowptr[node + 1] - beg;
+    if (walk && sub == 0) {
+        walk[4 * node] = beg, walk[4 * node + 1] = d;
+        if (d == 0) walk[4 * node + 2] = 0, walk[4 * node + 3] = 0;
+    }
     if (d > CSR_HUB_DEGREE) {
         if (sub == 0) hubs[atomicAdd(&hubs[N], 1)] = (int32_t)node;
         return;
@@ -101,6 +127,7 @@
         int64_t s = edge_index[id];
         s = s < 0 ? 0 : (s >= N ? N - 1 : s);
         src_sorted[beg + rank] = (int32_t)s;
+        if (walk) walk_put_src(walk, node, rank, d, (int32_t)s);
     }
 }
 
@@ -108,7 +135,8 @@
                                                                   const int32_t* __restrict__ rowptr, int32_t* ids,
                                                                   int64_t N, int32_t* __restrict__ perm,
                                                                   int32_t* __restrict__ src_sorted,
-                                                                  const int32_t* __restrict__ hubs) {
+                                                                  const int32_t* __restrict__ hubs,
+                                                                  int32_t* __restrict__ walk) {
     const int n_hubs = hubs[N];
     for (int h = blockIdx.x; h < n_hubs; h += gridDim.x) {
         const int node = hubs[h];
@@ -133,6 +161,7 @@
             int64_t s = edge_index[id];
             s = s < 0 ? 0 : (s >= N ? N - 1 : s);
             src_sorted[beg + i] = (int32_t)s;
+            if (walk && i < 2) walk_put_src(walk, node, (int)i, d, (int32_t)s);
         }
         __syncthreads();
     }
@@ -214,7 +243,8 @@
 
 __global__ __launch_bounds__(1024) void csr_split_kernel(const int* __restrict__ rowptr, int N, int max_len, int nv_bound,
                                                          int* __restrict__ vrowptr, int64_t* __restrict__ vseg,
-                                                         const float* __restrict__ num_neigh, float* __restrict__ vnn) {
+                                                         const float* __restrict__ num_neigh, float* __restrict__ vnn,
+                                                         const int* __restrict__ src_sorted, int* __restrict__ vwalk) {
     __shared__ int sh[1024];
     __shared__ int carry_s;
     const int t = threadIdx.x;
@@ -244,8 +274,15 @@
             for (int i = 0; i < k; ++i) {
                 const int v = first + i;
                 if (v < nv_bound) {
-                    vrowptr[v] = beg + (int)((int64_t)i * d / k);
+                    const int vb = beg + (int)((int64_t)i * d / k);
+                    vrowptr[v] = vb;
                     if (vnn) vnn[v] = num_neigh[n];
+                    if (vwalk) {
+                        const int vd = (i + 1 < k ? beg + (int)((int64_t)(i + 1) * d / k) : beg + d) - vb;
+                        int4 rec = {vb, vd, 0, 0};
+                        if (vd > 0) rec.z = src_sorted[vb], rec.w = src_sorted[vb + (vd > 1 ? 1 : 0)];
+                        reinterpret_cast<int4*>(vwalk)[v] = rec;
+                    }
                 }
             }
         }
@@ -258,6 +295,7 @@
     for (int v = nv + t; v <= nv_bound; v += 1024) {
         vrowptr[v] = E;
         if (vnn && v < nv_bound) vnn[v] = 1.0f;
+        if (vwalk && v < nv_bound) reinterpret_cast<int4*>(vwalk)[v] = int4{E, 0, 0, 0};
     }
 }
 
@@ -290,15 +328,30 @@
 
 extern "C" int matten_csr_counting_max_avg_degree(void) { return (int)CSR_COUNTING_MAX_AVG_DEGREE; }
 
-extern "C" int matten_csr_build(const int64_t* edge_index, int64_t E, int64_t N, int32_t* perm, int32_t* rowptr,
-                                int32_t* src_sorted, void* workspace, size_t workspace_bytes, int32_t* err_flag,
-                                matten_stream_t stream_) {
+extern "C" int matten_walk_records(const int32_t* rowptr, const int32_t* src_sorted, int64_t N, int32_t* walk,
+                                   matten_stream_t stream_) {
+    if (N < 0 || N >= ((int64_t)1 << 29)) return MATTEN_EINVAL;
+    if (N == 0) return MATTEN_OK;
+    if (!rowptr || !walk || ((uintptr_t)walk & 15)) return MATTEN_EINVAL;
+    walk_records_kernel<<<(unsigned)matten_cdiv(N, 256), 256, 0, (hipStream_t)stream_>>>(rowptr, src_sorted, N, walk);
+    MATTEN_LAUNCH_CHECK();
+    return MATTEN_OK;
+}
+
+extern "C" int matten_csr_build_walk(const int64_t* edge_index, int64_t E, int64_t N, int32_t* perm, int32_t* rowptr,
+                                     int32_t* src_sorted, int32_t* walk, void* workspace, size_t workspace_bytes,
+                                     int32_t* err_flag, matten_stream_t stream_) {
     hipStream_t stream = (hipStream_t)stream_;
     if (E < 0 || N < 0 || N >= ((int64_t)1 << 31) || E >= ((int64_t)1 << 31)) return MATTEN_EINVAL;
     if (!rowptr || !err_flag) return MATTEN_EINVAL;
+    if (walk && (((uintptr_t)walk & 15) || N >= ((int64_t)1 << 29))) return MATTEN_EINVAL;
     if (E == 0) {
         zero_i32_kernel<<<(unsigned)matten_cdiv(N + 1, 256), 256, 0, stream>>>(rowptr, N + 1);
         MATTEN_LAUNCH_CHECK();
+        if (walk && N > 0) {
+            zero_i32_kernel<<<(unsigned)matten_cdiv(4 * N, 256), 256, 0, stream>>>(walk, 4 * N);
+            MATTEN_LAUNCH_CHECK();
+        }
         return MATTEN_OK;
     }
     if (!edge_index || !perm || !src_sorted || !workspace) return MATTEN_EINVAL;
@@ -331,12 +384,12 @@
         csr_place_kernel<<<(unsigned)matten_cdiv(E, T), T, 0, stream>>>(edge_index, E, N, rowptr, slot, ids);
         MATTEN_LAUNCH_CHECK();
         csr_rank_kernel<<<(unsigned)matten_cdiv(N * 16, T), T, 0, stream>>>(edge_index, rowptr, ids, E, N, perm,
-                                                                           src_sorted, deg);
+                                                                           src_sorted, deg, walk);
         MATTEN_LAUNCH_CHECK();
         if (E > CSR_HUB_DEGREE) {
             const int64_t max_hubs = E / CSR_HUB_DEGREE;
             csr_hub_kernel<<<(unsigned)(max_hubs < CSR_HUB_BLOCKS ? max_hubs : CSR_HUB_BLOCKS), CSR_HUB_THREADS, 0,
-                             stream>>>(edge_index, rowptr, ids, N, perm, src_sorted, deg);
+                             stream>>>(edge_index, rowptr, ids, N, perm, src_sorted, deg, walk);
             MATTEN_LAUNCH_CHECK();
         }
         return MATTEN_OK;
@@ -350,7 +403,15 @@
     MATTEN_LAUNCH_CHECK();
     csr_src_kernel<<<(unsigned)matten_cdiv(E, T), T, 0, stream>>>(edge_index, perm, E, N, src_sorted);
     MATTEN_LAUNCH_CHECK();
+    if (walk) return matten_walk_records(rowptr, src_sorted, N, walk, stream_);
     return MATTEN_OK;
+}
+
+extern "C" int matten_csr_build(const int64_t* edge_index, int64_t E, int64_t N, int32_t* perm, int32_t* rowptr,
+                                int32_t* src_sorted, void* workspace, size_t workspace_bytes, int32_t* err_flag,
+                                matten_stream_t stream_) {
+    return matten_csr_build_walk(edge_index, E, N, perm, rowptr, src_sorted, nullptr, workspace, workspace_bytes, err_flag,
+                                 stream_);
 }
 
 extern "C" int matten_group_by_key(const int64_t* key, int64_t n, int64_t n_keys, int32_t* order, int32_t* seg,
@@ -408,15 +469,22 @@
     return max_len > 0 ? n_nodes + n_edges / max_len : n_nodes;
 }
 
-extern "C" int matten_csr_split(const int32_t* rowptr, int64_t n_nodes, int64_t n_edges, int64_t max_len, int32_t* vrowptr,
-                                int64_t* vseg, const float* num_neigh, float* vnn, matten_stream_t stream_) {
+extern "C" int matten_csr_split_walk(const int32_t* rowptr, int64_t n_nodes, int64_t n_edges, int64_t max_len,
+                                     int32_t* vrowptr, int64_t* vseg, const float* num_neigh, float* vnn,
+                                     const int32_t* src_sorted, int32_t* vwalk, matten_stream_t stream_) {
     if (n_nodes < 0 || n_edges < 0 || max_len <= 0 || n_nodes >= ((int64_t)1 << 30) || n_edges >= ((int64_t)1 << 31))
         return MATTEN_EINVAL;
     if (!rowptr || !vrowptr || !vseg || ((num_neigh == nullptr) != (vnn == nullptr))) return MATTEN_EINVAL;
+    if (vwalk && (((uintptr_t)vwalk & 15) || (n_edges > 0 && !src_sorted))) return MATTEN_EINVAL;
     const int64_t bound = matten_csr_split_bound(n_nodes, n_edges, max_len);
-    if (bound >= ((int64_t)1 << 31)) return MATTEN_EINVAL;
+    if (bound >= ((int64_t)1 << 31) || (vwalk && bound >= ((int64_t)1 << 29))) return MATTEN_EINVAL;
     csr_split_kernel<<<1, 1024, 0, (hipStream_t)stream_>>>(rowptr, (int)n_nodes, (int)max_len, (int)bound, vrowptr, vseg,
-                                                          num_neigh, vnn);
+                                                          num_neigh, vnn, src_sorted, vwalk);
     MATTEN_LAUNCH_CHECK();
     return MATTEN_OK;
 }
+
+extern "C" int matten_csr_split(const int32_t* rowptr, int64_t n_nodes, int64_t n_edges, int64_t max_len, int32_t* vrowptr,
+                                int64_t* vseg, const float* num_neigh, float* vnn, matten_stream_t stream_) {
+    return matten_csr_split_walk(rowptr, n_nodes, n_edges, max_len, vrowptr, vseg, num_neigh, vnn, nullptr, nullptr, stream_);
+}
diff --git a/matten_amd/csrc/neighbor.hip b/matten_amd/csrc/neighbor.hip
--- a/matten_amd/csrc/neighbor.hip
+++ b/matten_amd/csrc/neighbor.hip
@@ -56,6 +56,7 @@
     int32_t* rowptr;
     int32_t* src_sorted;
     int32_t* perm;
+    int32_t* walk;
     int64_t n_atoms;
 };
 
@@ -86,10 +87,21 @@
     if (FILL && num_neigh && j == lo) num_neigh[i] = (float)(offsets[pair + n] - offsets[pair]);
     const int64_t pair_t = c.pair_ptr[b] + (j - lo) * n + (i - lo);
     int64_t out_t = 0;
+    int64_t seg_beg = 0;
+    int seg_deg = 0;
     if (FILL && csr.rowptr) {
         out_t = csr.offsets_t[pair_t] - csr.offsets_t[0];
         if (i == lo) csr.rowptr[j] = (int32_t)out_t;
         if (pair == 0) csr.rowptr[csr.n_atoms] = (int32_t)n_edges;
+        if (csr.walk) {
+            const int64_t pj = c.pair_ptr[b] + (j - lo) * n;
+            seg_beg = csr.offsets_t[pj] - csr.offsets_t[0];
+            seg_deg = (int)(csr.offsets_t[pj + n] - csr.offsets_t[pj]);
+            if (i == lo) {
+                csr.walk[4 * j] = (int32_t)seg_beg, csr.walk[4 * j + 1] = seg_deg;
+                if (seg_deg == 0) csr.walk[4 * j + 2] = 0, csr.walk[4 * j + 3] = 0;
+            }
+        }
     }
     int cnt = 0;
     for (int sx = x0; sx <= x1; ++sx)
@@ -115,6 +127,14 @@
                         if (csr.rowptr) {
                             csr.perm[out_t] = (int32_t)out;
                             csr.src_sorted[out_t] = (int32_t)i;
+                            if (csr.walk && out_t - seg_beg < 2) {
+                                if (out_t == seg_beg) {
+                                    csr.walk[4 * j + 2] = (int32_t)i;
+                                    if (seg_deg == 1) csr.walk[4 * j + 3] = (int32_t)i;
+                                } else {
+                                    csr.walk[4 * j + 3] = (int32_t)i;
+                                }
+                            }
                             ++out_t;
                         }
                         ++out;
@@ -185,11 +205,12 @@
     return MATTEN_OK;
 }
 
-extern "C" int matten_neighbor_fill(const double* pos, const double* cell, const int64_t* ptr, const double* frac,
-                                    const double* bound, const int64_t* pair_ptr, double r_cut, int64_t n_crystals,
-                                    int64_t max_atoms, const int64_t* offsets, int64_t n_edges, int64_t* edge_index,
-                                    float* edge_cell_shift, float* num_neigh, const int64_t* offsets_t, int64_t n_atoms,
-                                    int32_t* rowptr, int32_t* src_sorted, int32_t* perm, matten_stream_t stream_) {
+extern "C" int matten_neighbor_fill_walk(const double* pos, const double* cell, const int64_t* ptr, const double* frac,
+                                         const double* bound, const int64_t* pair_ptr, double r_cut, int64_t n_crystals,
+                                         int64_t max_atoms, const int64_t* offsets, int64_t n_edges, int64_t* edge_index,
+                                         float* edge_cell_shift, float* num_neigh, const int64_t* offsets_t,
+                                         int64_t n_atoms, int32_t* rowptr, int32_t* src_sorted, int32_t* perm,
+                                         int32_t* walk, matten_stream_t stream_) {
     hipStream_t stream = (hipStream_t)stream_;
     if (n_crystals < 0 || max_atoms < 0 || n_edges < 0 || !(r_cut > 0.0) || n_crystals > 65535) return MATTEN_EINVAL;
     if (n_crystals == 0 || max_atoms == 0) return MATTEN_OK;
@@ -199,11 +220,22 @@
     if (want_csr && (!offsets_t || !rowptr || n_atoms < 0 || n_edges >= ((int64_t)1 << 31) ||
                      (n_edges > 0 && (!src_sorted || !perm))))
         return MATTEN_EINVAL;
+    if (walk && (!want_csr || ((uintptr_t)walk & 15) || n_atoms >= ((int64_t)1 << 29))) return MATTEN_EINVAL;
     Cry c{pos, cell, ptr, frac, bound, pair_ptr};
-    CsrOut csr{offsets_t, want_csr ? rowptr : nullptr, src_sorted, perm, n_atoms};
+    CsrOut csr{offsets_t, want_csr ? rowptr : nullptr, src_sorted, perm, walk, n_atoms};
     dim3 grid((unsigned)matten_cdiv(max_atoms * max_atoms, 256), (unsigned)n_crystals);
     neighbor_kernel<true><<<grid, 256, 0, stream>>>(c, r_cut, nullptr, nullptr, offsets, edge_index, n_edges, edge_cell_shift,
                                                     num_neigh, csr);
     MATTEN_LAUNCH_CHECK();
     return MATTEN_OK;
 }
+
+extern "C" int matten_neighbor_fill(const double* pos, const double* cell, const int64_t* ptr, const double* frac,
+                                    const double* bound, const int64_t* pair_ptr, double r_cut, int64_t n_crystals,
+                                    int64_t max_atoms, const int64_t* offsets, int64_t n_edges, int64_t* edge_index,
+                                    float* edge_cell_shift, float* num_neigh, const int64_t* offsets_t, int64_t n_atoms,
+                                    int32_t* rowptr, int32_t* src_sorted, int32_t* perm, matten_stream_t stream_) {
+    return matten_neighbor_fill_walk(pos, cell, ptr, frac, bound, pair_ptr, r_cut, n_crystals, max_atoms, offsets, n_edges,
+                                     edge_index, edge_cell_shift, num_neigh, offsets_t, n_atoms, rowptr, src_sorted, perm,
+                                     nullptr, stream_);
+}
diff --git a/matten_amd/csrc/node.hip b/matten_amd/csrc/node.hip
--- a/matten_amd/csrc/node.hip
+++ b/matten_amd/csrc/node.hip
@@ -197,4 +197,4 @@
     return MATTEN_OK;
 }
 
-extern "C" int matten_abi_version(void) { return 45; }
+extern "C" int matten_abi_version(void) { return 46; }
diff --git a/matten_amd/csrc/tp_fused.hip b/matten_amd/csrc/tp_fused.hip
--- a/matten_amd/csrc/tp_fused.hip
+++ b/matten_amd/csrc/tp_fused.hip
@@ -35,8 +35,10 @@
 };
 
 template <int L1, int GI>
-__device__ __forceinline__ void run_group(const Args& a, const GroupEntry& ge, float* __restrict__ tile, int node,
-                                          int lane, bool valid, int beg, int deg_node, int maxdeg) {
+__device__ __forceinline__ void run_group(const Args& a, const GroupEntry& ge, float* __restrict__ tile, int cu_log2,
+                                          const UnitNodes& un, int lane) {
+    const int node = un.node, beg = un.beg, deg_node = un.deg, maxdeg = un.maxdeg;
+    const bool valid = un.valid;
     const int deg = valid ? deg_node : 0;
     using G = matten::Group<L1, GI>;
     constexpr int NC = G::NC;
@@ -45,7 +47,6 @@
     for (int k = 0; k < G::NACC; ++k) acc[k] = 0.0f;
 
     const unsigned mask = ge.mask;
-    const int cu_log2 = ge.cu_log2;
     const int cu = 1 << cu_log2;
     const int npw = 64 >> cu_log2;
     const int ch_log2 = npw >= 16 ? 0 : (4 - (6 - cu_log2));
@@ -98,8 +99,8 @@
     float xn[G::D1];
     int src_nn;
     {
-        const int src0 = a.src_sorted[min(beg, e_last)];
-        src_nn = a.src_sorted[min(beg + 1, e_last)];
+        const int src0 = un.has_src ? un.src0 : a.src_sorted[min(beg, e_last)];
+        src_nn = un.has_src ? un.src1 : a.src_sorted[min(beg + 1, e_last)];
         const float* xp0 = a.x + (int64_t)src0 * a.d_in + xcol;
 #pragma unroll
         for (int i = 0; i < G::D1; ++i) xn[i] = xp0[i];
@@ -166,7 +167,7 @@
     StoreAgg{}.store<G>(a, ge, acc, a_scale_inv, node, j, u, valid);
 }
 
-#define MATTEN_RGS_ARGS a, ge, tile, stage, (um >> 8) & 0xffff, tile_id, r, reps, lane, StoreAgg{}
+#define MATTEN_RGS_ARGS a, ge, tile, stage, (um >> 8) & 0xffff, cu_log2, raw0, tile_id, r, reps, lane, StoreAgg{}
 #define MATTEN_RGS(L1, GI, TT, TD, P) \
     do { \
         using HM = HotMask<L1, GI>; \
@@ -199,7 +200,7 @@
 #endif
 
 #define MATTEN_GROUP_CASE(L1, GI) \
-    case (L1 * matten::GROUP_KIND_STRIDE + GI): run_group<L1, GI>(a, ge, tile, un.node, lane, un.valid, un.beg, un.deg, un.maxdeg); break;
+    case (L1 * matten::GROUP_KIND_STRIDE + GI): run_group<L1, GI>(a, ge, tile, cu_log2, un, lane); break;
 
 #ifndef TPF_MIN_BLOCKS
 #define TPF_MIN_BLOCKS 3
@@ -241,14 +242,17 @@
     const bool shared_stage = (um >> 24) & 1;
     const int reps = 1 << ((um >> 27) & 3);
 
-    const int cu_log2 = ge.cu_log2;
+    int cu_log2;
+    if ((um >> 29) & 7) cu_log2 = ((um >> 29) & 7) - 1;
+    else cu_log2 = ge.cu_log2;
+    const RawNodes raw0 = unit_nodes_issue(a, a.walk != nullptr, cu_log2, tile_id, r, lane);
     const int nodes_per_wave = 64 >> cu_log2;
     if (shared_stage) {
         float* stage = lds + WAVES_PER_BLOCK * a.lds_per_wave;
         const bool paired = (um >> 26) & 1;
         if ((um >> 25) & 1) {
-            if (paired) run_loader_only_paired(a, ge, stage, tile_id, r, reps, lane);
-            else run_loader_only(a, ge, stage, tile_id, r, reps, lane);
+            if (paired) run_loader_only_paired(a, ge, stage, cu_log2, raw0, tile_id, r, reps, lane);
+            else run_loader_only(a, ge, stage, cu_log2, raw0, tile_id, r, reps, lane);
             return;
         }
         switch (ge.kind & (KIND_MERGED - 1)) {
@@ -258,7 +262,7 @@
         return;
     }
 #if !(defined(MATTEN_LAB) && defined(TPF_ONLY_VARIANT))
-    const UnitNodes un = unit_nodes(a, ge, tile_id, r, lane);
+    const UnitNodes un = unit_nodes_finish(a, raw0, ge.mul);
     switch (ge.kind & (KIND_MERGED - 1)) {
         TPF_FOR_EACH_GROUP(MATTEN_GROUP_CASE)
         default: break;
@@ -572,13 +576,13 @@
 }
 #endif
 
-extern "C" int matten_tp_fused(const float* x, int64_t d_in, const uint16_t* h2s, const float* w2p, int64_t w_pad,
-                               const float* sh_sorted, int64_t sh_stride, const int32_t* rowptr,
-                               const int32_t* src_sorted, int64_t n_nodes, const int32_t* group_entries,
-                               const int32_t* unit_map, int64_t n_entries, int64_t units_per_tile,
-                               int64_t lds_floats_per_wave, int64_t d_mid, float avg_num_neighbors,
-                               const float* num_neigh, const uint16_t* a_split, const float* a_scale_inv, float* agg,
-                               matten_stream_t stream_) {
+extern "C" int matten_tp_fused_walk(const float* x, int64_t d_in, const uint16_t* h2s, const float* w2p, int64_t w_pad,
+                                    const float* sh_sorted, int64_t sh_stride, const int32_t* rowptr,
+                                    const int32_t* src_sorted, const int32_t* walk, int64_t n_nodes,
+                                    const int32_t* group_entries, const int32_t* unit_map, int64_t n_entries,
+                                    int64_t units_per_tile, int64_t lds_floats_per_wave, int64_t d_mid,
+                                    float avg_num_neighbors, const float* num_neigh, const uint16_t* a_split,
+                                    const float* a_scale_inv, float* agg, matten_stream_t stream_) {
     hipStream_t stream = (hipStream_t)stream_;
     if (n_nodes < 0 || d_in <= 0 || w_pad <= 0 || sh_stride < 32 || (sh_stride & 3) || n_entries <= 0 ||
         units_per_tile <= 0 || d_mid <= 0 || lds_floats_per_wave <= 0 || (lds_floats_per_wave & 3))
@@ -590,7 +594,8 @@
     const size_t lds = sizeof(float) * ((size_t)lds_floats_per_wave * WAVES_PER_BLOCK + STAGE_TOTAL_FLOATS + PAIR_INFO_INTS);
     if (lds > 64 * 1024) return MATTEN_EINVAL;
     if ((a_split == nullptr) != (a_scale_inv == nullptr)) return MATTEN_EINVAL;
-    Args a{x, (const _Float16*)h2s, w2p, (const _Float16*)a_split, a_scale_inv, sh_sorted, rowptr, src_sorted, num_neigh, agg, (int)d_in, (int)w_pad, (int)sh_stride,
+    if ((uintptr_t)walk & 15) return MATTEN_EINVAL;
+    Args a{x, (const _Float16*)h2s, w2p, (const _Float16*)a_split, a_scale_inv, sh_sorted, rowptr, src_sorted, (const WalkRec*)walk, num_neigh, agg, (int)d_in, (int)w_pad, (int)sh_stride,
            (int)d_mid, (int)n_nodes, (int)lds_floats_per_wave, avg_num_neighbors};
     const int n_tiles = (int)matten_cdiv(n_nodes, TILE_NODES);
     const int blocks_per_tile = (int)matten_cdiv(units_per_tile, WAVES_PER_BLOCK);
@@ -610,6 +615,18 @@
     return MATTEN_OK;
 }
 
+extern "C" int matten_tp_fused(const float* x, int64_t d_in, const uint16_t* h2s, const float* w2p, int64_t w_pad,
+                               const float* sh_sorted, int64_t sh_stride, const int32_t* rowptr,
+                               const int32_t* src_sorted, int64_t n_nodes, const int32_t* group_entries,
+                               const int32_t* unit_map, int64_t n_entries, int64_t units_per_tile,
+                               int64_t lds_floats_per_wave, int64_t d_mid, float avg_num_neighbors,
+                               const float* num_neigh, const uint16_t* a_split, const float* a_scale_inv, float* agg,
+                               matten_stream_t stream_) {
+    return matten_tp_fused_walk(x, d_in, h2s, w2p, w_pad, sh_sorted, sh_stride, rowptr, src_sorted, nullptr, n_nodes,
+                                group_entries, unit_map, n_entries, units_per_tile, lds_floats_per_wave, d_mid,
+                                avg_num_neighbors, num_neigh, a_split, a_scale_inv, agg, stream_);
+}
+
 extern "C" int matten_tp_max_cols(void) { return TPF_MAX_COLS; }
 extern "C" int matten_tp_max_cols_l0(void) { return TPF_MAX_COLS_L0; }
 extern "C" int matten_tp_max_cols_l1(void) { return TPF_MAX_COLS_L1; }
diff --git a/matten_amd/csrc/tp_walk.h b/matten_amd/csrc/tp_walk.h
--- a/matten_amd/csrc/tp_walk.h
+++ b/matten_amd/csrc/tp_walk.h
@@ -148,6 +148,9 @@
 };
 static_assert(sizeof(GroupEntry) == 32 * 4, "GroupEntry layout");
 
+struct __attribute__((aligned(16))) WalkRec { int beg, deg, src0, src1; };
+static_assert(sizeof(WalkRec) == 16, "WalkRec layout");
+
 struct Args {
     const float* x;
     const _Float16* h2s;
@@ -157,6 +160,7 @@
     const float* sh;
     const int* rowptr;
     const int* src_sorted;
+    const WalkRec* walk;
     const float* num_neigh;
     float* agg;
     int d_in, w_pad, sh_stride, d_mid, n_nodes, lds_per_wave;
@@ -169,31 +173,38 @@
 
 struct UnitNodes {
     int node, beg, deg, maxdeg;
-    bool valid;
+    int src0, src1;
+    bool valid, has_src;
 };
 struct RawNodes {
-    int node, b0, b1;
-    bool valid;
+    int node, u;
+    WalkRec rec;
+    bool in_range, walked;
 };
-__device__ __forceinline__ RawNodes unit_nodes_issue(const Args& a, const GroupEntry& ge, int tile_id, int r, int lane) {
-    const int cu_log2 = ge.cu_log2;
+__device__ __forceinline__ RawNodes unit_nodes_issue(const Args& a, bool use_walk, int cu_log2, int tile_id, int r, int lane) {
     const int nodes_per_wave = 64 >> cu_log2;
     const int g_in_tile = r * nodes_per_wave + (lane >> cu_log2);
-    const int u = lane & ((1 << cu_log2) - 1);
     RawNodes n;
+    n.u = lane & ((1 << cu_log2) - 1);
     n.node = tile_id * TILE_NODES + g_in_tile;
-    const bool in_range = (g_in_tile < TILE_NODES) && (n.node < a.n_nodes);
-    n.valid = in_range && (u < ge.mul);
-    n.b0 = 0, n.b1 = 0;
-    if (in_range) {
-        n.b0 = a.rowptr[n.node];
-        n.b1 = a.rowptr[n.node + 1];
+    n.in_range = (g_in_tile < TILE_NODES) && (n.node < a.n_nodes);
+    n.rec = WalkRec{0, 0, 0, 0};
+    n.walked = use_walk;
+    if (n.in_range) {
+        if (use_walk) {
+            n.rec = a.walk[n.node];
+        } else {
+            n.rec.beg = a.rowptr[n.node];
+            n.rec.deg = a.rowptr[n.node + 1];
+        }
     }
     return n;
 }
-__device__ __forceinline__ UnitNodes unit_nodes_finish(const RawNodes& raw) {
+__device__ __forceinline__ UnitNodes unit_nodes_finish(const Args& a, const RawNodes& raw, int mul) {
     UnitNodes n;
-    n.node = raw.node, n.valid = raw.valid, n.beg = raw.b0, n.deg = raw.b1 - raw.b0;
+    n.node = raw.node, n.valid = raw.in_range && (raw.u < mul), n.beg = raw.rec.beg;
+    n.deg = raw.walked ? raw.rec.deg : raw.rec.deg - raw.rec.beg;
+    n.src0 = raw.rec.src0, n.src1 = raw.rec.src1, n.has_src = raw.walked;
     int maxdeg = n.deg;
 #pragma unroll
     for (int off = 32; off > 0; off >>= 1) maxdeg = max(maxdeg, __shfl_xor(maxdeg, off));
@@ -201,8 +212,8 @@
     n.maxdeg = maxdeg;
     return n;
 }
-__device__ __forceinline__ UnitNodes unit_nodes(const Args& a, const GroupEntry& ge, int tile_id, int r, int lane) {
-    return unit_nodes_finish(unit_nodes_issue(a, ge, tile_id, r, lane));
+__device__ __forceinline__ UnitNodes unit_nodes(const Args& a, int cu_log2, int mul, int tile_id, int r, int lane) {
+    return unit_nodes_finish(a, unit_nodes_issue(a, a.walk != nullptr, cu_log2, tile_id, r, lane), mul);
 }
 
 constexpr int STAGE_ROW = 68;
@@ -325,11 +336,12 @@
 };
 
 __device__ __forceinline__ void run_loader_only_paired(const Args& a, const GroupEntry& ge, float* __restrict__ stage,
-                                                       int tile_id, int r0, int reps, int lane) {
+                                                       int cu_log2, const RawNodes& raw0, int tile_id, int r0, int reps,
+                                                       int lane) {
     for (int rep = 0; rep < reps; ++rep) {
-        const UnitNodes un = unit_nodes(a, ge, tile_id, r0 + 2 * rep, lane);
+        const UnitNodes un = rep == 0 ? unit_nodes_finish(a, raw0, ge.mul) : unit_nodes(a, cu_log2, ge.mul, tile_id, r0 + 2 * rep, lane);
         PairLoader ld;
-        ld.init(a, stage, reinterpret_cast<int*>(stage + STAGE_TOTAL_FLOATS), ge.cu_log2, un.beg, un.deg, un.maxdeg);
+        ld.init(a, stage, reinterpret_cast<int*>(stage + STAGE_TOTAL_FLOATS), cu_log2, un.beg, un.deg, un.maxdeg);
         ld.issue(0);
         ld.publish(0);
         __syncthreads();
@@ -343,12 +355,12 @@
 }
 
 template <int TT>
-__device__ __forceinline__ void run_loader_only_t(const Args& a, const GroupEntry& ge, float* __restrict__ stage, int tile_id,
-                                                  int r0, int reps, int lane) {
+__device__ __forceinline__ void run_loader_only_t(const Args& a, const GroupEntry& ge, float* __restrict__ stage, int cu_log2,
+                                                  const RawNodes& raw0, int tile_id, int r0, int reps, int lane) {
     for (int rep = 0; rep < reps; ++rep) {
-        const UnitNodes un = unit_nodes(a, ge, tile_id, r0 + rep, lane);
+        const UnitNodes un = rep == 0 ? unit_nodes_finish(a, raw0, ge.mul) : unit_nodes(a, cu_log2, ge.mul, tile_id, r0 + rep, lane);
         StageLoader<TT> ld;
-        ld.init(a, stage, ge.cu_log2, un.beg, un.deg);
+        ld.init(a, stage, cu_log2, un.beg, un.deg);
         ld.issue(0);
         ld.publish(0);
         __syncthreads();
@@ -360,19 +372,22 @@
         }
     }
 }
-__device__ __forceinline__ void run_loader_only(const Args& a, const GroupEntry& ge, float* __restrict__ stage, int tile_id,
-                                                int r0, int reps, int lane) {
-    if ((64 >> ge.cu_log2) > 16) run_loader_only_t<2>(a, ge, stage, tile_id, r0, reps, lane);
-    else run_loader_only_t<1>(a, ge, stage, tile_id, r0, reps, lane);
+__device__ __forceinline__ void run_loader_only(const Args& a, const GroupEntry& ge, float* __restrict__ stage, int cu_log2,
+                                                const RawNodes& raw0, int tile_id, int r0, int reps, int lane) {
+    if ((64 >> cu_log2) > 16) run_loader_only_t<2>(a, ge, stage, cu_log2, raw0, tile_id, r0, reps, lane);
+    else run_loader_only_t<1>(a, ge, stage, cu_log2, raw0, tile_id, r0, reps, lane);
 }
 
 template <int L1, int GI>
 struct TwoDeepOk { static constexpr bool value = L1 == 0 || (L1 == 1 && (GI == 0 || TPF_PAIR_SUM)); };
 
+template <int L1, int GI, bool PAIRED>
+struct WalkRecOk { static constexpr bool value = !(PAIRED && GI == 0 && (L1 == 0 || L1 == 2 || L1 == 3)); };
+
 template <int L1, int GI, int TT, int TWO_DEEP, bool PAIRED, unsigned CMASK, class Epilogue>
 __device__ __forceinline__ void run_group_shared(const Args& a, const GroupEntry& ge, float* __restrict__ tile,
-                                                 float* __restrict__ stage, int entry, int tile_id, int r0, int reps, int lane,
-                                                 const Epilogue& epi) {
+                                                 float* __restrict__ stage, int entry, int cu_log2, const RawNodes& raw0,
+                                                 int tile_id, int r0, int reps, int lane, const Epilogue& epi) {
     static_assert(!PAIRED || TT == 1, "paired workgroups stage 2 x 16 rows");
 #if TPF_TRACING
     const unsigned tr_in_hi = tpf_stamp_hi();
@@ -386,7 +401,6 @@
     constexpr int NC = G::NC;
 
     const unsigned mask = ge.mask;
-    const int cu_log2 = ge.cu_log2;
     const int cu = 1 << cu_log2;
     const int npw = 64 >> cu_log2;
     const int ch_log2 = npw >= 16 ? 0 : 4 - (6 - cu_log2);
@@ -473,7 +487,7 @@
         if constexpr (chunk_deep) {
             int s0q[XQ];
 #pragma unroll
-            for (int i = 0; i < XQ; ++i) s0q[i] = a.src_sorted[min(beg + i, e_last)];
+            for (int i = 0; i < XQ; ++i) s0q[i] = (un.has_src && i < 2) ? (i == 0 ? un.src0 : un.src1) : a.src_sorted[min(beg + i, e_last)];
 #pragma unroll
             for (int i = 0; i < XQ; ++i) sq[i] = a.src_sorted[min(beg + CH + i, e_last)];
 #pragma unroll
@@ -483,8 +497,8 @@
             }
             return;
         }
-        const int src0 = a.src_sorted[min(beg, e_last)];
-        const int src1 = a.src_sorted[min(beg + 1, e_last)];
+        const int src0 = un.has_src ? un.src0 : a.src_sorted[min(beg, e_last)];
+        const int src1 = un.has_src ? un.src1 : a.src_sorted[min(beg + 1, e_last)];
         const float* xp0 = a.x + (int64_t)src0 * a.d_in + xcol;
 #pragma unroll
         for (int i = 0; i < G::D1; ++i) xn[i] = xp0[i];
@@ -498,13 +512,14 @@
         }
     };
     constexpr int RSTEP = PAIRED ? 2 : 1;
-    start_group(unit_nodes(a, ge, tile_id, r0, lane));
+    start_group(unit_nodes_finish(a, raw0, ge.mul));
     for (int rep = 0; rep < reps; ++rep) {
 #if TPF_TRACING
     const unsigned tr_rep = rep == 0 ? tr_in : tpf_stamp();
 #endif
     const bool more = rep + 1 < reps;
-    const RawNodes raw_next = unit_nodes_issue(a, ge, tile_id, r0 + RSTEP * (rep + (more ? 1 : 0)), lane);
+    const RawNodes raw_next = unit_nodes_issue(a, WalkRecOk<L1, GI, PAIRED>::value && a.walk != nullptr, cu_log2, tile_id,
+                                               r0 + RSTEP * (rep + (more ? 1 : 0)), lane);
     float acc[G::NACC];
 #pragma unroll
     for (int k = 0; k < G::NACC; ++k) acc[k] = 0.0f;
@@ -713,12 +728,12 @@
 #endif
     const int node_done = node;
     const bool valid_done = valid;
-    if (TPF_REP_PREFETCH && more) start_group(unit_nodes_finish(raw_next));
+    if (TPF_REP_PREFETCH && more) start_group(unit_nodes_finish(a, raw_next, ge.mul));
 #if TPF_TRACING
     tr_epi_sg += (unsigned)(tpf_stamp() - tr_end);
 #endif
     epi.template store<G>(a, ge, acc, a_scale_inv, node_done, j, u, valid_done);
-    if (!TPF_REP_PREFETCH && more) start_group(unit_nodes_finish(raw_next));
+    if (!TPF_REP_PREFETCH && more) start_group(unit_nodes_finish(a, raw_next, ge.mul));
 #if TPF_TRACING
     if (a.trace && lane == 0) {
         if (rep + 1 == reps) asm volatile("s_waitcnt vmcnt(0)" ::: "memory");
diff --git a/matten_amd/nn/_nequip.py b/matten_amd/nn/_nequip.py
--- a/matten_amd/nn/_nequip.py
+++ b/matten_amd/nn/_nequip.py
@@ -17,7 +17,7 @@
 def ensure_graph(data: DataKey.Type, err=None) -> DataKey.Type:
     if DataKey.AMD_ROWPTR not in data:
         n_nodes = data[DataKey.POSITIONS].shape[0]
-        perm, rowptr, src, err = ops.csr_build(data[DataKey.EDGE_INDEX], n_nodes, err=err)
+        perm, rowptr, src, _, err = ops.csr_build_walk(data[DataKey.EDGE_INDEX], n_nodes, err=err)
         data[DataKey.AMD_PERM], data[DataKey.AMD_ROWPTR], data[DataKey.AMD_SRC] = perm, rowptr, src
         data["_amd_csr_err"] = err
     return data
diff --git a/matten_amd/nn/utils.py b/matten_amd/nn/utils.py
--- a/matten_amd/nn/utils.py
+++ b/matten_amd/nn/utils.py
@@ -317,14 +317,19 @@
                 key = ("_amd_csr_split", piece, num_neigh is None)
                 split = data.get(key)
                 if split is None or split[3] is not rowptr:
-                    split = ops.csr_split(rowptr, data[DataKey.AMD_SRC].shape[0], piece, num_neigh) + (rowptr,)
+                    split = ops.csr_split(rowptr, data[DataKey.AMD_SRC].shape[0], piece, num_neigh,
+                                          src_sorted=data[DataKey.AMD_SRC]) + (rowptr,)
                     data[key] = split
+            walked = rowptr if split is None else split[0]
+            walk = ops.walk_of(walked)
+            if walk is None:
+                walk = ops.walk_records(walked, data[DataKey.AMD_SRC])
             agg = ops.tp_fused(
                 node_feats, h2p, w2p, data[DataKey.AMD_SH], rowptr if split is None else split[0], data[DataKey.AMD_SRC],
                 out_layout[0] if out_layout is not None else self._tables.get("gentries", dev),
                 self._tables.get("gumap", dev), len(self.plan.fused_unit_map),
                 self.plan.fused_lds_floats_per_wave, out_layout[1] if out_layout is not None else self.plan.d_mid, avg,
-                num_neigh if split is None else split[2], a_split=self.a_split(r0, r1),
+                num_neigh if split is None else split[2], a_split=self.a_split(r0, r1), walk=walk,
             )
             return agg if split is None else ops.segment_reduce(agg, split[1], mean=False)
         w_edge = self.weight_nn(data[DataKey.AMD_GEOM], int(nb), r0, r1)
diff --git a/matten_amd/ops.py b/matten_amd/ops.py
--- a/matten_amd/ops.py
+++ b/matten_amd/ops.py
@@ -90,7 +90,31 @@
     return err
 
 
+def walk_of(rowptr: torch.Tensor):
+    return getattr(rowptr, "_amd_walk", None)
+
+
+def walk_records(rowptr: torch.Tensor, src_sorted: torch.Tensor) -> torch.Tensor:
+    lib = _lib.load()
+    rowptr = _need(rowptr, torch.int32, "rowptr")
+    src_sorted = _need(src_sorted, torch.int32, "src_sorted")
+    N = rowptr.shape[0] - 1
+    walk = torch.empty(N, 4, dtype=torch.int32, device=rowptr.device)
+    _lib.check(lib.matten_walk_records(_ptr(rowptr), _ptr(src_sorted), N, _ptr(walk), _stream()), "matten_walk_records")
+    rowptr._amd_walk = walk
+    return walk
+
+
+def csr_build_walk(edge_index: torch.Tensor, n_nodes: int, err: torch.Tensor = None):
+    return _csr_build(edge_index, n_nodes, err, True)
+
+
 def csr_build(edge_index: torch.Tensor, n_nodes: int, err: torch.Tensor = None) -> Tuple[torch.Tensor, torch.Tensor, torch.Tensor, torch.Tensor]:
+    perm, rowptr, src, _, err = _csr_build(edge_index, n_nodes, err, False)
+    return perm, rowptr, src, err
+
+
+def _csr_build(edge_index, n_nodes: int, err, want_walk: bool):
     lib = _lib.load()
     edge_index = _need(edge_index, torch.int64, "edge_index")
     E = edge_index.shape[1]
@@ -98,18 +122,21 @@
     perm = torch.empty(E, dtype=torch.int32, device=dev)
     rowptr = torch.empty(n_nodes + 1, dtype=torch.int32, device=dev)
     src = torch.empty(E, dtype=torch.int32, device=dev)
+    walk = torch.empty(n_nodes, 4, dtype=torch.int32, device=dev) if want_walk else None
     err = _err_flag(err, dev)
     nbytes = lib.matten_csr_workspace_bytes(E, n_nodes)
     ws = torch.empty(max(nbytes, 1), dtype=torch.uint8, device=dev)
     _lib.check(
-        lib.matten_csr_build(_ptr(edge_index), E, n_nodes, _ptr(perm), _ptr(rowptr), _ptr(src), _ptr(ws), nbytes,
-                             _ptr(err), _stream()),
+        lib.matten_csr_build_walk(_ptr(edge_index), E, n_nodes, _ptr(perm), _ptr(rowptr), _ptr(src), _ptr(walk), _ptr(ws),
+                                  nbytes, _ptr(err), _stream()),
         "matten_csr_build",
     )
-    return perm, rowptr, src, err
-
-
-def csr_split(rowptr: torch.Tensor, n_edges: int, max_len: int, num_neigh: torch.Tensor = None):
+    if walk is not None:
+        rowptr._amd_walk = walk
+    return perm, rowptr, src, walk, err
+
+
+def csr_split(rowptr: torch.Tensor, n_edges: int, max_len: int, num_neigh: torch.Tensor = None, src_sorted: torch.Tensor = None):
     lib = _lib.load()
     rowptr = _need(rowptr, torch.int32, "rowptr")
     N = rowptr.shape[0] - 1
@@ -121,8 +148,14 @@
     if num_neigh is not None:
         num_neigh = _need(num_neigh, torch.float32, "num_neigh")
         vnn = torch.empty(bound, dtype=torch.float32, device=dev)
-    _lib.check(lib.matten_csr_split(_ptr(rowptr), N, n_edges, max_len, _ptr(vrowptr), _ptr(vseg), _ptr(num_neigh), _ptr(vnn),
-                                    _stream()), "matten_csr_split")
+    vwalk = None
+    if src_sorted is not None:
+        src_sorted = _need(src_sorted, torch.int32, "src_sorted")
+        vwalk = torch.empty(bound, 4, dtype=torch.int32, device=dev)
+    _lib.check(lib.matten_csr_split_walk(_ptr(rowptr), N, n_edges, max_len, _ptr(vrowptr), _ptr(vseg), _ptr(num_neigh),
+                                         _ptr(vnn), _ptr(src_sorted), _ptr(vwalk), _stream()), "matten_csr_split")
+    if vwalk is not None:
+        vrowptr._amd_walk = vwalk
     return vrowptr, vseg, vnn
 
 
@@ -568,7 +601,7 @@
 
 def tp_fused(x, h2p, w2p, sh_sorted, rowptr, src_sorted, entries, unit_map, units_per_tile: int,
              lds_floats_per_wave: int, d_mid: int, avg_num_neighbors: float, num_neigh=None,
-             a_split=None) -> torch.Tensor:
+             a_split=None, walk=None) -> torch.Tensor:
     lib = _lib.load()
     from .plan import TP_TILE_NODES
 
@@ -599,14 +632,18 @@
             raise ValueError("a_scale_inv needs one value per group entry")
     if unit_map.numel() != units_per_tile:
         raise ValueError(f"unit_map has {unit_map.numel()} units, expected {units_per_tile} (plan.fused_unit_map)")
+    if walk is not None:
+        walk = _need(walk, torch.int32, "walk")
+        if tuple(walk.shape) != (N, 4):
+            raise ValueError(f"walk must be [{N},4] int32 (one record per row of rowptr), got {tuple(walk.shape)}")
     agg = torch.empty(N, d_mid, dtype=torch.float32, device=x.device)
     with _timed(f"tp_scatter/d_mid={d_mid}/d_in={x.shape[1]}"):
-        rc = lib.matten_tp_fused(_ptr(x), d_in, _ptr(h2p), _ptr(w2p), w2p.shape[1], _ptr(sh_sorted),
-                                 sh_sorted.shape[1], _ptr(rowptr), _ptr(src_sorted), N, _ptr(entries),
-                                 _ptr(unit_map), entries.shape[0], units_per_tile, lds_floats_per_wave, d_mid,
-                                 float(avg_num_neighbors or 0.0), _ptr(num_neigh),
-                                 _ptr(a_split[0]) if a_split is not None else None,
-                                 _ptr(a_split[1]) if a_split is not None else None, _ptr(agg), _stream())
+        rc = lib.matten_tp_fused_walk(_ptr(x), d_in, _ptr(h2p), _ptr(w2p), w2p.shape[1], _ptr(sh_sorted),
+                                      sh_sorted.shape[1], _ptr(rowptr), _ptr(src_sorted), _ptr(walk), N, _ptr(entries),
+                                      _ptr(unit_map), entries.shape[0], units_per_tile, lds_floats_per_wave, d_mid,
+                                      float(avg_num_neighbors or 0.0), _ptr(num_neigh),
+                                      _ptr(a_split[0]) if a_split is not None else None,
+                                      _ptr(a_split[1]) if a_split is not None else None, _ptr(agg), _stream())
     _lib.check(rc, "matten_tp_fused")
     return agg
 
@@ -1019,17 +1056,21 @@
     edge_index = torch.empty(2, E, dtype=torch.int64, device=dev)
     shifts = torch.empty(E, 3, dtype=torch.float32, device=dev)
     num_neigh = torch.empty(N, dtype=torch.float32, device=dev)
-    csr = offsets_t = None
+    csr = offsets_t = walk = None
     if want_csr and n_pairs and E < 2 ** 31:
+        walk = torch.empty(N, 4, dtype=torch.int32, device=dev)
         offsets_t = scan[n_pairs:]
         csr = (torch.empty(E, dtype=torch.int32, device=dev), torch.empty(N + 1, dtype=torch.int32, device=dev),
                torch.empty(E, dtype=torch.int32, device=dev))
     with _timed("neighbor_fill"):
         _lib.check(
-            lib.matten_neighbor_fill(_ptr(pos64), _ptr(cell64), _ptr(ptr), _ptr(frac), _ptr(bound), _ptr(pair_ptr),
-                                     float(r_cut), B, int(max_atoms), _ptr(offsets), E, _ptr(edge_index), _ptr(shifts),
-                                     _ptr(num_neigh), _ptr(offsets_t), N, _ptr(csr[1]) if csr else None,
-                                     _ptr(csr[2]) if csr else None, _ptr(csr[0]) if csr else None, _stream()),
+            lib.matten_neighbor_fill_walk(_ptr(pos64), _ptr(cell64), _ptr(ptr), _ptr(frac), _ptr(bound), _ptr(pair_ptr),
+                                          float(r_cut), B, int(max_atoms), _ptr(offsets), E, _ptr(edge_index), _ptr(shifts),
+                                          _ptr(num_neigh), _ptr(offsets_t), N, _ptr(csr[1]) if csr else None,
+                                          _ptr(csr[2]) if csr else None, _ptr(csr[0]) if csr else None, _ptr(walk),
+                                          _stream()),
             "matten_neighbor_fill",
         )
+    if csr is not None:
+        csr[1]._amd_walk = walk
     return edge_index, shifts, num_neigh, offsets, int(min_edges), csr
diff --git a/matten_amd/plan.py b/matten_amd/plan.py
--- a/matten_amd/plan.py
+++ b/matten_amd/plan.py
@@ -84,6 +84,7 @@
 FUSED_UNIT_LOADER_ONLY = 1 << 25
 FUSED_UNIT_PAIRED = 1 << 26
 FUSED_UNIT_REPS_SHIFT = 27
+FUSED_UNIT_LANES_SHIFT = 29
 
 
 def fused_persist(cu_log2: int, groups: int, mode: str) -> int:
@@ -142,8 +143,9 @@
     for cu_log2, blk, mode in fused_workgroups(ent, order):
         groups = -(-TP_TILE_NODES // max(1, 64 >> cu_log2))
         assert groups < 256
+        assert 0 <= cu_log2 <= 6 and all(int(ent[e][3]) == cu_log2 for e in blk), "unit word and entry disagree on the lanes per node"
         reps = fused_persist(cu_log2, groups, mode) if mode in ("shared", "paired") else 1
-        rbits = (reps.bit_length() - 1) << FUSED_UNIT_REPS_SHIFT
+        rbits = ((reps.bit_length() - 1) << FUSED_UNIT_REPS_SHIFT) | ((cu_log2 + 1) << FUSED_UNIT_LANES_SHIFT)
         if mode == "shared":
             for r in range(0, groups, reps):
                 shared_units += [FUSED_UNIT_SHARED | rbits | (e << 8) | r for e in blk]
@@ -156,7 +158,7 @@
                     shared_units += [flags | (e << 8) | rr for e in blk]
                     shared_units += [flags | FUSED_UNIT_LOADER_ONLY | (blk[-1] << 8) | rr] * (2 - len(blk))
         else:
-            plain_units += [(e << 8) | r for e in blk for r in range(groups)]
+            plain_units += [rbits | (e << 8) | r for e in blk for r in range(groups)]
     return np.array(shared_units + plain_units, dtype=np.int64).astype(np.int32)
 
 
```

After: 1.175 billion edge-TP/s. 0.928x the previous value.
